# aszepieniec/stark-anatomy

Measured on AMD Instinct MI355X. Metric: ntt_field_elements_per_sec, higher is better.
Workload: dtype u128; 1 GPU; ntt_fwd_inv_2^20_1gpu; log2n=20, parallelism=single, passes_per_transform=2

## Files before the change

### stark-anatomy_amd/csrc/core.h

```cpp
#pragma once
#include <hip/hip_runtime.h>
#include <dlfcn.h>
#include <cstdio>
#include <cstdlib>
#include <cstring>
#include <algorithm>
#include <atomic>
#include <chrono>
#include <cerrno>
#include <thread>
#include <sys/random.h>
#include <deque>
#include <functional>
#include <future>
#include <map>
#include <mutex>
#include <string>
#include <tuple>
#include <vector>

#pragma GCC visibility push(default)
#include "../../include/starkcore.h"
#pragma GCC visibility pop
#include "ntt_plan.h"

namespace sc { struct FoldIn; }
using namespace sc;

struct sc_vec {
    Fe* d;
    uint64_t n;
    bool owned = true;
};
struct sc_later {
    int slot;
    uint64_t seq;
    hipStream_t st;
};
struct sc_merkle {
    uint64_t* d_levels;
    uint64_t N;
    int logN;
    int slot = -1;
    uint64_t seq = 0;
    hipStream_t st = nullptr;
    bool have_root = false;
    bool lazy = false;
    uint8_t root[64] = {};
};

struct sc_merkle_forest {
    uint64_t* d_levels;
    uint64_t N, count;
    int logN;
    uint64_t* h_roots = nullptr;
    Fe* d_cm = nullptr;
    hipEvent_t done = nullptr;
    hipStream_t st = nullptr;
    bool have_roots = false;
};

namespace sci {

struct DevBuf {
    void* p = nullptr;
    size_t bytes = 0;
};

struct PlanKey {
    int logn;
    uint64_t lo, hi;
    bool operator<(const PlanKey& o) const { return std::tie(logn, lo, hi) < std::tie(o.logn, o.lo, o.hi); }
};
struct PlanTables {
    Fe* mt = nullptr;
    int mt_log = 0;
    Fe* tl = nullptr;
    Fe* th = nullptr;
    Fe* th_ninv = nullptr;
    struct Direct { int logA, logR; bool scaled; Fe* d; };
    std::vector<Direct> direct;
    uint64_t last_use = 0;
};
struct OuterKey {
    uint64_t lo, hi, order, len, batch, col_base;
    int ninv;
    bool operator<(const OuterKey& o) const { return std::tie(lo, hi, order, len, batch, col_base, ninv) < std::tie(o.lo, o.hi, o.order, o.len, o.batch, o.col_base, o.ninv); }
};
struct OuterTable {
    Fe* d = nullptr;
    uint64_t last_use = 0;
};
struct PowKey {
    uint64_t lo, hi, hi_count;
    bool operator<(const PowKey& o) const { return std::tie(lo, hi, hi_count) < std::tie(o.lo, o.hi, o.hi_count); }
};
struct PowTables {
    Fe* lo = nullptr;
    Fe* hi = nullptr;
    uint64_t last_use = 0;
};

struct Ctx {
    bool init = false;
    int device = -1;
    hipStream_t stream = nullptr;
    std::string err;
    NttTuning tuning;
    std::map<PlanKey, PlanTables> plans;
    std::map<PowKey, PowTables> pows;
    std::map<OuterKey, OuterTable> outers;
    uint64_t tick = 0;
    bool foreign_streams = false;
    int small_divisor_direct = 1;
    int div_cols_launch_log = 26;
    int tree_cols_launch_log = 26;
    int eval_chunk_log = 8;
    int eval_points_across_min = 32;
    int eval_across_min_products_log = 26;
    int rescue_tree_split_max_nodes = -1;
    int grind_window = -1;
    int grind_unrolled = 0;
    int div_cols_chunk = 0;
    std::vector<hipStream_t> seen_streams;
    DevBuf scratch[8];
    std::map<hipStream_t, DevBuf> ntt_work;
    std::map<hipStream_t, DevBuf> ntt_flags;
    int fast_fixups = 1;
    int num_cus = 256;
    int xcd_remap = 1;
    int fixed_shapes = 1;
    int prio_balance = -1;
    int wave_local = 1;
    unsigned long long* trace = nullptr;
    int forest_four_lane_wgs = 256;
    int merkle_big_nlev = 2;
    int fri_tail = -1;
    int fri_tail_stall = -1;
    size_t verify_stage_bytes = 64ull << 20;
    uint8_t* root_slots = nullptr;
    uint8_t* later_words = nullptr;
    uint64_t root_seq = 0;
    std::vector<int> free_root_slots;
};
constexpr int ROOT_SLOTS = 256;
constexpr size_t ROOT_SLOT_BYTES = 128;
constexpr size_t LATER_WORD_BYTES = 128;
constexpr long SPIN_POLLS = 40000000;

struct PendingFree {
    void* p;
    size_t bytes;
    std::vector<hipEvent_t> evs;
};
#define HIPCHK(expr)                                                                                          \
    do {                                                                                                      \
        hipError_t _e = (expr);                                                                               \
        if (_e != hipSuccess) return fail(SC_ERR_HIP, std::string(#expr) + ": " + hipGetErrorString(_e));     \
    } while (0)

#define SCCHK(expr)              \
    do {                         \
        int _rc = (expr);        \
        if (_rc != SC_OK) return _rc; \
    } while (0)

struct NttOpts {
    uint64_t in_limit = ~0ull;
    const PowTables* coset = nullptr;
    uint32_t cols = 1;
    uint64_t col_stride_in = 0;
};
constexpr uint64_t COLS_ELEMS_PER_LAUNCH = 1ull << 26;
constexpr uint64_t SMALL_DIVISOR = 8;

constexpr uint64_t FUSE_MAX_W = 1ull << 17;

enum BuildMode { BUILD_SYNC = 0, BUILD_ASYNC = 1, BUILD_NOROOT = 2 };

extern Ctx g;
extern std::mutex g_mu;
extern hipStream_t g_comm_stream_for_free;
extern std::future<void> g_rand_worker;
extern size_t g_rand_prefetched;
extern std::multimap<size_t, void*> g_pool;
extern size_t g_pool_bytes, g_pool_cap;
extern std::deque<PendingFree> g_pending;
extern std::vector<hipEvent_t> g_event_pool;

void reap_pending(bool block);
hipError_t pool_alloc(void** p, size_t bytes);
void pool_free(void* p, size_t bytes);
void pool_clear();
hipEvent_t event_get();
int fail(int code, const std::string& msg);
int ensure_init();
int grow_buffer(DevBuf& b, size_t bytes, void** out);
inline int scratch(int slot, size_t bytes, void** out) { return grow_buffer(g.scratch[slot], bytes, out); }
int check_root(Fe root, uint64_t n);
int build_pow_table(Fe** out, uint64_t count, Fe base_m, uint64_t step, Fe scale_m, hipStream_t st);
void free_plans();
int evict_outer_tables();
int get_plan(Fe root, int logn, bool need_ninv, hipStream_t st, PlanTables** out);
inline NttTables tables_of(const PlanTables& t) {
    NttTables tb;
    tb.mt = t.mt; tb.mt_log = t.mt_log; tb.tl = t.tl; tb.th = t.th;
    return tb;
}
int get_pow(Fe base, uint64_t count, hipStream_t st, PowTables** out);
int plan_batched_direct(NttPlanDesc& d, BatchKind kind, int loglen, int logbatch, PlanTables* pt, const Fe* in, Fe* work, Fe* out, BatchExtras ex, hipStream_t st, bool* ok);
int run_plan(NttPlanDesc& d, hipStream_t st);
int ntt_device(const Fe* d_in, Fe* d_out, int logn, Fe root, bool inverse_scale, const NttOpts& o, hipStream_t st);
Fe root_inverse(Fe root, uint64_t n);
int ntt_any(const Fe* d_in, Fe* d_out, uint64_t n, Fe root, bool inverse, const NttOpts& o, hipStream_t st);
int upload(void* d, const void* h, size_t bytes, hipStream_t st);
int download(void* h, const void* d, size_t bytes, hipStream_t st);
int pointwise_div_device(const Fe* a, const Fe* b, Fe* out, uint64_t n, hipStream_t st);
int pointwise_div_enqueue(const Fe* a, const Fe* b, Fe* out, uint64_t n, hipStream_t st, uint32_t* flag);
int gather_device(const Fe* v, const uint64_t* d_idx, uint64_t k, Fe* d_out, hipStream_t st);
int read_small_polled(const void* d_src, size_t bytes, hipStream_t st, void* host_out);
bool upload_small(void* d_dst, const void* host, size_t bytes, hipStream_t st);

int merkle_climb(uint64_t* levels, uint64_t N, int lvl, hipStream_t st, volatile uint64_t* host = nullptr, uint64_t seq = 0, bool* published = nullptr);
int merkle_finish(uint64_t* levels, uint64_t width, hipStream_t st);
int root_slot_get();
int merkle_build_device(const Fe* d_elems, uint64_t N, uint8_t root_out[64], sc_merkle** tree, hipStream_t st, BuildMode mode = BUILD_SYNC, const FoldIn* fold = nullptr);
int merkle_root_wait(sc_merkle* t, bool from_free = false);
void root_poll_unlocked(std::unique_lock<std::mutex>& lk, const sc_merkle* t);
int fold_prepare(const Fe* d_in, uint64_t N, Fe alpha, Fe offset, Fe omega, Fe* d_out, hipStream_t st, FoldIn* f);
int fold_device(const Fe* d_in, uint64_t N, Fe alpha, Fe offset, Fe omega, Fe* d_out, hipStream_t st);
int fold_and_build(const Fe* d_in, uint64_t N, Fe alpha, Fe offset, Fe omega, Fe* d_out, sc_merkle** tree, hipStream_t st);
int fold_constants(uint64_t N, Fe offset, Fe omega, hipStream_t st, PowTables** pw_out, Fe* i2o_m_out);
int host_pool_get(size_t bytes, void** out);
int host_pool_put(void* p);
bool host_pool_holds(const void* p, size_t bytes);
int verify_stage_buffer(size_t bytes, uint8_t** out);

int grind_seeds_locked(const std::string& what, const void* seeds, uint64_t count, int bits, uint64_t start, uint64_t max_nonces, uint64_t* nonces_out,
                       uint8_t* found_out, void* stream);

Fe canonical_root(int logn);
Fe ninv_scaled(int logn, int j);
int ntt_cols(const Fe* in, Fe* out, int loglen, int logbatch, bool inverse, hipStream_t st);

constexpr size_t SEEN_STREAMS = 8;
inline hipStream_t pick_stream(void* s) {
    if (s && (hipStream_t)s != g.stream) {
        g.foreign_streams = true;
        hipStream_t st = (hipStream_t)s;
        if (g.seen_streams.size() <= SEEN_STREAMS && std::find(g.seen_streams.begin(), g.seen_streams.end(), st) == g.seen_streams.end())
            g.seen_streams.push_back(st);
    }
    return s ? (hipStream_t)s : g.stream;
}
inline void release_after_streams(void* p, size_t bytes) {
    if (!p) return;
    if (g.seen_streams.size() > SEEN_STREAMS) {
        (void)hipDeviceSynchronize();
        g.seen_streams.clear();
        pool_free(p, bytes);
        return;
    }
    PendingFree f{p, bytes, {}};
    auto mark = [&](hipStream_t st) -> bool {
        if (hipStreamQuery(st) == hipSuccess) return true;
        (void)hipGetLastError();
        hipEvent_t e = event_get();
        if (!e) { (void)hipStreamSynchronize(st); (void)hipGetLastError(); return true; }
        if (hipEventRecord(e, st) != hipSuccess) { (void)hipGetLastError(); g_event_pool.push_back(e); return false; }
        f.evs.push_back(e);
        return true;
    };
    if (g.stream) (void)mark(g.stream);
    if (g_comm_stream_for_free) (void)mark(g_comm_stream_for_free);
    for (size_t i = 0; i < g.seen_streams.size();) {
        if (mark(g.seen_streams[i])) ++i;
        else g.seen_streams.erase(g.seen_streams.begin() + i);
    }
    if (f.evs.empty()) { pool_free(p, bytes); return; }
    g_pending.push_back(std::move(f));
    reap_pending(false);
}
inline Fe fe_from(const uint64_t v[2]) { return Fe{v[0], v[1]}; }
inline bool is_pow2(uint64_t n) { return n && !(n & (n - 1)); }
inline int ilog2(uint64_t n) { int l = 0; while ((1ull << l) < n) ++l; return l; }

struct PoolTmp {
    void* p = nullptr;
    size_t bytes = 0;
    ~PoolTmp() { if (p) pool_free(p, bytes); }
    int get(size_t b) {
        bytes = b;
        HIPCHK(pool_alloc(&p, b));
        return SC_OK;
    }
    Fe* fe() const { return (Fe*)p; }
};

struct PoolTmpAsync {
    void* p = nullptr;
    size_t bytes = 0;
    ~PoolTmpAsync() { if (p) release_after_streams(p, bytes); }
    int get(size_t b) {
        bytes = b ? b : sizeof(Fe);
        HIPCHK(pool_alloc(&p, bytes));
        return SC_OK;
    }
    Fe* fe() const { return (Fe*)p; }
};

}
using namespace sci;
```

### stark-anatomy_amd/csrc/core.hip

```cpp
#include "core.h"


template <int LOGE> struct PassThreads { static constexpr int value = LOGE >= 4 ? 256 : (LOGE == 3 ? 512 : 1024); };

template <int LOGE>
__global__ void __launch_bounds__(PassThreads<LOGE>::value) ntt_pass_kernel(const PassParams P, uint32_t ntiles, int xcd_remap) {
    extern __shared__ __attribute__((aligned(16))) unsigned char smem_raw[];
    Fe* lds = reinterpret_cast<Fe*>(smem_raw);
    uint32_t wg = blockIdx.x, colbits = 0;
    if (P.col_enable) { colbits = (wg >> P.col_tiles_log) << P.col_tiles_log; wg -= colbits; }
    uint32_t tile = wg;
    if (xcd_remap) tile = (wg & 7u) * (ntiles >> 3) + (wg >> 3);
    tile |= colbits;
    Fe* tw = lds + (1u << (P.logR + P.logC));
    tile_twiddles_to_lds(P, P.logR, threadIdx.x, blockDim.x, tw);
    __syncthreads();
    const int nrounds = (P.logR + LOGE - 1) / LOGE;
    int sh = P.logR;
    for (int r = 0; r < nrounds; ++r) {
        const int s = (r == 0) ? (P.logR - LOGE * (nrounds - 1)) : LOGE;
        sh -= s;
        ntt_round_dispatch<LOGE>(P, s, sh, r == 0, tile, threadIdx.x, lds, tw);
        if (r + 1 < nrounds) __syncthreads();
    }
}

constexpr int TRACE_STAMPS = 16;
template <int LOGE, int GLR, int GLC, bool TRACE, bool ALT = false>
__global__ void __launch_bounds__(1 << (GLR + GLC - LOGE)) ntt_pass_kernel_fixed(const PassParams P, uint32_t ntiles, int xcd_remap, int wave_local) {
    extern __shared__ __attribute__((aligned(16))) unsigned char smem_raw[];
    Fe* lds = reinterpret_cast<Fe*>(smem_raw);
    unsigned long long* trow = nullptr;
    if constexpr (TRACE) {
        if (P.trace) {
            trow = P.trace + ((size_t)blockIdx.x * (blockDim.x >> 6) + (threadIdx.x >> 6)) * TRACE_STAMPS;
            if ((threadIdx.x & 63u) == 0) { trow[0] = __builtin_amdgcn_s_memtime(); trow[15] = __builtin_amdgcn_s_memrealtime(); }
        }
    }
    uint32_t wg = blockIdx.x, colbits = 0;
    if (P.col_enable) { colbits = (wg >> P.col_tiles_log) << P.col_tiles_log; wg -= colbits; }
    uint32_t tile = wg;
    if (xcd_remap) tile = (wg & 7u) * (ntiles >> 3) + (wg >> 3);
    tile |= colbits;
    Fe* tw = lds + (1u << (GLR + GLC));
    auto stamp = [&](int i) {
        if constexpr (TRACE) {
            if (trow) {
                if (i == 2) __builtin_amdgcn_s_waitcnt(0);
                if ((threadIdx.x & 63u) == 0 && i < 13) trow[i] = __builtin_amdgcn_s_memtime();
            }
        }
    };
    auto sync = [] { __syncthreads(); };
    auto wsync = [] { __builtin_amdgcn_fence(__ATOMIC_RELEASE, "wavefront"); __builtin_amdgcn_wave_barrier(); __builtin_amdgcn_fence(__ATOMIC_ACQUIRE, "wavefront"); };
    FixedRounds<LOGE, GLR, GLC, 0, ALT>::run(P, tile, threadIdx.x, lds, tw, sync, wsync, stamp, wave_local != 0);
    if constexpr (TRACE) {
        if (trow && (threadIdx.x & 63u) == 0) { __builtin_amdgcn_s_waitcnt(0); trow[14] = __builtin_amdgcn_s_memtime(); trow[13] = __builtin_amdgcn_s_memrealtime(); }
    }
}

template <int GLR, int GLC>
__device__ __forceinline__ uint32_t fixed8_tile(const PassParams& P, uint32_t index, uint32_t ntiles, int xcd_remap) {
    uint32_t wg = index, colbits = 0;
    if (P.col_enable) { colbits = (wg >> P.col_tiles_log) << P.col_tiles_log; wg -= colbits; }
    uint32_t tile = wg;
    if (xcd_remap) tile = (wg & 7u) * (ntiles >> 3) + (wg >> 3);
    return tile | colbits;
}
template <int GLR, int GLC>
__global__ void __launch_bounds__(1 << (GLR + GLC - 3)) __attribute__((amdgpu_waves_per_eu(4)))
ntt_pass_kernel_fixed8(const PassParams P, uint32_t ntiles, int xcd_remap, int wave_local, uint32_t* flags) {
    extern __shared__ __attribute__((aligned(16))) unsigned char smem_raw[];
    Fe* lds = reinterpret_cast<Fe*>(smem_raw);
    const uint32_t tile = fixed8_tile<GLR, GLC>(P, blockIdx.x, ntiles, xcd_remap);
    Fe* tw = lds + (1u << (GLR + GLC));
    auto stamp = [](int) {};
    auto sync = [] { __syncthreads(); };
    auto wsync = [] { __builtin_amdgcn_fence(__ATOMIC_RELEASE, "wavefront"); __builtin_amdgcn_wave_barrier(); __builtin_amdgcn_fence(__ATOMIC_ACQUIRE, "wavefront"); };
    rare_t rare = 0;
    FixedRounds<3, GLR, GLC, 0, false, true>::run(P, tile, threadIdx.x, lds, tw, sync, wsync, stamp, wave_local != 0, rare);
    if (rare_any(rare)) Round<3, 3, GLR, GLC>::store_word_at(flags + blockIdx.x, 0u, 1u);
}

template <int GLR, int GLC>
__global__ void __launch_bounds__(1 << (GLR + GLC - 3)) __attribute__((amdgpu_waves_per_eu(4)))
ntt_pass_redo8_kernel(const PassParams P, uint32_t ntiles, int xcd_remap, int wave_local, uint32_t* flags, int all) {
    extern __shared__ __attribute__((aligned(16))) unsigned char smem_raw[];
    if (!all && flags[blockIdx.x] == 0) return;
    Fe* lds = reinterpret_cast<Fe*>(smem_raw);
    Fe* tw = lds + (1u << (GLR + GLC));
    auto stamp = [](int) {};
    auto sync = [] { __syncthreads(); };
    auto wsync = [] { __builtin_amdgcn_fence(__ATOMIC_RELEASE, "wavefront"); __builtin_amdgcn_wave_barrier(); __builtin_amdgcn_fence(__ATOMIC_ACQUIRE, "wavefront"); };
    FixedRounds<3, GLR, GLC, 0, false>::run(P, fixed8_tile<GLR, GLC>(P, blockIdx.x, ntiles, xcd_remap), threadIdx.x, lds, tw, sync, wsync, stamp, wave_local != 0);
    if (!all) __syncthreads();
    if (threadIdx.x == 0) flags[blockIdx.x] = 0;
}

__global__ void __launch_bounds__(256) pow_table_kernel(Fe* out, uint64_t count, Fe base_m, uint64_t step, Fe scale_m) {
    uint64_t i = (uint64_t)blockIdx.x * blockDim.x + threadIdx.x;
    if (i < count) out[i] = pow_table_entry(base_m, i, step, scale_m);
}

__global__ void __launch_bounds__(256) twiddle_table_kernel(Fe* out, int logB, uint64_t count, uint64_t scale_exp, const Fe* __restrict__ tl, const Fe* __restrict__ th) {
    uint64_t i = (uint64_t)blockIdx.x * blockDim.x + threadIdx.x;
    if (i >= count) return;
    uint64_t k = i >> logB, b = i & ((1ull << logB) - 1);
    out[i] = pow2level(tl, th, b * k * scale_exp);
}

__global__ void __launch_bounds__(256) pointwise_mul_kernel(const Fe* __restrict__ a, const Fe* __restrict__ b, Fe* __restrict__ out, uint64_t n) {
    uint64_t i = (uint64_t)blockIdx.x * blockDim.x + threadIdx.x;
    if (i < n) out[i] = fe_mul(a[i], b[i]);
}

template <int K>
__global__ void __launch_bounds__(256) pointwise_div_kernel(const Fe* __restrict__ a, const Fe* __restrict__ b, Fe* __restrict__ out, uint64_t n, uint32_t* flag) {
    const uint64_t nthreads = (uint64_t)gridDim.x * blockDim.x;
    const uint64_t t = (uint64_t)blockIdx.x * blockDim.x + threadIdx.x;
    Fe bm[K], pre[K];
    Fe acc = fe_mont_one();
    bool zero = false;
#pragma unroll
    for (int k = 0; k < K; ++k) {
        uint64_t i = t + (uint64_t)k * nthreads;
        Fe v = (i < n) ? b[i] : fe_one();
        zero |= fe_is_zero(v);
        bm[k] = to_mont(v);
        pre[k] = acc;
        acc = mont_mul(acc, bm[k]);
    }
    if (zero) atomicOr(flag, 1u);
    Fe inv = mont_inv(acc);
#pragma unroll
    for (int k = K - 1; k >= 0; --k) {
        uint64_t i = t + (uint64_t)k * nthreads;
        Fe ik = mont_mul(inv, pre[k]);
        inv = mont_mul(inv, bm[k]);
        if (i < n) out[i] = mont_mul(a[i], ik);
    }
}

__global__ void __launch_bounds__(256) short_poly_coset_kernel(const Fe* __restrict__ b, uint32_t nb, Fe off_m, const Fe* __restrict__ tl, const Fe* __restrict__ th, Fe* __restrict__ out, uint64_t order) {
    const uint64_t i = (uint64_t)blockIdx.x * blockDim.x + threadIdx.x;
    if (i >= order) return;
    const Fe x_m = mont_mul(off_m, pow2level(tl, th, i));
    Fe acc = b[nb - 1];
    for (uint32_t k = nb - 1; k-- > 0;) acc = fe_add(mont_mul(acc, x_m), b[k]);
    out[i] = acc;
}

__global__ void __launch_bounds__(256) scale_pow_kernel(const Fe* __restrict__ in, Fe* __restrict__ out, uint64_t n, const Fe* __restrict__ lo, const Fe* __restrict__ hi) {
    uint64_t i = (uint64_t)blockIdx.x * blockDim.x + threadIdx.x;
    if (i < n) out[i] = mont_mul(in[i], pow2level(lo, hi, i));
}

__global__ void __launch_bounds__(256) scale_slab_kernel(const Fe* __restrict__ in, Fe* __restrict__ out, uint64_t rows, int logcols, uint64_t row_len, uint64_t col_base,
                                                         const Fe* __restrict__ lo, const Fe* __restrict__ hi) {
    uint64_t t = (uint64_t)blockIdx.x * blockDim.x + threadIdx.x;
    if (t >= (rows << logcols)) return;
    uint64_t r = t >> logcols, c = t & ((1ull << logcols) - 1);
    out[t] = mont_mul(in[t], pow2level(lo, hi, r * row_len + col_base + c));
}

__global__ void __launch_bounds__(256) axpy_shift_kernel(Fe* __restrict__ acc, const Fe* __restrict__ src, uint64_t n_src, uint64_t shift, Fe w_m) {
    uint64_t j = (uint64_t)blockIdx.x * blockDim.x + threadIdx.x;
    if (j >= n_src) return;
    acc[shift + j] = fe_add(acc[shift + j], mont_mul(src[j], w_m));
}

constexpr int DEGREE_PER_THREAD = 4;
constexpr unsigned DEGREE_MAX_BLOCKS = 2048;
constexpr int DEGREE_SLOTS = 8;
__global__ void __launch_bounds__(256) vec_degree_kernel(const Fe* __restrict__ v, uint64_t n, long long* out) {
    const uint64_t step = (uint64_t)gridDim.x * (256 * DEGREE_PER_THREAD);
    long long best = -1;
    for (uint64_t base = (uint64_t)blockIdx.x * (256 * DEGREE_PER_THREAD) + threadIdx.x; base - threadIdx.x < n; base += step) {
        Fe x[DEGREE_PER_THREAD];
#pragma unroll
        for (int k = 0; k < DEGREE_PER_THREAD; ++k) {
            const uint64_t i = base + 256u * k;
            x[k] = i < n ? v[i] : Fe{0, 0};
        }
#pragma unroll
        for (int k = 0; k < DEGREE_PER_THREAD; ++k) {
            const unsigned long long lanes = __ballot(!fe_is_zero(x[k]));
            if (lanes) best = (long long)(base - (threadIdx.x & 63u) + 256u * k + (63 - __clzll((long long)lanes)));
        }
    }
    __shared__ long long wave_best[4];
    if ((threadIdx.x & 63u) == 0) wave_best[threadIdx.x >> 6] = best;
    __syncthreads();
    if (threadIdx.x == 0) {
        long long m = wave_best[0];
#pragma unroll
        for (int w = 1; w < 4; ++w) m = wave_best[w] > m ? wave_best[w] : m;
        if (m >= 0) atomicMax(out + (blockIdx.x & (DEGREE_SLOTS - 1)), m);
    }
}
__global__ void __launch_bounds__(256) vec_degree_cols_kernel(const Fe* __restrict__ v, uint64_t n, uint64_t ld, uint32_t per_col, long long* out) {
    const uint64_t col = blockIdx.x / per_col;
    const uint32_t part = blockIdx.x - (uint32_t)col * per_col;
    const Fe* __restrict__ w = v + col * ld;
    const uint64_t step = (uint64_t)per_col * (256 * DEGREE_PER_THREAD);
    long long best = -1;
    for (uint64_t base = (uint64_t)part * (256 * DEGREE_PER_THREAD) + threadIdx.x; base - threadIdx.x < n; base += step) {
        Fe x[DEGREE_PER_THREAD];
#pragma unroll
        for (int k = 0; k < DEGREE_PER_THREAD; ++k) {
            const uint64_t i = base + 256u * k;
            x[k] = i < n ? w[i] : Fe{0, 0};
        }
#pragma unroll
        for (int k = 0; k < DEGREE_PER_THREAD; ++k) {
            const unsigned long long lanes = __ballot(!fe_is_zero(x[k]));
            if (lanes) best = (long long)(base - (threadIdx.x & 63u) + 256u * k + (63 - __clzll((long long)lanes)));
        }
    }
    __shared__ long long wave_best[4];
    if ((threadIdx.x & 63u) == 0) wave_best[threadIdx.x >> 6] = best;
    __syncthreads();
    if (threadIdx.x == 0) {
        long long m = wave_best[0];
#pragma unroll
        for (int k = 1; k < 4; ++k) m = wave_best[k] > m ? wave_best[k] : m;
        if (m >= 0) atomicMax(out + col, m);
    }
}
static int degree_read(void* fl, hipStream_t st, long long* deg) {
    long long slots[DEGREE_SLOTS];
    SCCHK(read_small_polled(fl, sizeof slots, st, slots));
    long long m = -1;
    for (int i = 0; i < DEGREE_SLOTS; ++i) m = slots[i] > m ? slots[i] : m;
    *deg = m;
    return SC_OK;
}
static inline unsigned degree_blocks(uint64_t n) {
    const uint64_t b = (n + 256 * DEGREE_PER_THREAD - 1) / (256 * DEGREE_PER_THREAD);
    return (unsigned)(b < DEGREE_MAX_BLOCKS ? (b ? b : 1) : DEGREE_MAX_BLOCKS);
}

__global__ void __launch_bounds__(256) mpoly_eval_kernel(const Fe* __restrict__ vals_m, uint32_t nvars, uint64_t n, const uint8_t* __restrict__ exps,
                                                        const Fe* __restrict__ coef_m, uint32_t nterms, Fe* __restrict__ out, const uint64_t* __restrict__ where) {
    uint64_t i = (uint64_t)blockIdx.x * blockDim.x + threadIdx.x;
    if (i >= n) return;
    Fe acc{0, 0};
    for (uint32_t t = 0; t < nterms; ++t) {
        Fe p = coef_m[t];
        const uint8_t* e = exps + (size_t)t * nvars;
        for (uint32_t j = 0; j < nvars; ++j) {
            const uint32_t ej = e[j];
            if (ej == 0) continue;
            const Fe v = where ? vals_m[where[2 * j] * n + ((i + where[2 * j + 1]) & (n - 1))] : vals_m[(uint64_t)j * n + i];
            for (uint32_t k = 0; k < ej; ++k) p = mont_mul(p, v);
        }
        acc = fe_add(acc, p);
    }
    out[i] = from_mont(acc);
}
__global__ void __launch_bounds__(256) to_mont_kernel(Fe* __restrict__ a, uint64_t n) {
    uint64_t i = (uint64_t)blockIdx.x * blockDim.x + threadIdx.x;
    if (i < n) a[i] = to_mont(a[i]);
}

__global__ void __launch_bounds__(256) field_selftest_kernel(int op, const Fe* __restrict__ a, const Fe* __restrict__ b, Fe* __restrict__ out, uint64_t n) {
    uint64_t i = (uint64_t)blockIdx.x * blockDim.x + threadIdx.x;
    if (i >= n) return;
    Fe x = a[i], y = b[i], r;
    switch (op) {
        case 0: r = mont_mul(x, y); break;
        case 1: r = fe_add(x, y); break;
        case 2: r = fe_sub(x, y); break;
        case 3: r = fe_mul(x, y); break;
        case 4: r = fe_half(x); break;
        case 5: r = from_mont(mont_inv(to_mont(x))); break;
        case 7: {
            Fe r0, r1;
            mont_mul2(x, y, x, y, r0, r1);
            r = fe_eq(r0, r1) ? r0 : Fe{~0ull, ~0ull};
            break;
        }
        default: r = mont_mul_c(x, y); break;
    }
    out[i] = r;
}

template <bool MASK> __device__ __forceinline__ uint32_t selftest_word(rare_t rare) {
    const uint32_t own = MASK ? (uint32_t)((rare >> (threadIdx.x & 63u)) & 1u) : (uint32_t)(rare != 0);
    return own | (rare_any(rare) ? 2u : 0u);
}
__global__ void __launch_bounds__(256) field_selftest2_kernel(int op, const Fe* __restrict__ a, const Fe* __restrict__ b, const Fe* __restrict__ c,
                                                             const Fe* __restrict__ d, Fe* __restrict__ out, uint32_t* __restrict__ word, uint64_t n) {
    uint64_t i = (uint64_t)blockIdx.x * blockDim.x + threadIdx.x;
    if (i >= n) return;
    const Fe x = a[i], y = b[i], z = c[i], w = d[i];
    Fe r0{0, 0}, r1{0, 0}, r2{0, 0}, r3{0, 0};
    rare_t rare = 0;
    uint32_t flags = 0;
    switch (op) {
        case 0: mont_mul2(x, y, z, w, r0, r1); break;
        case 1: fe_addsub2(x, y, z, w, r0, r1, r2, r3); break;
        case 2: r0 = fe_add_fast(x, y, rare); flags = selftest_word<SC_ASM_ADDSUB != 0>(rare); break;
        case 3: r0 = fe_sub_fast(x, y, rare); flags = selftest_word<SC_ASM_ADDSUB != 0>(rare); break;
        case 4: r0 = mont_mul_fast(x, y, rare); flags = selftest_word<SC_ASM_MUL != 0>(rare); break;
        case 5: mont_mul2_fast(x, y, z, w, r0, r1, rare); flags = selftest_word<SC_ASM_MUL != 0>(rare); break;
        case 6: fe_addsub2_fast(x, y, z, w, r0, r1, r2, r3, rare); flags = selftest_word<SC_ASM_ADDSUB != 0>(rare); break;
        default: r0 = fe_neg(x); break;
    }
    out[i] = r0; out[n + i] = r1; out[2 * n + i] = r2; out[3 * n + i] = r3;
    word[i] = flags;
}

__global__ void __launch_bounds__(256) sample_bytes_kernel(const uint8_t* __restrict__ bytes, uint64_t count, uint32_t width, Fe* __restrict__ out) {
    uint64_t i = (uint64_t)blockIdx.x * blockDim.x + threadIdx.x;
    if (i >= count) return;
    out[i] = fe_sample_bytes(bytes + i * width, width);
}

__global__ void __launch_bounds__(256) gather_kernel(const Fe* __restrict__ v, const uint64_t* __restrict__ idx, uint64_t k, Fe* __restrict__ out) {
    uint64_t i = (uint64_t)blockIdx.x * blockDim.x + threadIdx.x;
    if (i < k) out[i] = v[idx[i]];
}


namespace sci {

Ctx g;
std::mutex g_mu;
hipStream_t g_comm_stream_for_free = nullptr;
std::future<void> g_rand_worker;
size_t g_rand_prefetched = 0;

std::multimap<size_t, void*> g_pool;
size_t g_pool_bytes = 0;
size_t g_pool_cap = 8ull << 30;

void reap_pending(bool block);
hipError_t pool_alloc(void** p, size_t bytes) {
    reap_pending(false);
    auto it = g_pool.find(bytes);
    if (it != g_pool.end()) {
        *p = it->second;
        g_pool.erase(it);
        g_pool_bytes -= bytes;
        return hipSuccess;
    }
    const bool slow_log = getenv("STARKCORE_LOG_SLOW_ALLOC") != nullptr;
    const auto t0 = std::chrono::steady_clock::now();
    hipError_t e = hipMalloc(p, bytes);
    if (slow_log) {
        const double ms = std::chrono::duration<double, std::milli>(std::chrono::steady_clock::now() - t0).count();
        if (ms > 1.0) fprintf(stderr, "starkcore: hipMalloc(%zu MB) took %.1f ms (pool %zu MB in %zu buffers)\n", bytes >> 20, ms, g_pool_bytes >> 20, g_pool.size());
    }
    if (e != hipSuccess) {
        (void)hipGetLastError();
        reap_pending(true);
        auto it2 = g_pool.find(bytes);
        if (it2 != g_pool.end()) {
            *p = it2->second;
            g_pool.erase(it2);
            g_pool_bytes -= bytes;
            return hipSuccess;
        }
        e = hipMalloc(p, bytes);
    }
    if (e != hipSuccess && !g_pool.empty()) {
        (void)hipDeviceSynchronize();
        for (auto& kv : g_pool) (void)hipFree(kv.second);
        g_pool.clear();
        g_pool_bytes = 0;
        (void)hipGetLastError();
        e = hipMalloc(p, bytes);
    }
    return e;
}

void pool_free(void* p, size_t bytes) {
    if (!p) return;
    if (g_pool_bytes + bytes <= g_pool_cap) {
        g_pool.emplace(bytes, p);
        g_pool_bytes += bytes;
    } else {
        const auto t0 = std::chrono::steady_clock::now();
        (void)hipFree(p);
        if (getenv("STARKCORE_LOG_SLOW_ALLOC")) {
            const double ms = std::chrono::duration<double, std::milli>(std::chrono::steady_clock::now() - t0).count();
            if (ms > 1.0) fprintf(stderr, "starkcore: hipFree(%zu MB) took %.1f ms (pool at its cap of %zu MB)\n", bytes >> 20, ms, g_pool_cap >> 20);
        }
    }
}

void pool_clear() {
    for (auto& kv : g_pool) (void)hipFree(kv.second);
    g_pool.clear();
    g_pool_bytes = 0;
}

std::deque<PendingFree> g_pending;
std::vector<hipEvent_t> g_event_pool;

hipEvent_t event_get() {
    if (!g_event_pool.empty()) { hipEvent_t e = g_event_pool.back(); g_event_pool.pop_back(); return e; }
    hipEvent_t e = nullptr;
    if (hipEventCreateWithFlags(&e, hipEventDisableTiming) != hipSuccess) { (void)hipGetLastError(); return nullptr; }
    return e;
}

void reap_pending(bool block) {
    for (size_t i = 0; i < g_pending.size();) {
        PendingFree& f = g_pending[i];
        bool done = true;
        for (hipEvent_t e : f.evs) {
            hipError_t q = block ? hipEventSynchronize(e) : hipEventQuery(e);
            if (q == hipErrorNotReady) { (void)hipGetLastError(); done = false; break; }
            if (q != hipSuccess) (void)hipGetLastError();
        }
        if (!done) { ++i; continue; }
        for (hipEvent_t e : f.evs) g_event_pool.push_back(e);
        pool_free(f.p, f.bytes);
        g_pending[i] = std::move(g_pending.back());
        g_pending.pop_back();
    }
}

int fail(int code, const std::string& msg) {
    g.err = msg;
    return code;
}

int ensure_init() {
    if (g.init) {
        static thread_local int bound = -1;
        if (bound != g.device) { HIPCHK(hipSetDevice(g.device)); bound = g.device; }
        return SC_OK;
    }
    int n = 0;
    hipError_t e = hipGetDeviceCount(&n);
    if (e != hipSuccess || n <= 0) return fail(SC_ERR_HIP, std::string("no HIP device available: ") + hipGetErrorString(e));
    int dev = 0;
    if (const char* lr = getenv("LOCAL_RANK")) dev = atoi(lr) % n;
    if (const char* sd = getenv("STARKCORE_DEVICE")) dev = atoi(sd) % n;
    HIPCHK(hipSetDevice(dev));
    HIPCHK(hipStreamCreateWithFlags(&g.stream, hipStreamNonBlocking));
    { int cus = 0; if (hipDeviceGetAttribute(&cus, hipDeviceAttributeMultiprocessorCount, dev) == hipSuccess && cus > 0) g.num_cus = cus; }
    { size_t free_b = 0, total_b = 0; if (hipMemGetInfo(&free_b, &total_b) == hipSuccess && total_b) g_pool_cap = total_b / 4; else (void)hipGetLastError(); }
    if (const char* lws = getenv("LOCAL_WORLD_SIZE")) { const int per_dev = (atoi(lws) + n - 1) / n; if (per_dev > 1) g_pool_cap /= (size_t)per_dev; }
    if (const char* cap = getenv("STARKCORE_POOL_CAP_MB")) g_pool_cap = (size_t)atoll(cap) << 20;
    g.device = dev;
    g.init = true;
    return SC_OK;
}

int grow_buffer(DevBuf& b, size_t bytes, void** out) {
    if (b.bytes < bytes) {
        if (b.p) { HIPCHK(hipDeviceSynchronize()); HIPCHK(hipFree(b.p)); b.p = nullptr; b.bytes = 0; }
        size_t want = bytes < (1u << 20) ? (1u << 20) : bytes;
        HIPCHK(hipMalloc(&b.p, want));
        b.bytes = want;
    }
    *out = b.p;
    return SC_OK;
}

int check_root(Fe root, uint64_t n) {
    if (fe_ge_p(root)) return fail(SC_ERR_BAD_ARG, "root is not a canonical residue");
    Fe rm = to_mont(root);
    Fe one = fe_mont_one();
    Fe half = mont_pow(rm, n / 2);
    Fe full = mont_mul(half, half);
    if (!fe_eq(full, one)) return fail(SC_ERR_ROOT_ORDER, "primitive root must be nth root of unity, where n is len(values)");
    if (fe_eq(half, one)) return fail(SC_ERR_ROOT_NOT_PRIMITIVE, "primitive root is not primitive nth root of unity, where n is len(values)");
    return SC_OK;
}

int build_pow_table(Fe** out, uint64_t count, Fe base_m, uint64_t step, Fe scale_m, hipStream_t st) {
    if (count == 0) count = 1;
    HIPCHK(hipMalloc((void**)out, count * sizeof(Fe)));
    unsigned blocks = (unsigned)((count + 255) / 256);
    hipLaunchKernelGGL(pow_table_kernel, dim3(blocks), dim3(256), 0, st, *out, count, base_m, step, scale_m);
    HIPCHK(hipGetLastError());
    return SC_OK;
}

void free_plan_tables(PlanTables& t) {
    hipFree(t.mt); hipFree(t.tl); hipFree(t.th);
    if (t.th_ninv) hipFree(t.th_ninv);
    for (const PlanTables::Direct& e : t.direct) hipFree(e.d);
}

void free_plans() {
    for (auto& kv : g.plans) free_plan_tables(kv.second);
    g.plans.clear();
    for (auto& kv : g.pows) { hipFree(kv.second.lo); hipFree(kv.second.hi); }
    g.pows.clear();
    for (auto& kv : g.outers) hipFree(kv.second.d);
    g.outers.clear();
}

constexpr uint64_t PIN_WINDOW = 64;
constexpr size_t PLAN_CAP = 256, POW_CAP = 64;

template <class Map, class FreeFn>
int evict_tables(Map& m, size_t cap, FreeFn free_entry) {
    if (m.size() < cap) return SC_OK;
    std::vector<std::pair<uint64_t, typename Map::iterator>> old;
    for (auto it = m.begin(); it != m.end(); ++it)
        if (it->second.last_use + PIN_WINDOW < g.tick) old.emplace_back(it->second.last_use, it);
    if (old.empty()) return SC_OK;
    std::sort(old.begin(), old.end(), [](const auto& a, const auto& b) { return a.first < b.first; });
    size_t drop = cap / 4 ? cap / 4 : 1;
    if (drop > old.size()) drop = old.size();
    HIPCHK(hipDeviceSynchronize());
    for (size_t i = 0; i < drop; ++i) { free_entry(old[i].second->second); m.erase(old[i].second); }
    return SC_OK;
}

int get_plan(Fe root, int logn, bool need_ninv, hipStream_t st, PlanTables** out) {
    PlanKey key{logn, root.lo, root.hi};
    auto it = g.plans.find(key);
    bool built = false;
    ++g.tick;
    if (it == g.plans.end()) {
        SCCHK(evict_tables(g.plans, PLAN_CAP, free_plan_tables));
        const uint64_t n = 1ull << logn;
        Fe rm = to_mont(root);
        const TableSizes sz = table_sizes(logn);
        PlanTables t;
        t.mt_log = sz.mt_log;
        SCCHK(build_pow_table(&t.mt, sz.mt, rm, n >> sz.mt_log, fe_mont_one(), st));
        SCCHK(build_pow_table(&t.tl, sz.tl, rm, 1, fe_mont_one(), st));
        SCCHK(build_pow_table(&t.th, sz.th, rm, 4096, fe_mont_one(), st));
        it = g.plans.emplace(key, t).first;
        built = true;
    }
    if (need_ninv && !it->second.th_ninv) {
        const uint64_t n = 1ull << logn;
        Fe ninv_m = mont_inv(to_mont(Fe{n, 0}));
        SCCHK(build_pow_table(&it->second.th_ninv, table_sizes(logn).th, to_mont(root), 4096, ninv_m, st));
        built = true;
    }
    if (built) HIPCHK(hipStreamSynchronize(st));
    it->second.last_use = g.tick;
    *out = &it->second;
    return SC_OK;
}

int get_pow(Fe base, uint64_t count, hipStream_t st, PowTables** out) {
    uint64_t hi_count = (count >> 12) + 1;
    uint64_t hc = 1; while (hc < hi_count) hc <<= 1;
    PowKey key{base.lo, base.hi, hc};
    auto it = g.pows.find(key);
    ++g.tick;
    if (it == g.pows.end()) {
        SCCHK(evict_tables(g.pows, POW_CAP, [](PowTables& t) { hipFree(t.lo); hipFree(t.hi); }));
        Fe bm = to_mont(base);
        PowTables t;
        SCCHK(build_pow_table(&t.lo, 4096, bm, 1, fe_mont_one(), st));
        SCCHK(build_pow_table(&t.hi, hc, bm, 4096, fe_mont_one(), st));
        HIPCHK(hipStreamSynchronize(st));
        it = g.pows.emplace(key, t).first;
    }
    it->second.last_use = g.tick;
    *out = &it->second;
    return SC_OK;
}

int direct_twiddles(PlanTables* pt, const NttPlanDesc& d, int i, bool scaled, hipStream_t st, const Fe** out) {
    const DirectTable t = direct_table(d, i, scaled);
    *out = nullptr;
    if (t.logR + t.logB > g.tuning.direct_tw_max_log) return SC_OK;
    for (const PlanTables::Direct& e : pt->direct)
        if (e.logA == t.logA && e.logR == t.logR && e.scaled == t.scaled) { *out = e.d; return SC_OK; }
    const uint64_t count = 1ull << (t.logR + t.logB);
    Fe* p;
    HIPCHK(hipMalloc((void**)&p, count * sizeof(Fe)));
    pt->direct.push_back({t.logA, t.logR, t.scaled, p});
    hipLaunchKernelGGL(twiddle_table_kernel, dim3((unsigned)((count + 255) / 256)), dim3(256), 0, st, p, t.logB, count, 1ull << t.logA,
                       pt->tl, t.scaled ? pt->th_ninv : pt->th);
    HIPCHK(hipGetLastError());
    HIPCHK(hipStreamSynchronize(st));
    *out = p;
    return SC_OK;
}

int plan_batched_direct(NttPlanDesc& d, BatchKind kind, int loglen, int logbatch, PlanTables* pt, const Fe* in, Fe* work, Fe* out, BatchExtras ex, hipStream_t st, bool* ok) {
    const NttTables tb = tables_of(*pt);
    *ok = plan_batched(d, kind, loglen, logbatch, tb, in, work, out, g.tuning, ex);
    if (!*ok || d.npasses != 2) return SC_OK;
    SCCHK(direct_twiddles(pt, d, 0, false, st, &ex.inner_twd));
    if (ex.inner_twd) *ok = plan_batched(d, kind, loglen, logbatch, tb, in, work, out, g.tuning, ex);
    return SC_OK;
}

int pass_flags(hipStream_t st, uint32_t nwg, uint32_t** out) {
    DevBuf& b = g.ntt_flags[st];
    const void* before = b.p;
    const size_t had = b.bytes;
    void* p;
    SCCHK(grow_buffer(b, (size_t)nwg * sizeof(uint32_t), &p));
    if (p != before || b.bytes != had) HIPCHK(hipMemsetAsync(p, 0, b.bytes, st));
    *out = (uint32_t*)p;
    return SC_OK;
}

template <int LOGE>
int launch_pass(const NttPassDesc& pd, hipStream_t st) {
    int remap = (g.xcd_remap && pd.ntiles >= 16 && (pd.ntiles & 7u) == 0) ? 1 : 0;
    const PassKernel k = pass_kernel(pd, g.fixed_shapes != 0);
    if constexpr (LOGE == 2) {
        if (k.kind == PK_FIXED4) {
            const int lr = pd.p.logR, lc = pd.p.logC;
#define SC_LAUNCH_FIXED(LR, LC, TR, ALT) \
    hipLaunchKernelGGL((ntt_pass_kernel_fixed<2, LR, LC, TR, ALT>), dim3(pd.ntiles * pd.cols), dim3(pd.threads), pd.lds_bytes, st, pd.p, pd.ntiles, remap, g.wave_local)
#define SC_FIXED(LR, LC)                                                          \
            if (lr == LR && lc == LC) {                                           \
                if (k.trace) SC_LAUNCH_FIXED(LR, LC, true, false);                \
                else if (k.alt) SC_LAUNCH_FIXED(LR, LC, false, true);             \
                else SC_LAUNCH_FIXED(LR, LC, false, false);                       \
                return SC_OK;                                                     \
            }
            SC_FIXED4_SHAPES(SC_FIXED)
#undef SC_FIXED
        }
    }
    if constexpr (LOGE == 3) {
        if (k.kind == PK_FIXED8) {
            const int lr = pd.p.logR, lc = pd.p.logC;
            const uint32_t nwg = pd.ntiles * pd.cols;
            const bool fast = g.fast_fixups != 0 && fast_pass_ok(pd.p) && !pass_in_place(pd);
            const int all = (!fast || g.fast_fixups == 2) ? 1 : 0;
            uint32_t* flags;
            SCCHK(pass_flags(st, nwg, &flags));
#define SC_FIXED8(LR, LC)                                                                                                                                   \
            if (lr == LR && lc == LC) {                                                                                                                     \
                if (fast) hipLaunchKernelGGL((ntt_pass_kernel_fixed8<LR, LC>), dim3(nwg), dim3(pd.threads), pd.lds_bytes, st, pd.p, pd.ntiles, remap, g.wave_local, flags); \
                hipLaunchKernelGGL((ntt_pass_redo8_kernel<LR, LC>), dim3(nwg), dim3(pd.threads), pd.lds_bytes, st, pd.p, pd.ntiles, remap, g.wave_local, flags, all); \
                return SC_OK;                                                                                                                               \
            }
            SC_FIXED8_SHAPES(SC_FIXED8)
#undef SC_FIXED8
        }
    }
    hipLaunchKernelGGL(ntt_pass_kernel<LOGE>, dim3(pd.ntiles * pd.cols), dim3(pd.threads), pd.lds_bytes, st, pd.p, pd.ntiles, remap);
    return SC_OK;
}

int run_plan(NttPlanDesc& d, hipStream_t st) {
    size_t trace_off = 0;
    for (int i = 0; i < d.npasses; ++i) {
        d.pass[i].p.prio_balance = pass_prio_balance(d.pass[i], g.prio_balance, g.num_cus);
        d.pass[i].p.trace = g.trace ? g.trace + trace_off : nullptr;
        trace_off += (size_t)d.pass[i].ntiles * d.pass[i].cols * (d.pass[i].threads >> 6) * TRACE_STAMPS;
        switch (d.pass[i].loge) {
            case 1: SCCHK(launch_pass<1>(d.pass[i], st)); break;
            case 2: SCCHK(launch_pass<2>(d.pass[i], st)); break;
            case 3: SCCHK(launch_pass<3>(d.pass[i], st)); break;
            case 4: SCCHK(launch_pass<4>(d.pass[i], st)); break;
            default: return fail(SC_ERR_UNSUPPORTED, "bad loge");
        }
        HIPCHK(hipGetLastError());
    }
    return SC_OK;
}

int ntt_device(const Fe* d_in, Fe* d_out, int logn, Fe root, bool inverse_scale, const NttOpts& o, hipStream_t st) {
    PlanTables* pt;
    SCCHK(get_plan(root, logn, inverse_scale, st, &pt));
    const uint64_t n = 1ull << logn;
    const int m = plan_num_passes(logn, g.tuning);
    NttTables tb = tables_of(*pt);
    tb.th_scaled = (inverse_scale && m > 1) ? pt->th_ninv : nullptr;
    NttIo io;
    io.in = d_in; io.out = d_out; io.in_limit = o.in_limit; io.cols = o.cols; io.col_stride_in = o.col_stride_in;
    if (m > 1) { void* w; SCCHK(grow_buffer(g.ntt_work[st], n * o.cols * sizeof(Fe), &w)); io.work = (Fe*)w; }
    if (o.coset) { io.ol = o.coset->lo; io.oh = o.coset->hi; }
    if (inverse_scale && m == 1) { io.scale_last = true; io.scale = mont_inv(to_mont(Fe{n, 0})); }
    NttPlanDesc d;
    if (!plan_ntt(d, logn, tb, io, g.tuning)) return fail(SC_ERR_UNSUPPORTED, "unsupported transform length");
    if (d.npasses > 1) {
        bool any = false;
        for (int i = 0; i + 1 < d.npasses; ++i) {
            SCCHK(direct_twiddles(pt, d, i, inverse_scale, st, &tb.twd[i]));
            any |= tb.twd[i] != nullptr;
        }
        if (any && !plan_ntt(d, logn, tb, io, g.tuning)) return fail(SC_ERR_UNSUPPORTED, "unsupported transform length");
    }
    return run_plan(d, st);
}

Fe root_inverse(Fe root, uint64_t n) {
    return from_mont(mont_pow(to_mont(root), n - 1));
}

int ntt_any(const Fe* d_in, Fe* d_out, uint64_t n, Fe root, bool inverse, const NttOpts& o, hipStream_t st) {
    if (n <= 1) {
        if (n == 1 && d_in != d_out) HIPCHK(hipMemcpyAsync(d_out, d_in, sizeof(Fe), hipMemcpyDeviceToDevice, st));
        return SC_OK;
    }
    if (!is_pow2(n)) return fail(SC_ERR_NOT_POW2, "cannot compute ntt of non-power-of-two sequence");
    SCCHK(check_root(root, n));
    return ntt_device(d_in, d_out, ilog2(n), inverse ? root_inverse(root, n) : root, inverse, o, st);
}

int upload(void* d, const void* h, size_t bytes, hipStream_t st) {
    if (bytes) HIPCHK(hipMemcpyAsync(d, h, bytes, hipMemcpyHostToDevice, st));
    return SC_OK;
}
int download(void* h, const void* d, size_t bytes, hipStream_t st) {
    if (bytes) HIPCHK(hipMemcpyAsync(h, d, bytes, hipMemcpyDeviceToHost, st));
    HIPCHK(hipStreamSynchronize(st));
    return SC_OK;
}

int pointwise_div_enqueue(const Fe* a, const Fe* b, Fe* out, uint64_t n, hipStream_t st, uint32_t* flag) {
    HIPCHK(hipMemsetAsync(flag, 0, 8, st));
    static const int K = [] { const char* e = getenv("STARKCORE_DIV_K"); return e && atoi(e) == 8 ? 8 : 16; }();
    const uint64_t threads = (n + K - 1) / K;
    const unsigned blocks = (unsigned)((threads + 255) / 256);
    if (K == 8) hipLaunchKernelGGL(pointwise_div_kernel<8>, dim3(blocks), dim3(256), 0, st, a, b, out, n, flag);
    else hipLaunchKernelGGL(pointwise_div_kernel<16>, dim3(blocks), dim3(256), 0, st, a, b, out, n, flag);
    HIPCHK(hipGetLastError());
    return SC_OK;
}
int pointwise_div_device(const Fe* a, const Fe* b, Fe* out, uint64_t n, hipStream_t st) {
    void* fl;
    SCCHK(scratch(4, 256, &fl));
    SCCHK(pointwise_div_enqueue(a, b, out, n, st, (uint32_t*)fl));
    uint64_t hflag = 0;
    SCCHK(read_small_polled(fl, 8, st, &hflag));
    if ((uint32_t)hflag) return fail(SC_ERR_DIV_ZERO, "divide by zero");
    return SC_OK;
}

__global__ void __launch_bounds__(64) words_publish_kernel(const uint64_t* __restrict__ src, uint32_t nwords, volatile uint64_t* host, uint64_t seq) {
    if (threadIdx.x < nwords) host[threadIdx.x] = src[threadIdx.x];
    __threadfence_system();
    if (threadIdx.x == 0) host[8] = seq;
}
int read_small_polled(const void* d_src, size_t bytes, hipStream_t st, void* host_out) {
    const int slot = (bytes <= 64 && ((uintptr_t)d_src & 7) == 0) ? root_slot_get() : -1;
    if (slot < 0) {
        HIPCHK(hipMemcpyAsync(host_out, d_src, bytes, hipMemcpyDeviceToHost, st));
        HIPCHK(hipStreamSynchronize(st));
        return SC_OK;
    }
    const uint64_t seq = ++g.root_seq;
    volatile uint64_t* host = (volatile uint64_t*)(g.root_slots + ROOT_SLOT_BYTES * slot);
    hipLaunchKernelGGL(words_publish_kernel, dim3(1), dim3(64), 0, st, (const uint64_t*)d_src, (uint32_t)((bytes + 7) / 8), host, seq);
    hipError_t e = hipGetLastError();
    bool landed = false;
    if (e == hipSuccess) {
        for (long spin = 0; spin < SPIN_POLLS; ++spin) {
            if (__atomic_load_n(host + 8, __ATOMIC_ACQUIRE) == seq) { landed = true; break; }
            if ((spin & 4095) == 4095) {
                e = hipStreamQuery(st);
                if (e != hipErrorNotReady) break;
                (void)hipGetLastError();
                e = hipSuccess;
            }
        }
        if (!landed) {
            (void)hipGetLastError();
            e = hipStreamSynchronize(st);
            landed = e == hipSuccess && __atomic_load_n(host + 8, __ATOMIC_ACQUIRE) == seq;
            if (e == hipSuccess && !landed) e = hipErrorUnknown;
        }
    }
    if (landed) memcpy(host_out, (const void*)host, bytes);
    else (void)hipStreamSynchronize(st);
    g.free_root_slots.push_back(slot);
    if (!landed) return fail(SC_ERR_HIP, hipGetErrorString(e));
    return SC_OK;
}

static int later_words(int slot, uint32_t** zero_flag, long long** degree_slots) {
    if (!g.later_words) HIPCHK(hipMalloc((void**)&g.later_words, LATER_WORD_BYTES * ROOT_SLOTS));
    uint8_t* w = g.later_words + LATER_WORD_BYTES * slot;
    *degree_slots = (long long*)w;
    *zero_flag = (uint32_t*)(w + DEGREE_SLOTS * sizeof(long long));
    return SC_OK;
}
__global__ void __launch_bounds__(64) divide_flags_publish_kernel(const uint32_t* __restrict__ zero_flag, const long long* __restrict__ degree_slots,
                                                                 volatile uint64_t* host, uint64_t seq) {
    if (threadIdx.x == 0) {
        long long m = -1;
        if (degree_slots) for (int i = 0; i < DEGREE_SLOTS; ++i) m = degree_slots[i] > m ? degree_slots[i] : m;
        host[0] = zero_flag ? (uint64_t)*zero_flag : 0ull;
        host[1] = (uint64_t)m;
        __threadfence_system();
        host[8] = seq;
    }
}
static int divide_flags_later(int slot, const uint32_t* zero_flag, const long long* degree_slots, hipStream_t st, sc_later** out) {
    const uint64_t seq = ++g.root_seq;
    volatile uint64_t* host = (volatile uint64_t*)(g.root_slots + ROOT_SLOT_BYTES * slot);
    hipLaunchKernelGGL(divide_flags_publish_kernel, dim3(1), dim3(64), 0, st, zero_flag, degree_slots, host, seq);
    HIPCHK(hipGetLastError());
    *out = new sc_later{slot, seq, st};
    return SC_OK;
}
static int later_abandon(int slot, hipStream_t st, int rc) {
    (void)hipStreamSynchronize(st);
    g.free_root_slots.push_back(slot);
    return rc;
}
int later_wait(sc_later* h, uint64_t words[8]) {
    volatile uint64_t* host = (volatile uint64_t*)(g.root_slots + ROOT_SLOT_BYTES * h->slot);
    bool landed = false;
    hipError_t e = hipSuccess;
    for (long spin = 0; spin < SPIN_POLLS; ++spin) {
        if (__atomic_load_n(host + 8, __ATOMIC_ACQUIRE) == h->seq) { landed = true; break; }
        if ((spin & 4095) == 4095) {
            e = hipStreamQuery(h->st);
            if (e != hipErrorNotReady) break;
            (void)hipGetLastError();
            e = hipSuccess;
        }
    }
    if (!landed) {
        (void)hipGetLastError();
        e = hipStreamSynchronize(h->st);
        landed = e == hipSuccess && __atomic_load_n(host + 8, __ATOMIC_ACQUIRE) == h->seq;
        if (e == hipSuccess && !landed) e = hipErrorUnknown;
    }
    if (landed) memcpy(words, (const void*)host, 64);
    g.free_root_slots.push_back(h->slot);
    delete h;
    if (!landed) return fail(SC_ERR_HIP, hipGetErrorString(e));
    return SC_OK;
}

int gather_device(const Fe* v, const uint64_t* d_idx, uint64_t k, Fe* d_out, hipStream_t st) {
    hipLaunchKernelGGL(gather_kernel, dim3((unsigned)((k + 255) / 256)), dim3(256), 0, st, v, d_idx, k, d_out);
    HIPCHK(hipGetLastError());
    return SC_OK;
}

int evict_outer_tables() { return evict_tables(g.outers, (size_t)16, [](OuterTable& t) { hipFree(t.d); }); }

}


extern "C" {

int sc_device_count(void) {
    int n = 0;
    if (hipGetDeviceCount(&n) != hipSuccess) return 0;
    return n;
}

int sc_init(int device) {
    std::lock_guard<std::mutex> lk(g_mu);
    if (g.init && (device < 0 || device == g.device)) return SC_OK;
    if (g.init) return fail(SC_ERR_BAD_ARG, "already initialised on another device");
    if (device >= 0) { char buf[16]; snprintf(buf, sizeof buf, "%d", device); setenv("STARKCORE_DEVICE", buf, 1); }
    return ensure_init();
}

int sc_shutdown(void) {
    std::lock_guard<std::mutex> lk(g_mu);
    if (g_rand_worker.valid()) { g_rand_worker.get(); g_rand_prefetched = 0; }
    if (!g.init) return SC_OK;
    hipDeviceSynchronize();
    reap_pending(true);
    for (hipEvent_t e : g_event_pool) (void)hipEventDestroy(e);
    g_event_pool.clear();
    free_plans();
    pool_clear();
    for (auto& b : g.scratch) { if (b.p) hipFree(b.p); b = DevBuf{}; }
    for (auto& kv : g.ntt_work) if (kv.second.p) hipFree(kv.second.p);
    g.ntt_work.clear();
    for (auto& kv : g.ntt_flags) if (kv.second.p) hipFree(kv.second.p);
    g.ntt_flags.clear();
    if (g.later_words) hipFree(g.later_words);
    g.later_words = nullptr;
    if (g.stream) hipStreamDestroy(g.stream);
    g.stream = nullptr;
    g.seen_streams.clear();
    g.foreign_streams = false;
    g.init = false;
    return SC_OK;
}

const char* sc_last_error(void) { return g.err.c_str(); }

int sc_synchronize(void) {
    std::lock_guard<std::mutex> lk(g_mu);
    SCCHK(ensure_init());
    HIPCHK(hipStreamSynchronize(g.stream));
    return SC_OK;
}

int sc_stream(void** stream_out) {
    std::lock_guard<std::mutex> lk(g_mu);
    SCCHK(ensure_init());
    if (!stream_out) return fail(SC_ERR_BAD_ARG, "null argument");
    *stream_out = (void*)g.stream;
    return SC_OK;
}

int sc_stream_join(void* other) {
    std::lock_guard<std::mutex> lk(g_mu);
    SCCHK(ensure_init());
    hipStream_t o = (hipStream_t)other;
    if (o == g.stream) return SC_OK;
    (void)pick_stream(other);
    hipEvent_t a = event_get(), b = event_get();
    if (!a || !b) { if (a) g_event_pool.push_back(a); if (b) g_event_pool.push_back(b); HIPCHK(hipStreamSynchronize(o)); HIPCHK(hipStreamSynchronize(g.stream)); return SC_OK; }
    hipError_t e = hipEventRecord(a, o);
    if (e == hipSuccess) e = hipStreamWaitEvent(g.stream, a, 0);
    if (e == hipSuccess) e = hipEventRecord(b, g.stream);
    if (e == hipSuccess) e = hipStreamWaitEvent(o, b, 0);
    g_event_pool.push_back(a);
    g_event_pool.push_back(b);
    if (e != hipSuccess) return fail(SC_ERR_HIP, hipGetErrorString(e));
    return SC_OK;
}

int sc_set_tuning(const char* key, int value) {
    std::lock_guard<std::mutex> lk(g_mu);
    std::string k(key ? key : "");
    if (k == "max_tile_log") g.tuning.max_tile_log = value;
    else if (k == "loge") g.tuning.loge = value;
    else if (k == "max_col_log") g.tuning.max_col_log = value;
    else if (k == "min_tiles_log") g.tuning.min_tiles_log = value;
    else if (k == "single_pass_max_log") g.tuning.single_pass_max_log = value;
    else if (k == "max_digit_log") g.tuning.max_digit_log = value;
    else if (k == "direct_tw_max_log") g.tuning.direct_tw_max_log = value;
    else if (k == "xcd_remap") g.xcd_remap = value;
    else if (k == "fixed_shapes") g.fixed_shapes = value;
    else if (k == "wave_local") g.wave_local = value;
    else if (k == "fast_fixups") g.fast_fixups = value < 0 ? 0 : (value > 2 ? 2 : value);
    else if (k == "prio_balance") g.prio_balance = value;
    else if (k == "loge_cols") g.tuning.loge_cols = value;
    else if (k == "tw_on_load") g.tuning.tw_on_load = value;
    else if (k == "prune") g.tuning.prune = value;
    else if (k == "merkle_big_nlev") g.merkle_big_nlev = value < 0 ? 0 : (value > 8 ? 8 : value);
    else if (k == "forest_four_lane_wgs") g.forest_four_lane_wgs = value < 0 ? 0 : value;
    else if (k == "fri_tail") g.fri_tail = value ? 1 : 0;
    else if (k == "small_divisor_direct") g.small_divisor_direct = value ? 1 : 0;
    else if (k == "div_cols_chunk") g.div_cols_chunk = value < 0 ? 0 : (value > 65535 ? 65535 : value);
    else if (k == "div_cols_launch_log") g.div_cols_launch_log = value < 1 ? 1 : (value > 26 ? 26 : value);
    else if (k == "tree_cols_launch_log") g.tree_cols_launch_log = value < 1 ? 1 : (value > 26 ? 26 : value);
    else if (k == "eval_chunk_log") g.eval_chunk_log = value < 8 ? 8 : (value > 24 ? 24 : value);
    else if (k == "eval_points_across_min") g.eval_points_across_min = value < 1 ? 1 : value;
    else if (k == "eval_across_min_products_log") g.eval_across_min_products_log = value < 0 ? 0 : (value > 64 ? 64 : value);
    else if (k == "rescue_tree_split_max_nodes") g.rescue_tree_split_max_nodes = value < -1 ? -1 : value;
    else if (k == "grind_window") g.grind_window = value < 1 ? -1 : value;
    else if (k == "grind_unrolled") g.grind_unrolled = value > 0 ? 1 : 0;
    else if (k == "verify_stage_kb") g.verify_stage_bytes = (size_t)(value < 16 ? 16 : value) << 10;
    else if (k == "fri_tail_stall") g.fri_tail_stall = value;
    else if (k == "pool_cap_mb") g_pool_cap = (size_t)(value < 0 ? 0 : value) << 20;
    else if (k == "pool_trim") {
        if (g.init) { (void)hipDeviceSynchronize(); reap_pending(true); pool_clear(); }
    }
    else return fail(SC_ERR_BAD_ARG, "unknown tuning key " + k);
    return SC_OK;
}

int sc_ntt_num_passes(uint64_t n) {
    std::lock_guard<std::mutex> lk(g_mu);
    if (n < 2 || !is_pow2(n)) return 0;
    return plan_num_passes(ilog2(n), g.tuning);
}

int sc_debug_trace(void* d_buf) {
    std::lock_guard<std::mutex> lk(g_mu);
    g.trace = (unsigned long long*)d_buf;
    return SC_OK;
}

int sc_vec_alloc(uint64_t n, sc_vec_t** out) {
    std::lock_guard<std::mutex> lk(g_mu);
    SCCHK(ensure_init());
    sc_vec* v = new sc_vec{nullptr, n};
    hipError_t e = pool_alloc((void**)&v->d, (n ? n : 1) * sizeof(Fe));
    if (e != hipSuccess) { delete v; return fail(SC_ERR_HIP, hipGetErrorString(e)); }
    *out = v;
    return SC_OK;
}
int sc_vec_free(sc_vec_t* v) {
    std::lock_guard<std::mutex> lk(g_mu);
    if (!v) return SC_OK;
    if (v->owned) release_after_streams(v->d, (v->n ? v->n : 1) * sizeof(Fe));
    delete v;
    return SC_OK;
}
int sc_vec_wrap(void* d_elems, uint64_t n, sc_vec_t** out) {
    if (!d_elems || !out) return fail(SC_ERR_BAD_ARG, "null argument");
    sc_vec* v = new sc_vec{(Fe*)d_elems, n};
    v->owned = false;
    *out = v;
    return SC_OK;
}
uint64_t sc_vec_len(const sc_vec_t* v) { return v ? v->n : 0; }
void* sc_vec_ptr(sc_vec_t* v) { return v ? v->d : nullptr; }
int sc_vec_zero(sc_vec_t* v) {
    std::lock_guard<std::mutex> lk(g_mu);
    if (!v) return fail(SC_ERR_BAD_ARG, "null vector");
    SCCHK(ensure_init());
    if (v->n) HIPCHK(hipMemsetAsync(v->d, 0, v->n * sizeof(Fe), g.stream));
    return SC_OK;
}
}
namespace sci {
struct SmallPayload { uint64_t w[256]; };
__global__ void __launch_bounds__(256) small_upload_kernel(uint64_t* __restrict__ dst, const SmallPayload p, uint32_t nwords) {
    if (threadIdx.x < nwords) dst[threadIdx.x] = p.w[threadIdx.x];
}
bool upload_small(void* d_dst, const void* host, size_t bytes, hipStream_t st) {
    if (bytes > 4 * sizeof(SmallPayload)) return false;
    const uint8_t* src = (const uint8_t*)host;
    uint64_t* dst = (uint64_t*)d_dst;
    for (size_t left = bytes; left;) {
        const size_t take = left < sizeof(SmallPayload) ? left : sizeof(SmallPayload);
        SmallPayload p;
        p.w[(take - 1) / 8] = 0;
        memcpy(p.w, src, take);
        hipLaunchKernelGGL(small_upload_kernel, dim3(1), dim3(256), 0, st, dst, p, (uint32_t)((take + 7) / 8));
        src += take; dst += (take + 7) / 8; left -= take;
    }
    return hipGetLastError() == hipSuccess;
}
}
extern "C" {
int sc_vec_upload(sc_vec_t* v, uint64_t offset, const void* host, uint64_t count) {
    std::lock_guard<std::mutex> lk(g_mu);
    SCCHK(ensure_init());
    if (!v || offset + count > v->n) return fail(SC_ERR_BAD_ARG, "upload out of range");
    if (count && upload_small(v->d + offset, host, count * sizeof(Fe), g.stream)) return SC_OK;
    SCCHK(upload(v->d + offset, host, count * sizeof(Fe), g.stream));
    HIPCHK(hipStreamSynchronize(g.stream));
    return SC_OK;
}
int sc_vec_download(const sc_vec_t* v, uint64_t offset, void* host, uint64_t count) {
    std::lock_guard<std::mutex> lk(g_mu);
    SCCHK(ensure_init());
    if (!v || offset + count > v->n) return fail(SC_ERR_BAD_ARG, "download out of range");
    return download(host, v->d + offset, count * sizeof(Fe), g.stream);
}
int sc_sample_bytes_dev(const void* bytes, uint64_t count, uint32_t width, void* d_out, void* stream) {
    std::lock_guard<std::mutex> lk(g_mu);
    SCCHK(ensure_init());
    if (!count) return SC_OK;
    if (!bytes || !d_out || width == 0 || width > 32) return fail(SC_ERR_BAD_ARG, "byte strings of 1..32 bytes expected");
    hipStream_t st = pick_stream(stream);
    void* buf;
    SCCHK(scratch(6, count * width + 256, &buf));
    SCCHK(upload(buf, bytes, count * width, st));
    hipLaunchKernelGGL(sample_bytes_kernel, dim3((unsigned)((count + 255) / 256)), dim3(256), 0, st, (const uint8_t*)buf, count, width, (Fe*)d_out);
    HIPCHK(hipGetLastError());
    HIPCHK(hipStreamSynchronize(st));
    return SC_OK;
}
namespace {
uint8_t* g_rand_host = nullptr;
size_t g_rand_host_bytes = 0;
hipEvent_t g_rand_copied = nullptr;
std::atomic<int> g_rand_failed{0};

void rand_fill(size_t bytes) {
    unsigned hw = std::thread::hardware_concurrency();
    size_t nthreads = bytes / (256u << 10);
    if (nthreads > 32) nthreads = 32;
    if (hw && nthreads > hw) nthreads = hw;
    static const long cap = [] { const char* e = getenv("STARKCORE_RAND_THREADS"); return e ? atol(e) : 0L; }();
    if (cap > 0 && nthreads > (size_t)cap) nthreads = (size_t)cap;
    if (nthreads < 1) nthreads = 1;
    auto fill = [](size_t a, size_t b) {
        while (a < b) {
            size_t want = b - a < (1u << 20) ? b - a : (1u << 20);
            ssize_t r = getrandom(g_rand_host + a, want, 0);
            if (r < 0) { if (errno == EINTR) continue; g_rand_failed = 1; return; }
            a += (size_t)r;
        }
    };
    if (nthreads == 1) { fill(0, bytes); return; }
    std::vector<std::thread> pool;
    const size_t per = (bytes + nthreads - 1) / nthreads;
    for (size_t i = 0; i < nthreads; ++i) {
        const size_t a = i * per, b = a + per < bytes ? a + per : bytes;
        if (a < b) pool.emplace_back(fill, a, b);
    }
    for (auto& t : pool) t.join();
}
uint8_t* g_rand_dev = nullptr;
size_t g_rand_dev_bytes = 0;
hipStream_t g_rand_stream = nullptr;
hipEvent_t g_rand_consumed = nullptr;

int rand_buffer(size_t bytes) {
    if (g_rand_worker.valid()) { g_rand_worker.get(); g_rand_prefetched = 0; }
    if (g_rand_copied) HIPCHK(hipEventSynchronize(g_rand_copied));
    if (g_rand_consumed) HIPCHK(hipEventSynchronize(g_rand_consumed));
    if (g_rand_host_bytes < bytes) {
        if (g_rand_host) { (void)hipHostFree(g_rand_host); g_rand_host = nullptr; g_rand_host_bytes = 0; }
        HIPCHK(hipHostMalloc((void**)&g_rand_host, bytes, hipHostMallocDefault));
        g_rand_host_bytes = bytes;
    }
    if (g_rand_dev_bytes < bytes) {
        if (g_rand_dev) { (void)hipFree(g_rand_dev); g_rand_dev = nullptr; g_rand_dev_bytes = 0; }
        HIPCHK(hipMalloc((void**)&g_rand_dev, bytes + 256));
        g_rand_dev_bytes = bytes;
    }
    if (!g_rand_copied) HIPCHK(hipEventCreateWithFlags(&g_rand_copied, hipEventDisableTiming));
    if (!g_rand_consumed) HIPCHK(hipEventCreateWithFlags(&g_rand_consumed, hipEventDisableTiming));
    if (!g_rand_stream) HIPCHK(hipStreamCreateWithFlags(&g_rand_stream, hipStreamNonBlocking));
    return SC_OK;
}
void rand_fill_and_copy(size_t bytes, int device) {
    rand_fill(bytes);
    if (g_rand_failed) return;
    if (hipSetDevice(device) != hipSuccess || hipMemcpyAsync(g_rand_dev, g_rand_host, bytes, hipMemcpyHostToDevice, g_rand_stream) != hipSuccess ||
        hipEventRecord(g_rand_copied, g_rand_stream) != hipSuccess) {
        (void)hipGetLastError();
        g_rand_failed = 2;
    }
}
}
int sc_urandom_prefetch(uint64_t count, uint32_t width) {
    std::lock_guard<std::mutex> lk(g_mu);
    SCCHK(ensure_init());
    if (!count || width == 0 || width > 32) return fail(SC_ERR_BAD_ARG, "byte strings of 1..32 bytes expected");
    const size_t bytes = (size_t)count * width;
    SCCHK(rand_buffer(bytes));
    g_rand_failed = 0;
    g_rand_prefetched = bytes;
    g_rand_worker = std::async(std::launch::async, rand_fill_and_copy, bytes, g.device);
    return SC_OK;
}
int sc_sample_urandom_dev(uint64_t count, uint32_t width, void* d_out, void* stream) {
    std::lock_guard<std::mutex> lk(g_mu);
    SCCHK(ensure_init());
    if (!count) return SC_OK;
    if (!d_out || width == 0 || width > 32) return fail(SC_ERR_BAD_ARG, "byte strings of 1..32 bytes expected");
    hipStream_t st = pick_stream(stream);
    const size_t bytes = (size_t)count * width;
    if (g_rand_worker.valid() && g_rand_prefetched == bytes) {
        g_rand_worker.get();
        g_rand_prefetched = 0;
        if (g_rand_failed == 1) return fail(SC_ERR_HIP, "getrandom failed");
        if (g_rand_failed == 2) return fail(SC_ERR_HIP, "copy of the drawn bytes failed");
        HIPCHK(hipStreamWaitEvent(st, g_rand_copied, 0));
    } else {
        SCCHK(rand_buffer(bytes));
        g_rand_failed = 0;
        rand_fill(bytes);
        if (g_rand_failed) return fail(SC_ERR_HIP, "getrandom failed");
        HIPCHK(hipMemcpyAsync(g_rand_dev, g_rand_host, bytes, hipMemcpyHostToDevice, st));
        HIPCHK(hipEventRecord(g_rand_copied, st));
    }
    hipLaunchKernelGGL(sample_bytes_kernel, dim3((unsigned)((count + 255) / 256)), dim3(256), 0, st, (const uint8_t*)g_rand_dev, count, width, (Fe*)d_out);
    HIPCHK(hipGetLastError());
    HIPCHK(hipEventRecord(g_rand_consumed, st));
    return SC_OK;
}

int sc_memcpy_dev(void* d_dst, const void* d_src, uint64_t count, void* stream) {
    std::lock_guard<std::mutex> lk(g_mu);
    SCCHK(ensure_init());
    if (count && (!d_dst || !d_src)) return fail(SC_ERR_BAD_ARG, "null argument");
    if (count) HIPCHK(hipMemcpyAsync(d_dst, d_src, count * sizeof(Fe), hipMemcpyDeviceToDevice, pick_stream(stream)));
    return SC_OK;
}
int sc_vec_gather(const sc_vec_t* v, const uint64_t* indices, uint64_t k, void* host_out) {
    std::lock_guard<std::mutex> lk(g_mu);
    SCCHK(ensure_init());
    if (!v) return fail(SC_ERR_BAD_ARG, "null vector");
    if (k == 0) return SC_OK;
    for (uint64_t i = 0; i < k; ++i) if (indices[i] >= v->n) return fail(SC_ERR_BAD_ARG, "gather index out of range");
    void* buf;
    const size_t idx_bytes = (k * 8 + 255) & ~255ull;
    SCCHK(scratch(4, 256 + idx_bytes + k * sizeof(Fe), &buf));
    uint64_t* d_idx = (uint64_t*)((char*)buf + 256);
    Fe* d_out = (Fe*)((char*)buf + 256 + idx_bytes);
    SCCHK(upload(d_idx, indices, k * 8, g.stream));
    hipLaunchKernelGGL(gather_kernel, dim3((unsigned)((k + 255) / 256)), dim3(256), 0, g.stream, v->d, d_idx, k, d_out);
    HIPCHK(hipGetLastError());
    return download(host_out, d_out, k * sizeof(Fe), g.stream);
}

int sc_field_selftest(int op, const void* a, const void* b, void* out, uint64_t n) {
    std::lock_guard<std::mutex> lk(g_mu);
    SCCHK(ensure_init());
    if (!n) return SC_OK;
    void *da, *db, *dc;
    SCCHK(scratch(1, n * sizeof(Fe), &da));
    SCCHK(scratch(2, n * sizeof(Fe), &db));
    SCCHK(scratch(3, n * sizeof(Fe), &dc));
    SCCHK(upload(da, a, n * sizeof(Fe), g.stream));
    SCCHK(upload(db, b, n * sizeof(Fe), g.stream));
    hipLaunchKernelGGL(field_selftest_kernel, dim3((unsigned)((n + 255) / 256)), dim3(256), 0, g.stream, op, (const Fe*)da, (const Fe*)db, (Fe*)dc, n);
    HIPCHK(hipGetLastError());
    return download(out, dc, n * sizeof(Fe), g.stream);
}

int sc_field_selftest2(int op, const void* a, const void* b, const void* c, const void* d, void* out, uint32_t* word, uint64_t n) {
    std::lock_guard<std::mutex> lk(g_mu);
    SCCHK(ensure_init());
    if (op < 0 || op > 7) return fail(SC_ERR_BAD_ARG, "unknown field self-test op");
    if (!n) return SC_OK;
    if (!a || !b || !c || !d || !out || !word) return fail(SC_ERR_BAD_ARG, "null argument");
    void *din, *dout, *dword;
    const size_t plane = n * sizeof(Fe);
    SCCHK(scratch(1, 4 * plane, &din));
    SCCHK(scratch(2, 4 * plane, &dout));
    SCCHK(scratch(3, n * sizeof(uint32_t), &dword));
    const void* src[4] = {a, b, c, d};
    for (int k = 0; k < 4; ++k) SCCHK(upload((char*)din + k * plane, src[k], plane, g.stream));
    const Fe* in = (const Fe*)din;
    hipLaunchKernelGGL(field_selftest2_kernel, dim3((unsigned)((n + 255) / 256)), dim3(256), 0, g.stream, op, in, in + n, in + 2 * n, in + 3 * n,
                       (Fe*)dout, (uint32_t*)dword, n);
    HIPCHK(hipGetLastError());
    HIPCHK(hipMemcpyAsync(out, dout, 4 * plane, hipMemcpyDeviceToHost, g.stream));
    return download(word, dword, n * sizeof(uint32_t), g.stream);
}

int sc_ntt_dev(const void* d_in, void* d_out, uint64_t n, const uint64_t root[2], int inverse, void* stream) {
    std::lock_guard<std::mutex> lk(g_mu);
    SCCHK(ensure_init());
    return ntt_any((const Fe*)d_in, (Fe*)d_out, n, fe_from(root), inverse != 0, NttOpts{}, pick_stream(stream));
}

int sc_ntt_columns_dev(const void* d_in, void* d_out, uint64_t n, uint64_t cols, const uint64_t root[2], int inverse, void* stream) {
    std::lock_guard<std::mutex> lk(g_mu);
    SCCHK(ensure_init());
    hipStream_t st = pick_stream(stream);
    if (cols == 0) return SC_OK;
    if (n > 1 && !is_pow2(n)) return fail(SC_ERR_NOT_POW2, "cannot compute ntt of non-power-of-two sequence");
    if (n <= 1) {
        if (n == 1 && d_in != d_out) HIPCHK(hipMemcpyAsync(d_out, d_in, cols * sizeof(Fe), hipMemcpyDeviceToDevice, st));
        return SC_OK;
    }
    const Fe* in = (const Fe*)d_in;
    Fe* out = (Fe*)d_out;
    uint64_t per = COLS_ELEMS_PER_LAUNCH / n;
    if (per < 1) per = 1;
    if (per > 65536) per = 65536;
    for (uint64_t done = 0; done < cols; done += per) {
        NttOpts o;
        o.cols = (uint32_t)(cols - done < per ? cols - done : per);
        SCCHK(ntt_any(in + done * n, out + done * n, n, fe_from(root), inverse != 0, o, st));
    }
    return SC_OK;
}

int sc_ntt(const void* in, void* out, uint64_t n, const uint64_t root[2], int inverse) {
    std::lock_guard<std::mutex> lk(g_mu);
    SCCHK(ensure_init());
    if (n == 0) return SC_OK;
    if (!is_pow2(n)) return fail(SC_ERR_NOT_POW2, "cannot compute ntt of non-power-of-two sequence");
    void* a; void* b;
    SCCHK(scratch(1, n * sizeof(Fe), &a));
    SCCHK(scratch(2, n * sizeof(Fe), &b));
    SCCHK(upload(a, in, n * sizeof(Fe), g.stream));
    SCCHK(ntt_any((const Fe*)a, (Fe*)b, n, fe_from(root), inverse != 0, NttOpts{}, g.stream));
    return download(out, b, n * sizeof(Fe), g.stream);
}

int sc_coset_evaluate_dev(const void* d_coeffs, uint64_t m, const uint64_t offset[2], const uint64_t generator[2], uint64_t order, void* d_out, void* stream) {
    std::lock_guard<std::mutex> lk(g_mu);
    SCCHK(ensure_init());
    hipStream_t st = pick_stream(stream);
    if (m > order) return fail(SC_ERR_BAD_ARG, "more coefficients than the evaluation order");
    if (order <= 1) {
        if (order == 1) {
            if (m == 1) HIPCHK(hipMemcpyAsync(d_out, d_coeffs, sizeof(Fe), hipMemcpyDeviceToDevice, st));
            else HIPCHK(hipMemsetAsync(d_out, 0, sizeof(Fe), st));
        }
        return SC_OK;
    }
    if (!is_pow2(order)) return fail(SC_ERR_NOT_POW2, "cannot compute ntt of non-power-of-two sequence");
    Fe gen = fe_from(generator), off = fe_from(offset);
    SCCHK(check_root(gen, order));
    if (fe_ge_p(off)) return fail(SC_ERR_BAD_ARG, "offset is not a canonical residue");
    PowTables* pw;
    SCCHK(get_pow(off, m ? m : 1, st, &pw));
    NttOpts o;
    o.in_limit = m;
    o.coset = pw;
    return ntt_device((const Fe*)d_coeffs, (Fe*)d_out, ilog2(order), gen, false, o, st);
}

int sc_coset_evaluate_columns_dev(const void* d_coeffs, uint64_t m, uint64_t cols, const uint64_t offset[2], const uint64_t generator[2], uint64_t order, void* d_out, void* stream) {
    std::lock_guard<std::mutex> lk(g_mu);
    SCCHK(ensure_init());
    hipStream_t st = pick_stream(stream);
    if (cols == 0) return SC_OK;
    if (m == 0 || m > order) return fail(SC_ERR_BAD_ARG, m ? "more coefficients than the evaluation order" : "a batch of empty polynomials");
    if (!is_pow2(order)) return fail(SC_ERR_NOT_POW2, "cannot compute ntt of non-power-of-two sequence");
    if (order < 2) return fail(SC_ERR_BAD_ARG, "evaluation order below 2");
    Fe gen = fe_from(generator), off = fe_from(offset);
    SCCHK(check_root(gen, order));
    if (fe_ge_p(off)) return fail(SC_ERR_BAD_ARG, "offset is not a canonical residue");
    PowTables* pw;
    SCCHK(get_pow(off, m, st, &pw));
    uint64_t per = COLS_ELEMS_PER_LAUNCH / order;
    if (per < 1) per = 1;
    if (per > 65536) per = 65536;
    for (uint64_t done = 0; done < cols; done += per) {
        NttOpts o;
        o.in_limit = m;
        o.coset = pw;
        o.cols = (uint32_t)(cols - done < per ? cols - done : per);
        o.col_stride_in = m;
        SCCHK(ntt_device((const Fe*)d_coeffs + done * m, (Fe*)d_out + done * order, ilog2(order), gen, false, o, st));
    }
    return SC_OK;
}

int sc_coset_evaluate(const void* coeffs, uint64_t m, const uint64_t offset[2], const uint64_t generator[2], uint64_t order, void* out) {
    void* a; void* b;
    {
        std::lock_guard<std::mutex> lk(g_mu);
        SCCHK(ensure_init());
        if (order == 0) return SC_OK;
        if (m > order) return fail(SC_ERR_BAD_ARG, "more coefficients than the evaluation order");
        SCCHK(scratch(1, (m ? m : 1) * sizeof(Fe), &a));
        SCCHK(scratch(2, order * sizeof(Fe), &b));
        SCCHK(upload(a, coeffs, m * sizeof(Fe), g.stream));
    }
    SCCHK(sc_coset_evaluate_dev(a, m, offset, generator, order, b, nullptr));
    std::lock_guard<std::mutex> lk(g_mu);
    return download(out, b, order * sizeof(Fe), g.stream);
}

int sc_pointwise_mul_dev(const void* d_a, const void* d_b, void* d_out, uint64_t n, void* stream) {
    std::lock_guard<std::mutex> lk(g_mu);
    SCCHK(ensure_init());
    if (!n) return SC_OK;
    hipLaunchKernelGGL(pointwise_mul_kernel, dim3((unsigned)((n + 255) / 256)), dim3(256), 0, pick_stream(stream), (const Fe*)d_a, (const Fe*)d_b, (Fe*)d_out, n);
    HIPCHK(hipGetLastError());
    return SC_OK;
}
int sc_pointwise_div_dev(const void* d_a, const void* d_b, void* d_out, uint64_t n, void* stream) {
    std::lock_guard<std::mutex> lk(g_mu);
    SCCHK(ensure_init());
    if (!n) return SC_OK;
    return pointwise_div_device((const Fe*)d_a, (const Fe*)d_b, (Fe*)d_out, n, pick_stream(stream));
}
int sc_scale_dev(const void* d_in, void* d_out, uint64_t n, const uint64_t factor[2], void* stream) {
    std::lock_guard<std::mutex> lk(g_mu);
    SCCHK(ensure_init());
    if (!n) return SC_OK;
    if (!factor || fe_ge_p(fe_from(factor))) return fail(SC_ERR_BAD_ARG, "factor is not a canonical residue");
    hipStream_t st = pick_stream(stream);
    PowTables* pw;
    SCCHK(get_pow(fe_from(factor), n, st, &pw));
    hipLaunchKernelGGL(scale_pow_kernel, dim3((unsigned)((n + 255) / 256)), dim3(256), 0, st, (const Fe*)d_in, (Fe*)d_out, n, pw->lo, pw->hi);
    HIPCHK(hipGetLastError());
    return SC_OK;
}

int sc_axpy_shift_dev(void* d_acc, uint64_t n_acc, const void* d_src, uint64_t n_src, uint64_t shift, const uint64_t weight[2], void* stream) {
    std::lock_guard<std::mutex> lk(g_mu);
    SCCHK(ensure_init());
    if (!n_src) return SC_OK;
    if (shift + n_src > n_acc || shift + n_src < shift) return fail(SC_ERR_BAD_ARG, "shifted term does not fit the accumulator");
    Fe w = fe_from(weight);
    if (fe_ge_p(w)) return fail(SC_ERR_BAD_ARG, "weight is not a canonical residue");
    hipLaunchKernelGGL(axpy_shift_kernel, dim3((unsigned)((n_src + 255) / 256)), dim3(256), 0, pick_stream(stream), (Fe*)d_acc, (const Fe*)d_src, n_src, shift, to_mont(w));
    HIPCHK(hipGetLastError());
    return SC_OK;
}

int sc_scale_slab_dev(const void* d_in, void* d_out, uint64_t rows, uint64_t cols, uint64_t row_len, uint64_t col_base, const uint64_t factor[2], void* stream) {
    std::lock_guard<std::mutex> lk(g_mu);
    SCCHK(ensure_init());
    if (!rows || !cols) return SC_OK;
    if (!is_pow2(cols) || col_base + cols > row_len) return fail(SC_ERR_BAD_ARG, "slab columns must be a power of two inside the row");
    if (!factor || fe_ge_p(fe_from(factor))) return fail(SC_ERR_BAD_ARG, "factor is not a canonical residue");
    hipStream_t st = pick_stream(stream);
    PowTables* pw;
    SCCHK(get_pow(fe_from(factor), rows * row_len, st, &pw));
    const uint64_t cnt = rows * cols;
    hipLaunchKernelGGL(scale_slab_kernel, dim3((unsigned)((cnt + 255) / 256)), dim3(256), 0, st, (const Fe*)d_in, (Fe*)d_out, rows, ilog2(cols), row_len, col_base, pw->lo, pw->hi);
    HIPCHK(hipGetLastError());
    return SC_OK;
}

int sc_poly_mul(const void* a, uint64_t na, const void* b, uint64_t nb, const uint64_t root[2], uint64_t order, void* out, uint64_t n_out) {
    std::lock_guard<std::mutex> lk(g_mu);
    SCCHK(ensure_init());
    if (!is_pow2(order) || order < 2) return fail(SC_ERR_NOT_POW2, "cannot compute ntt of non-power-of-two sequence");
    if (na > order || nb > order || n_out > order || na == 0 || nb == 0) return fail(SC_ERR_BAD_ARG, "operand longer than the transform order");
    Fe rt = fe_from(root);
    SCCHK(check_root(rt, order));
    hipStream_t st = g.stream;
    void *da, *db, *dc;
    SCCHK(scratch(1, order * sizeof(Fe), &da));
    SCCHK(scratch(2, order * sizeof(Fe), &db));
    SCCHK(scratch(3, order * sizeof(Fe), &dc));
    const int logn = ilog2(order);
    NttOpts o;
    SCCHK(upload(dc, a, na * sizeof(Fe), st));
    o.in_limit = na;
    SCCHK(ntt_device((const Fe*)dc, (Fe*)da, logn, rt, false, o, st));
    SCCHK(upload(dc, b, nb * sizeof(Fe), st));
    o.in_limit = nb;
    SCCHK(ntt_device((const Fe*)dc, (Fe*)db, logn, rt, false, o, st));
    hipLaunchKernelGGL(pointwise_mul_kernel, dim3((unsigned)((order + 255) / 256)), dim3(256), 0, st, (const Fe*)da, (const Fe*)db, (Fe*)dc, order);
    HIPCHK(hipGetLastError());
    SCCHK(ntt_device((const Fe*)dc, (Fe*)da, logn, root_inverse(rt, order), true, NttOpts{}, st));
    return download(out, da, n_out * sizeof(Fe), st);
}

static int coset_divide_core(const Fe* d_a, uint64_t na, const Fe* d_b, uint64_t nb, Fe off, Fe rt, uint64_t order, Fe** full, hipStream_t st, uint32_t* zero_flag = nullptr) {
    void *da, *db, *dc;
    SCCHK(scratch(1, order * sizeof(Fe), &da));
    SCCHK(scratch(2, order * sizeof(Fe), &db));
    SCCHK(scratch(3, order * sizeof(Fe), &dc));
    const int logn = ilog2(order);
    PowTables* pw;
    SCCHK(get_pow(off, order, st, &pw));
    NttOpts o;
    o.coset = pw;
    o.in_limit = na;
    SCCHK(ntt_device(d_a, (Fe*)da, logn, rt, false, o, st));
    if (nb <= SMALL_DIVISOR && g.small_divisor_direct) {
        PlanTables* pt;
        SCCHK(get_plan(rt, logn, false, st, &pt));
        hipLaunchKernelGGL(short_poly_coset_kernel, dim3((unsigned)((order + 255) / 256)), dim3(256), 0, st, d_b, (uint32_t)nb, to_mont(off), pt->tl, pt->th, (Fe*)db, order);
        HIPCHK(hipGetLastError());
    } else {
        o.in_limit = nb;
        SCCHK(ntt_device(d_b, (Fe*)db, logn, rt, false, o, st));
    }
    if (zero_flag) SCCHK(pointwise_div_enqueue((const Fe*)da, (const Fe*)db, (Fe*)dc, order, st, zero_flag));
    else SCCHK(pointwise_div_device((const Fe*)da, (const Fe*)db, (Fe*)dc, order, st));
    SCCHK(ntt_device((const Fe*)dc, (Fe*)da, logn, root_inverse(rt, order), true, NttOpts{}, st));
    Fe off_inv = from_mont(mont_inv(to_mont(off)));
    PowTables* pinv;
    SCCHK(get_pow(off_inv, order, st, &pinv));
    hipLaunchKernelGGL(scale_pow_kernel, dim3((unsigned)((order + 255) / 256)), dim3(256), 0, st, (const Fe*)da, (Fe*)db, order, pinv->lo, pinv->hi);
    HIPCHK(hipGetLastError());
    *full = (Fe*)db;
    return SC_OK;
}

static int coset_divide_args(uint64_t na, uint64_t nb, uint64_t n_out, const uint64_t offset[2], const uint64_t root[2], uint64_t order, Fe* rt, Fe* off) {
    if (!is_pow2(order) || order < 2) return fail(SC_ERR_NOT_POW2, "cannot compute ntt of non-power-of-two sequence");
    if (na > order || nb > order || n_out > order || na == 0 || nb == 0) return fail(SC_ERR_BAD_ARG, "operand longer than the transform order");
    *rt = fe_from(root); *off = fe_from(offset);
    SCCHK(check_root(*rt, order));
    if (fe_is_zero(*off) || fe_ge_p(*off)) return fail(SC_ERR_BAD_ARG, "bad coset offset");
    return SC_OK;
}

int sc_coset_divide(const void* a, uint64_t na, const void* b, uint64_t nb, const uint64_t offset[2], const uint64_t root[2], uint64_t order, void* out, uint64_t n_out) {
    std::lock_guard<std::mutex> lk(g_mu);
    SCCHK(ensure_init());
    Fe rt, off;
    SCCHK(coset_divide_args(na, nb, n_out, offset, root, order, &rt, &off));
    hipStream_t st = g.stream;
    void *ua, *ub;
    SCCHK(scratch(6, (na + nb) * sizeof(Fe), &ua));
    ub = (Fe*)ua + na;
    SCCHK(upload(ua, a, na * sizeof(Fe), st));
    SCCHK(upload(ub, b, nb * sizeof(Fe), st));
    Fe* full;
    SCCHK(coset_divide_core((const Fe*)ua, na, (const Fe*)ub, nb, off, rt, order, &full, st));
    return download(out, full, n_out * sizeof(Fe), st);
}

int sc_coset_divide_dev(const void* d_a, uint64_t na, const void* d_b, uint64_t nb, const uint64_t offset[2], const uint64_t root[2], uint64_t order,
                        void* d_out, uint64_t n_out, int* exact, void* stream) {
    std::lock_guard<std::mutex> lk(g_mu);
    SCCHK(ensure_init());
    Fe rt, off;
    SCCHK(coset_divide_args(na, nb, n_out, offset, root, order, &rt, &off));
    hipStream_t st = pick_stream(stream);
    Fe* full;
    SCCHK(coset_divide_core((const Fe*)d_a, na, (const Fe*)d_b, nb, off, rt, order, &full, st));
    if (n_out) HIPCHK(hipMemcpyAsync(d_out, full, n_out * sizeof(Fe), hipMemcpyDeviceToDevice, st));
    if (exact) {
        void* fl;
        SCCHK(scratch(7, 256, &fl));
        long long deg = -1;
        HIPCHK(hipMemsetAsync(fl, 0xFF, DEGREE_SLOTS * sizeof deg, st));
        if (order > n_out) {
            const uint64_t cnt = order - n_out;
            hipLaunchKernelGGL(vec_degree_kernel, dim3(degree_blocks(cnt)), dim3(256), 0, st, (const Fe*)full + n_out, cnt, (long long*)fl);
            HIPCHK(hipGetLastError());
        }
        SCCHK(degree_read(fl, st, &deg));
        *exact = deg < 0 ? 1 : 0;
    }
    return SC_OK;
}

int sc_coset_divide_later_dev(const void* d_a, uint64_t na, const void* d_b, uint64_t nb, const uint64_t offset[2], const uint64_t root[2], uint64_t order,
                              void* d_out, uint64_t n_out, sc_later_t** later, void* stream) {
    std::lock_guard<std::mutex> lk(g_mu);
    SCCHK(ensure_init());
    if (!later) return fail(SC_ERR_BAD_ARG, "null argument");
    Fe rt, off;
    SCCHK(coset_divide_args(na, nb, n_out, offset, root, order, &rt, &off));
    hipStream_t st = pick_stream(stream);
    const int slot = root_slot_get();
    if (slot < 0) return fail(SC_ERR_UNSUPPORTED, "no pinned slot free for a deferred check (nothing enqueued)");
    const int rc = [&]() -> int {
        uint32_t* zero_flag;
        long long* deg;
        SCCHK(later_words(slot, &zero_flag, &deg));
        Fe* full;
        SCCHK(coset_divide_core((const Fe*)d_a, na, (const Fe*)d_b, nb, off, rt, order, &full, st, zero_flag));
        if (n_out) HIPCHK(hipMemcpyAsync(d_out, full, n_out * sizeof(Fe), hipMemcpyDeviceToDevice, st));
        HIPCHK(hipMemsetAsync(deg, 0xFF, DEGREE_SLOTS * sizeof(long long), st));
        if (order > n_out) {
            const uint64_t cnt = order - n_out;
            hipLaunchKernelGGL(vec_degree_kernel, dim3(degree_blocks(cnt)), dim3(256), 0, st, (const Fe*)full + n_out, cnt, deg);
            HIPCHK(hipGetLastError());
        }
        return divide_flags_later(slot, zero_flag, deg, st, later);
    }();
    return rc == SC_OK ? SC_OK : later_abandon(slot, st, rc);
}
int sc_pointwise_div_later_dev(const void* d_a, const void* d_b, void* d_out, uint64_t n, sc_later_t** later, void* stream) {
    std::lock_guard<std::mutex> lk(g_mu);
    SCCHK(ensure_init());
    if (!later || !n) return fail(SC_ERR_BAD_ARG, "null argument");
    hipStream_t st = pick_stream(stream);
    const int slot = root_slot_get();
    if (slot < 0) return fail(SC_ERR_UNSUPPORTED, "no pinned slot free for a deferred check (nothing enqueued)");
    const int rc = [&]() -> int {
        uint32_t* zero_flag;
        long long* deg;
        SCCHK(later_words(slot, &zero_flag, &deg));
        SCCHK(pointwise_div_enqueue((const Fe*)d_a, (const Fe*)d_b, (Fe*)d_out, n, st, zero_flag));
        return divide_flags_later(slot, zero_flag, nullptr, st, later);
    }();
    return rc == SC_OK ? SC_OK : later_abandon(slot, st, rc);
}
int sc_later_wait(sc_later_t* later, int64_t words_out[8]) {
    std::lock_guard<std::mutex> lk(g_mu);
    if (!later || !words_out) return fail(SC_ERR_BAD_ARG, "null argument");
    SCCHK(ensure_init());
    return later_wait(later, (uint64_t*)words_out);
}

int sc_vec_degree_dev(const void* d_v, uint64_t n, int64_t* degree_out, void* stream) {
    std::lock_guard<std::mutex> lk(g_mu);
    SCCHK(ensure_init());
    hipStream_t st = pick_stream(stream);
    void* fl;
    SCCHK(scratch(7, 256, &fl));
    long long deg = -1;
    HIPCHK(hipMemsetAsync(fl, 0xFF, DEGREE_SLOTS * sizeof deg, st));
    const uint64_t top = n < (1ull << 16) ? n : (1ull << 16);
    if (top) {
        hipLaunchKernelGGL(vec_degree_kernel, dim3(degree_blocks(top)), dim3(256), 0, st, (const Fe*)d_v + (n - top), top, (long long*)fl);
        HIPCHK(hipGetLastError());
    }
    SCCHK(degree_read(fl, st, &deg));
    if (deg >= 0) deg += (long long)(n - top);
    else if (n > top) {
        hipLaunchKernelGGL(vec_degree_kernel, dim3(degree_blocks(n - top)), dim3(256), 0, st, (const Fe*)d_v, n - top, (long long*)fl);
        HIPCHK(hipGetLastError());
        SCCHK(degree_read(fl, st, &deg));
    }
    *degree_out = (int64_t)deg;
    return SC_OK;
}

constexpr uint64_t DEGREE_COLS_PER_LAUNCH = 4096;
int sc_vec_degree_columns_dev(const void* d_v, uint64_t n, uint64_t ld, uint64_t cols, int64_t* degrees_out, void* stream) {
    std::lock_guard<std::mutex> lk(g_mu);
    SCCHK(ensure_init());
    if (cols == 0) return SC_OK;
    if (!degrees_out || (n && !d_v) || ld < n) return fail(SC_ERR_BAD_ARG, n && ld < n ? "a column stride below the column length" : "null argument");
    hipStream_t st = pick_stream(stream);
    if (n == 0) {
        for (uint64_t c = 0; c < cols; ++c) degrees_out[c] = -1;
        return SC_OK;
    }
    void* fl;
    SCCHK(scratch(7, DEGREE_COLS_PER_LAUNCH * sizeof(long long), &fl));
    const uint64_t rows = (n + 256 * DEGREE_PER_THREAD - 1) / (256 * DEGREE_PER_THREAD);
    const uint32_t per_col = (uint32_t)(rows < 64 ? rows : 64);
    for (uint64_t done = 0; done < cols; done += DEGREE_COLS_PER_LAUNCH) {
        const uint64_t k = cols - done < DEGREE_COLS_PER_LAUNCH ? cols - done : DEGREE_COLS_PER_LAUNCH;
        const uint64_t words = (k + DEGREE_SLOTS - 1) / DEGREE_SLOTS * DEGREE_SLOTS;
        HIPCHK(hipMemsetAsync(fl, 0xFF, words * sizeof(long long), st));
        hipLaunchKernelGGL(vec_degree_cols_kernel, dim3((unsigned)(k * per_col)), dim3(256), 0, st, (const Fe*)d_v + done * ld, n, ld, per_col, (long long*)fl);
        HIPCHK(hipGetLastError());
        for (uint64_t w = 0; w < k; w += DEGREE_SLOTS) {
            long long slots[DEGREE_SLOTS];
            SCCHK(read_small_polled((const long long*)fl + w, sizeof slots, st, slots));
            for (uint64_t i = 0; i < DEGREE_SLOTS && w + i < k; ++i) degrees_out[done + w + i] = (int64_t)slots[i];
        }
    }
    return SC_OK;
}

int sc_mpoly_eval_dev(void* d_vals, uint64_t nvars, uint64_t n, const uint8_t* exps, const void* coefs, uint64_t nterms, void* d_out, void* stream) {
    return sc_mpoly_eval_ex_dev(d_vals, nvars, n, exps, coefs, nterms, d_out, 0, stream);
}
int sc_mpoly_eval_ex_dev(void* d_vals, uint64_t nvars, uint64_t n, const uint8_t* exps, const void* coefs, uint64_t nterms, void* d_out, int vals_converted, void* stream) {
    return sc_mpoly_eval_rot_dev(d_vals, nvars, n, exps, coefs, nterms, d_out, vals_converted, nullptr, nullptr, stream);
}
int sc_mpoly_eval_rot_dev(void* d_vals, uint64_t nvars, uint64_t n, const uint8_t* exps, const void* coefs, uint64_t nterms, void* d_out, int vals_converted,
                          const uint32_t* var_src, const uint64_t* var_rot, void* stream) {
    std::lock_guard<std::mutex> lk(g_mu);
    SCCHK(ensure_init());
    hipStream_t st = pick_stream(stream);
    if (!d_vals || !d_out || nvars == 0 || nvars > 255 || n == 0) return fail(SC_ERR_BAD_ARG, "bad argument");
    if ((var_src == nullptr) != (var_rot == nullptr)) return fail(SC_ERR_BAD_ARG, "var_src and var_rot come together");
    std::vector<uint64_t> where;
    if (var_src) {
        if (!is_pow2(n)) return fail(SC_ERR_NOT_POW2, "turned variables need a power-of-two domain");
        const uint8_t* e = exps;
        for (uint64_t j = 0; j < nvars; ++j) {
            const uint32_t s = var_src[j];
            if (s == SC_MPOLY_ABSENT) {
                for (uint64_t t = 0; t < nterms; ++t) if (e[t * nvars + j]) return fail(SC_ERR_BAD_ARG, "a term uses a variable that is marked absent");
                where.push_back(j); where.push_back(0);
                continue;
            }
            if (s >= nvars || var_src[s] != s || var_rot[s] != 0 || (s == j && var_rot[j] != 0)) return fail(SC_ERR_BAD_ARG, "a turned variable must point at one stored in its own place");
            where.push_back(s); where.push_back(var_rot[j] & (n - 1));
        }
    }
    const Fe* c = (const Fe*)coefs;
    std::vector<Fe> cm(nterms ? nterms : 1);
    for (uint64_t t = 0; t < nterms; ++t) {
        if (fe_ge_p(c[t])) return fail(SC_ERR_BAD_ARG, "coefficient is not a canonical residue");
        cm[t] = to_mont(c[t]);
    }
    const size_t cbytes = (cm.size() * sizeof(Fe) + 255) & ~255ull;
    const size_t ebytes = (nterms * nvars + 255) & ~255ull;
    void* buf;
    SCCHK(scratch(4, cbytes + ebytes + 16 * nvars + 256, &buf));
    uint64_t* d_where = where.empty() ? nullptr : (uint64_t*)((char*)buf + cbytes + ebytes);
    const bool small = upload_small(buf, cm.data(), cm.size() * sizeof(Fe), st) && (!nterms || upload_small((char*)buf + cbytes, exps, nterms * nvars, st)) &&
                       (!d_where || upload_small(d_where, where.data(), where.size() * 8, st));
    if (!small) {
        SCCHK(upload(buf, cm.data(), cm.size() * sizeof(Fe), st));
        if (nterms) SCCHK(upload((char*)buf + cbytes, exps, nterms * nvars, st));
        if (d_where) SCCHK(upload(d_where, where.data(), where.size() * 8, st));
    }
    if (!vals_converted) {
        if (!var_src) hipLaunchKernelGGL(to_mont_kernel, dim3((unsigned)((nvars * n + 255) / 256)), dim3(256), 0, st, (Fe*)d_vals, nvars * n);
        else
            for (uint64_t j = 0; j < nvars; ++j)
                if (var_src[j] == j) hipLaunchKernelGGL(to_mont_kernel, dim3((unsigned)((n + 255) / 256)), dim3(256), 0, st, (Fe*)d_vals + j * n, n);
    }
    hipLaunchKernelGGL(mpoly_eval_kernel, dim3((unsigned)((n + 255) / 256)), dim3(256), 0, st, (const Fe*)d_vals, (uint32_t)nvars, n,
                       (const uint8_t*)((char*)buf + cbytes), (const Fe*)buf, (uint32_t)nterms, (Fe*)d_out, (const uint64_t*)d_where);
    HIPCHK(hipGetLastError());
    if (!small || st != g.stream) HIPCHK(hipStreamSynchronize(st));
    return SC_OK;
}

}
```

### stark-anatomy_amd/csrc/field.cuh

```cuda
#pragma once
#include <stdint.h>

#if defined(__HIPCC__)
#define SC_HD __host__ __device__ __forceinline__
#else
#define SC_HD inline
#endif

namespace sc {

typedef unsigned __int128 u128;

struct alignas(16) Fe {
    uint64_t lo, hi;
};

static constexpr uint64_t P_LO = 1ull;
static constexpr uint64_t P_HI = 0xCB80000000000000ull;
static constexpr uint64_t R_LO = 0xFFFFFFFFFFFFFFFFull, R_HI = 0x347FFFFFFFFFFFFFull;
static constexpr uint64_t R2_LO = 0x5BD53A7F0E778236ull, R2_HI = 0xAAF4AD9A1A6AEDC2ull;

SC_HD Fe fe_zero() { return Fe{0, 0}; }
SC_HD Fe fe_one() { return Fe{1, 0}; }
SC_HD Fe fe_mont_one() { return Fe{R_LO, R_HI}; }
SC_HD bool fe_is_zero(Fe a) { return (a.lo | a.hi) == 0; }
SC_HD bool fe_eq(Fe a, Fe b) { return a.lo == b.lo && a.hi == b.hi; }
SC_HD bool fe_ge_p(Fe a) { return a.hi > P_HI || (a.hi == P_HI && a.lo >= P_LO); }

SC_HD Fe fe_add(Fe a, Fe b);
SC_HD Fe fe_sub(Fe a, Fe b);
SC_HD Fe mont_mul(Fe a, Fe b);

SC_HD Fe fe_add_c(Fe a, Fe b) {
    uint64_t lo = a.lo + b.lo;
    uint64_t c0 = lo < a.lo;
    uint64_t hi = a.hi + b.hi;
    uint64_t c1 = hi < a.hi;
    uint64_t hi2 = hi + c0;
    c1 |= (hi2 < hi);
    bool ge = c1 || hi2 > P_HI || (hi2 == P_HI && lo >= P_LO);
    uint64_t sl = ge ? P_LO : 0, sh = ge ? P_HI : 0;
    uint64_t rl = lo - sl;
    uint64_t br = lo < sl;
    return Fe{rl, hi2 - sh - br};
}

SC_HD Fe fe_sub_c(Fe a, Fe b) {
    uint64_t lo = a.lo - b.lo;
    uint64_t b0 = a.lo < b.lo;
    uint64_t hi = a.hi - b.hi;
    uint64_t b1 = a.hi < b.hi;
    uint64_t hi2 = hi - b0;
    b1 |= (hi < b0);
    uint64_t al = b1 ? P_LO : 0, ah = b1 ? P_HI : 0;
    uint64_t rl = lo + al;
    uint64_t c = rl < lo;
    return Fe{rl, hi2 + ah + c};
}

SC_HD Fe fe_neg(Fe a) { return fe_is_zero(a) ? a : fe_sub(Fe{P_LO, P_HI}, a); }

SC_HD Fe fe_half(Fe a) {
    if (a.lo & 1) {
        uint64_t lo = a.lo + P_LO;
        uint64_t c0 = lo < a.lo;
        uint64_t hi = a.hi + P_HI;
        uint64_t c1 = hi < a.hi;
        uint64_t hi2 = hi + c0;
        c1 |= (hi2 < hi);
        return Fe{(lo >> 1) | (hi2 << 63), (hi2 >> 1) | (c1 << 63)};
    }
    return Fe{(a.lo >> 1) | (a.hi << 63), a.hi >> 1};
}

SC_HD Fe mont_mul_c(Fe a, Fe b) {
    u128 p00 = (u128)a.lo * b.lo, p01 = (u128)a.lo * b.hi, p10 = (u128)a.hi * b.lo, p11 = (u128)a.hi * b.hi;
    uint64_t t0 = (uint64_t)p00;
    u128 mid = (p00 >> 64) + (uint64_t)p01 + (uint64_t)p10;
    uint64_t t1 = (uint64_t)mid;
    u128 hi = (mid >> 64) + (p01 >> 64) + (p10 >> 64) + (uint64_t)p11;
    uint64_t t2 = (uint64_t)hi;
    uint64_t t3 = (uint64_t)((hi >> 64) + (p11 >> 64));
    uint64_t m0 = 0 - t0;
    u128 x = (u128)m0 * P_HI + t1 + (uint64_t)(t0 != 0);
    uint64_t u1 = (uint64_t)x;
    u128 y = (x >> 64) + t2;
    uint64_t u2 = (uint64_t)y;
    uint64_t u3 = t3 + (uint64_t)(y >> 64);
    uint64_t c3 = u3 < t3;
    uint64_t m1 = 0 - u1;
    u128 x2 = (u128)m1 * P_HI + u2 + (uint64_t)(u1 != 0);
    uint64_t v2 = (uint64_t)x2;
    u128 y2 = (x2 >> 64) + u3;
    uint64_t v3 = (uint64_t)y2;
    uint64_t c4 = c3 + (uint64_t)(y2 >> 64);
    bool ge = c4 || v3 > P_HI || (v3 == P_HI && v2 >= P_LO);
    uint64_t sl = ge ? P_LO : 0, sh = ge ? P_HI : 0;
    uint64_t rl = v2 - sl;
    uint64_t br = v2 < sl;
    return Fe{rl, v3 - sh - br};
}

typedef uint64_t rare_t;
static constexpr uint32_t P_TOP32 = (uint32_t)(P_HI >> 32);

SC_HD Fe fe_fixup_fast_c(uint64_t lo, uint64_t hi, bool neg, rare_t& rare) {
    const uint32_t d0 = (uint32_t)lo, d3 = (uint32_t)(hi >> 32);
    const uint32_t o0 = d0 + (neg ? 1u : 0u);
    rare |= (neg && o0 == 0) ? 1u : 0u;
    const uint32_t o3 = neg ? d3 + P_TOP32 : d3;
    return Fe{(lo & 0xFFFFFFFF00000000ull) | o0, (hi & 0xFFFFFFFFull) | ((uint64_t)o3 << 32)};
}
SC_HD Fe fe_sub_fast_c(Fe a, Fe b, rare_t& rare) {
    const uint64_t lo = a.lo - b.lo;
    const uint64_t b0 = a.lo < b.lo;
    const uint64_t hi = a.hi - b.hi;
    const bool neg = (a.hi < b.hi) || (hi < b0);
    return fe_fixup_fast_c(lo, hi - b0, neg, rare);
}
SC_HD Fe fe_add_fast_c(Fe a, Fe b, rare_t& rare) {
    const uint64_t lo = a.lo + b.lo;
    const uint64_t c0 = lo < a.lo;
    const uint64_t hi = a.hi + b.hi;
    const uint64_t hi2 = hi + c0;
    const bool ca = (hi < a.hi) || (hi2 < hi);
    const uint32_t r0 = (uint32_t)lo, r3 = (uint32_t)(hi2 >> 32);
    const bool sel = ca || r3 >= P_TOP32;
    const uint32_t o0 = r0 - (sel ? 1u : 0u);
    rare |= (sel && r0 == 0) ? 1u : 0u;
    const uint32_t o3 = sel ? r3 - P_TOP32 : r3;
    return Fe{(lo & 0xFFFFFFFF00000000ull) | o0, (hi2 & 0xFFFFFFFFull) | ((uint64_t)o3 << 32)};
}
SC_HD Fe mont_mul_fast_c(Fe a, Fe b, rare_t& rare) {
    u128 p00 = (u128)a.lo * b.lo, p01 = (u128)a.lo * b.hi, p10 = (u128)a.hi * b.lo, p11 = (u128)a.hi * b.hi;
    const uint64_t t0 = (uint64_t)p00;
    u128 mid = (p00 >> 64) + (uint64_t)p01 + (uint64_t)p10;
    const uint64_t t1 = (uint64_t)mid;
    u128 top = (mid >> 64) + (p01 >> 64) + (p10 >> 64) + p11;
    const uint32_t w0 = (uint32_t)t0, w1 = (uint32_t)(t0 >> 32), w2 = (uint32_t)t1, w3 = (uint32_t)(t1 >> 32);
    const uint64_t PH = P_TOP32;
    const uint64_t s0 = (uint64_t)w0 * PH;
    const uint32_t m3 = w3 - (uint32_t)s0;
    const uint64_t delta = w3 < (uint32_t)s0;
    const uint64_t s1 = (uint64_t)w1 * PH + (s0 >> 32);
    const uint64_t s2 = (uint64_t)w2 * PH + (s1 >> 32);
    const uint64_t s3 = (uint64_t)m3 * PH + (s2 >> 32);
    const u128 q = (u128)(uint32_t)s1 | ((u128)(uint32_t)s2 << 32) | ((u128)s3 << 64);
    const u128 d = top - q;
    const bool neg = top < q || d < delta;
    const u128 r = d - delta;
    return fe_fixup_fast_c((uint64_t)r, (uint64_t)(r >> 64), neg, rare);
}

SC_HD Fe to_mont(Fe a) { return mont_mul(a, Fe{R2_LO, R2_HI}); }
SC_HD Fe from_mont(Fe a) { return mont_mul(a, fe_one()); }
SC_HD Fe fe_mul(Fe a, Fe b) { return mont_mul(mont_mul(a, b), Fe{R2_LO, R2_HI}); }

SC_HD Fe mont_pow(Fe base_m, uint64_t e) {
    Fe acc = fe_mont_one();
    while (e) {
        if (e & 1) acc = mont_mul(acc, base_m);
        base_m = mont_mul(base_m, base_m);
        e >>= 1;
    }
    return acc;
}

SC_HD Fe mont_pow128(Fe base_m, uint64_t e_lo, uint64_t e_hi) {
    Fe acc = fe_mont_one();
    for (int i = 0; i < 64; ++i) {
        if ((e_lo >> i) & 1) acc = mont_mul(acc, base_m);
        base_m = mont_mul(base_m, base_m);
    }
    for (int i = 0; i < 64 && (e_hi >> i); ++i) {
        if ((e_hi >> i) & 1) acc = mont_mul(acc, base_m);
        base_m = mont_mul(base_m, base_m);
    }
    return acc;
}

SC_HD Fe mont_sqr_n(Fe v, int n) {
    for (int i = 0; i < n; ++i) v = mont_mul(v, v);
    return v;
}
SC_HD Fe mont_inv(Fe x) {
#if !defined(__HIP_DEVICE_COMPILE__)
    return mont_pow128(x, 0xFFFFFFFFFFFFFFFFull, P_HI - 1);
#else
    const Fe x2 = mont_mul(mont_sqr_n(x, 1), x);
    const Fe x3 = mont_mul(mont_sqr_n(x2, 1), x);
    const Fe x6 = mont_mul(mont_sqr_n(x3, 3), x3);
    const Fe x7 = mont_mul(mont_sqr_n(x6, 1), x);
    const Fe x14 = mont_mul(mont_sqr_n(x7, 7), x7);
    const Fe x28 = mont_mul(mont_sqr_n(x14, 14), x14);
    const Fe x29 = mont_mul(mont_sqr_n(x28, 1), x);
    const Fe x58 = mont_mul(mont_sqr_n(x29, 29), x29);
    const Fe x59 = mont_mul(mont_sqr_n(x58, 1), x);
    const Fe x118 = mont_mul(mont_sqr_n(x59, 59), x59);
    const Fe y = mont_mul(mont_sqr_n(x118, 1), x);
    const Fe z = mont_mul(y, x);
    Fe w = mont_mul(mont_sqr_n(z, 1), z);
    w = mont_mul(mont_sqr_n(w, 3), z);
    w = mont_mul(mont_sqr_n(w, 2), z);
    w = mont_mul(mont_sqr_n(w, 1), z);
    w = mont_sqr_n(w, 1);
    return mont_mul(w, y);
#endif
}

}

#ifndef SC_ASM_MUL
#define SC_ASM_MUL 1
#endif
#ifndef SC_ASM_ADDSUB
#define SC_ASM_ADDSUB 1
#endif
#include "field_asm.cuh"

namespace sc {
SC_HD Fe mont_mul(Fe a, Fe b) {
#if defined(__HIP_DEVICE_COMPILE__) && SC_ASM_MUL
    return mont_mul_asm(a, b);
#else
    return mont_mul_c(a, b);
#endif
}
#ifndef SC_MUL2
#define SC_MUL2 1
#endif
SC_HD void mont_mul2(Fe a0, Fe b0, Fe a1, Fe b1, Fe& r0, Fe& r1) {
#if defined(__HIP_DEVICE_COMPILE__) && SC_ASM_MUL && SC_MUL2
    mont_mul2_asm(a0, b0, a1, b1, r0, r1);
#else
    r0 = mont_mul(a0, b0);
    r1 = mont_mul(a1, b1);
#endif
}
SC_HD void fe_addsub2(Fe u0, Fe v0, Fe u1, Fe v1, Fe& s0, Fe& d0, Fe& s1, Fe& d1) {
#if defined(__HIP_DEVICE_COMPILE__) && SC_ASM_ADDSUB && SC_MUL2
    fe_addsub2_asm(u0, v0, u1, v1, s0, d0, s1, d1);
#else
    s0 = fe_add(u0, v0); d0 = fe_sub(u0, v0);
    s1 = fe_add(u1, v1); d1 = fe_sub(u1, v1);
#endif
}
SC_HD Fe fe_add(Fe a, Fe b) {
#if defined(__HIP_DEVICE_COMPILE__) && SC_ASM_ADDSUB
    return fe_add_asm(a, b);
#else
    return fe_add_c(a, b);
#endif
}
SC_HD Fe fe_sub(Fe a, Fe b) {
#if defined(__HIP_DEVICE_COMPILE__) && SC_ASM_ADDSUB
    return fe_sub_asm(a, b);
#else
    return fe_sub_c(a, b);
#endif
}
SC_HD bool rare_any(rare_t rare) {
#if defined(__HIP_DEVICE_COMPILE__)
    return rare_any_asm(rare);
#else
    return rare != 0;
#endif
}
SC_HD Fe fe_add_fast(Fe a, Fe b, rare_t& rare) {
#if defined(__HIP_DEVICE_COMPILE__) && SC_ASM_ADDSUB
    return fe_add_fast_asm(a, b, rare);
#else
    return fe_add_fast_c(a, b, rare);
#endif
}
SC_HD Fe fe_sub_fast(Fe a, Fe b, rare_t& rare) {
#if defined(__HIP_DEVICE_COMPILE__) && SC_ASM_ADDSUB
    return fe_sub_fast_asm(a, b, rare);
#else
    return fe_sub_fast_c(a, b, rare);
#endif
}
SC_HD Fe mont_mul_fast(Fe a, Fe b, rare_t& rare) {
#if defined(__HIP_DEVICE_COMPILE__) && SC_ASM_MUL
    return mont_mul_fast_asm(a, b, rare);
#else
    return mont_mul_fast_c(a, b, rare);
#endif
}
SC_HD void mont_mul2_fast(Fe a0, Fe b0, Fe a1, Fe b1, Fe& r0, Fe& r1, rare_t& rare) {
#if defined(__HIP_DEVICE_COMPILE__) && SC_ASM_MUL && SC_MUL2
    mont_mul2_fast_asm(a0, b0, a1, b1, r0, r1, rare);
#else
    r0 = mont_mul_fast(a0, b0, rare);
    r1 = mont_mul_fast(a1, b1, rare);
#endif
}
SC_HD void fe_addsub2_fast(Fe u0, Fe v0, Fe u1, Fe v1, Fe& s0, Fe& d0, Fe& s1, Fe& d1, rare_t& rare) {
#if defined(__HIP_DEVICE_COMPILE__) && SC_ASM_ADDSUB && SC_MUL2
    fe_addsub2_fast_asm(u0, v0, u1, v1, s0, d0, s1, d1, rare);
#else
    s0 = fe_add_fast(u0, v0, rare); d0 = fe_sub_fast(u0, v0, rare);
    s1 = fe_add_fast(u1, v1, rare); d1 = fe_sub_fast(u1, v1, rare);
#endif
}

SC_HD Fe fe_sample_bytes(const uint8_t* b, uint32_t width) {
    uint64_t w0 = 0, w1 = 0, w2 = 0, w3 = 0;
    for (uint32_t k = 0; k < width; ++k) {
        const uint32_t pos = width - 1 - k;
        const uint64_t v = (uint64_t)b[k] << (8 * (pos & 7));
        const uint32_t word = pos >> 3;
        w0 |= word == 0 ? v : 0;
        w1 |= word == 1 ? v : 0;
        w2 |= word == 2 ? v : 0;
        w3 |= word == 3 ? v : 0;
    }
    Fe lo{w0, w1}, hi{w2, w3};
    if (fe_ge_p(lo)) lo = fe_sub(lo, Fe{P_LO, P_HI});
    if (fe_ge_p(hi)) hi = fe_sub(hi, Fe{P_LO, P_HI});
    return fe_add(lo, to_mont(hi));
}
}
```

### stark-anatomy_amd/csrc/field_asm.cuh

```cuda
#pragma once

#if defined(__HIP_DEVICE_COMPILE__)
namespace sc {

typedef uint64_t smask_t;

#ifndef SC_HAZ_NOP
#define SC_HAZ_NOP "s_nop 1\n\t"
#endif

__device__ __forceinline__ uint64_t a_mad(uint32_t a, uint32_t b, uint64_t c) {
    uint64_t d; smask_t cy;
    asm("v_mad_u64_u32 %0, %1, %2, %3, %4" : "=v"(d), "=s"(cy) : "v"(a), "v"(b), "v"(c));
    return d;
}
__device__ __forceinline__ uint64_t a_madc(uint32_t a, uint32_t b, uint64_t c, smask_t& cy) {
    uint64_t d;
    asm("v_mad_u64_u32 %0, %1, %2, %3, %4" : "=v"(d), "=s"(cy) : "v"(a), "v"(b), "v"(c));
    return d;
}
__device__ __forceinline__ uint32_t a_add_co(uint32_t x, uint32_t y, smask_t& co) {
    uint32_t s;
    asm("v_add_co_u32_e64 %0, %1, %2, %3" : "=v"(s), "=s"(co) : "v"(x), "v"(y));
    return s;
}
__device__ __forceinline__ uint32_t a_addc(uint32_t x, uint32_t y, smask_t ci, smask_t& co) {
    uint32_t s;
    asm(SC_HAZ_NOP "v_addc_co_u32_e64 %0, %1, %2, %3, %4" : "=v"(s), "=s"(co) : "v"(x), "v"(y), "s"(ci));
    return s;
}
__device__ __forceinline__ uint32_t a_addc_last(uint32_t x, uint32_t y, smask_t ci) {
    uint32_t s; smask_t co;
    asm(SC_HAZ_NOP "v_addc_co_u32_e64 %0, %1, %2, %3, %4" : "=v"(s), "=s"(co) : "v"(x), "v"(y), "s"(ci));
    return s;
}
__device__ __forceinline__ uint32_t a_inc(uint32_t x, smask_t ci) {
    uint32_t s; smask_t co;
    asm(SC_HAZ_NOP "v_addc_co_u32_e64 %0, %1, 0, %2, %3" : "=v"(s), "=s"(co) : "v"(x), "s"(ci));
    return s;
}
__device__ __forceinline__ uint32_t a_sub_co(uint32_t x, uint32_t y, smask_t& bo) {
    uint32_t s;
    asm("v_sub_co_u32_e64 %0, %1, %2, %3" : "=v"(s), "=s"(bo) : "v"(x), "v"(y));
    return s;
}
__device__ __forceinline__ uint32_t a_subb(uint32_t x, uint32_t y, smask_t bi, smask_t& bo) {
    uint32_t s;
    asm(SC_HAZ_NOP "v_subb_co_u32_e64 %0, %1, %2, %3, %4" : "=v"(s), "=s"(bo) : "v"(x), "v"(y), "s"(bi));
    return s;
}
__device__ __forceinline__ uint32_t a_negb(uint32_t y, smask_t bi, smask_t& bo) {
    uint32_t s;
    asm(SC_HAZ_NOP "v_subb_co_u32_e64 %0, %1, 0, %2, %3" : "=v"(s), "=s"(bo) : "v"(y), "s"(bi));
    return s;
}
__device__ __forceinline__ uint32_t a_cnd(uint32_t a, uint32_t b, smask_t sel) {
    uint32_t r;
    asm(SC_HAZ_NOP "v_cndmask_b32_e64 %0, %1, %2, %3" : "=v"(r) : "v"(a), "v"(b), "s"(sel));
    return r;
}

__device__ __forceinline__ void rare_or(smask_t& rare, smask_t c) { asm volatile("s_or_b64 %0, %0, %1" : "+s"(rare) : "s"(c) : "scc"); }
__device__ __forceinline__ bool rare_any_asm(smask_t rare) {
    uint32_t any;
    asm("s_cmp_lg_u64 %1, 0\n\ts_cselect_b32 %0, 1, 0" : "=s"(any) : "s"(rare) : "scc");
    return __builtin_amdgcn_readfirstlane(any) != 0;
}

__device__ __forceinline__ uint32_t lo32(uint64_t x) { return (uint32_t)x; }
__device__ __forceinline__ uint32_t hi32(uint64_t x) { return (uint32_t)(x >> 32); }

static constexpr uint32_t PH3 = 0xCB800000u;

__device__ __forceinline__ Fe a_cond_sub_p(uint32_t r0, uint32_t r1, uint32_t r2, uint32_t r3, smask_t cf) {
    smask_t b;
    uint32_t d0 = a_sub_co(r0, 1u, b);
    uint32_t d1 = a_subb(r1, 0u, b, b);
    uint32_t d2 = a_subb(r2, 0u, b, b);
    uint32_t d3 = a_subb(r3, PH3, b, b);
    smask_t sel = cf | ~b;
    uint32_t o0 = a_cnd(r0, d0, sel), o1 = a_cnd(r1, d1, sel), o2 = a_cnd(r2, d2, sel), o3 = a_cnd(r3, d3, sel);
    return Fe{((uint64_t)o1 << 32) | o0, ((uint64_t)o3 << 32) | o2};
}

__device__ __forceinline__ Fe a_fixup_fast(uint32_t d0, uint32_t d1, uint32_t d2, uint32_t d3, smask_t bw, smask_t& rare) {
    smask_t c;
    const uint32_t d3p = d3 + PH3;
    uint32_t o0 = a_addc(d0, 0u, bw, c);
    uint32_t o3 = a_cnd(d3, d3p, bw);
    rare_or(rare, c);
    return Fe{((uint64_t)d1 << 32) | o0, ((uint64_t)o3 << 32) | d2};
}

template <bool FAST>
__device__ __forceinline__ Fe mont_mul_core(Fe a, Fe b, smask_t& rare) {
    const uint32_t a0 = lo32(a.lo), a1 = hi32(a.lo), a2 = lo32(a.hi), a3 = hi32(a.hi);
    const uint32_t b0 = lo32(b.lo), b1 = hi32(b.lo), b2 = lo32(b.hi), b3 = hi32(b.hi);
    smask_t c;
    uint64_t E0 = a_mad(a0, b0, 0);
    uint64_t O0 = a_mad(a0, b1, 0);
    O0 = a_madc(a1, b0, O0, c);
    uint32_t nO0 = a_inc(0u, c);
    uint64_t E1 = a_mad(a0, b2, 0);
    E1 = a_madc(a1, b1, E1, c);
    uint32_t nE1 = a_inc(0u, c);
    E1 = a_madc(a2, b0, E1, c);
    nE1 = a_inc(nE1, c);
    uint64_t O1 = a_mad(a0, b3, (uint64_t)nO0);
    O1 = a_madc(a1, b2, O1, c);
    uint32_t nO1 = a_inc(0u, c);
    O1 = a_madc(a2, b1, O1, c);
    nO1 = a_inc(nO1, c);
    O1 = a_madc(a3, b0, O1, c);
    nO1 = a_inc(nO1, c);
    uint64_t E2 = a_mad(a1, b3, (uint64_t)nE1);
    E2 = a_madc(a2, b2, E2, c);
    uint32_t nE2 = a_inc(0u, c);
    E2 = a_madc(a3, b1, E2, c);
    nE2 = a_inc(nE2, c);
    uint64_t O2 = a_mad(a2, b3, (uint64_t)nO1);
    O2 = a_madc(a3, b2, O2, c);
    uint32_t nO2 = a_inc(0u, c);
    uint64_t E3 = a_mad(a3, b3, (uint64_t)nE2);
    const uint32_t t0 = lo32(E0);
    uint32_t t1 = a_add_co(hi32(E0), lo32(O0), c);
    uint32_t t2 = a_addc(lo32(E1), hi32(O0), c, c);
    uint32_t t3 = a_addc(hi32(E1), lo32(O1), c, c);
    uint32_t t4 = a_addc(lo32(E2), hi32(O1), c, c);
    uint32_t t5 = a_addc(hi32(E2), lo32(O2), c, c);
    uint32_t t6 = a_addc(lo32(E3), hi32(O2), c, c);
    uint32_t t7 = a_addc_last(hi32(E3), nO2, c);
    const uint32_t PHc = PH3;
    uint64_t s0 = a_mad(t0, PHc, 0);
    smask_t bw;
    uint32_t m3 = a_sub_co(t3, lo32(s0), bw);
    uint64_t s1 = a_mad(t1, PHc, (uint64_t)hi32(s0));
    uint64_t s2 = a_mad(t2, PHc, (uint64_t)hi32(s1));
    uint64_t s3 = a_mad(m3, PHc, (uint64_t)hi32(s2));
    uint32_t r0 = a_subb(t4, lo32(s1), bw, bw);
    uint32_t r1 = a_subb(t5, lo32(s2), bw, bw);
    uint32_t r2 = a_subb(t6, lo32(s3), bw, bw);
    uint32_t r3 = a_subb(t7, hi32(s3), bw, bw);
    if constexpr (FAST) return a_fixup_fast(r0, r1, r2, r3, bw, rare);
    uint32_t ph = a_cnd(0u, PH3, bw);
    uint32_t o0 = a_addc(r0, 0u, bw, c);
    uint32_t o1 = a_addc(r1, 0u, c, c);
    uint32_t o2 = a_addc(r2, 0u, c, c);
    uint32_t o3 = a_addc_last(r3, ph, c);
    return Fe{((uint64_t)o1 << 32) | o0, ((uint64_t)o3 << 32) | o2};
}
__device__ __forceinline__ Fe mont_mul_asm(Fe a, Fe b) {
    smask_t none = 0;
    return mont_mul_core<false>(a, b, none);
}
__device__ __forceinline__ Fe mont_mul_fast_asm(Fe a, Fe b, smask_t& rare) { return mont_mul_core<true>(a, b, rare); }

#define SC_V_MAD(d, cy, x, y, c)   asm volatile("v_mad_u64_u32 %0, %1, %2, %3, %4" : "=v"(d), "=s"(cy) : "v"(x), "v"(y), "v"(c))
#define SC_V_INC(d, x, ci, co)     asm volatile("v_addc_co_u32_e64 %0, %1, 0, %2, %3" : "=v"(d), "=s"(co) : "v"(x), "s"(ci))
#define SC_V_ADDCO(d, co, x, y)    asm volatile("v_add_co_u32_e64 %0, %1, %2, %3" : "=v"(d), "=s"(co) : "v"(x), "v"(y))
#define SC_V_ADDC(d, co, x, y, ci) asm volatile("v_addc_co_u32_e64 %0, %1, %2, %3, %4" : "=v"(d), "=s"(co) : "v"(x), "v"(y), "s"(ci))
#define SC_V_SUBCO(d, bo, x, y)    asm volatile("v_sub_co_u32_e64 %0, %1, %2, %3" : "=v"(d), "=s"(bo) : "v"(x), "v"(y))
#define SC_V_SUBB(d, bo, x, y, bi) asm volatile("v_subb_co_u32_e64 %0, %1, %2, %3, %4" : "=v"(d), "=s"(bo) : "v"(x), "v"(y), "s"(bi))
#define SC_V_CND(d, x, y, m)       asm volatile("v_cndmask_b32_e64 %0, %1, %2, %3" : "=v"(d) : "v"(x), "v"(y), "s"(m))
#define SC_V_NOP0()                asm volatile("s_nop 0")

template <int W> __device__ __forceinline__ void v_mad_dump(uint64_t& d, uint32_t x, uint32_t y, uint64_t c) {
    if constexpr (W == 0) asm volatile("v_mad_u64_u32 %0, vcc, %1, %2, %3" : "=v"(d) : "v"(x), "v"(y), "v"(c) : "vcc");
    else asm volatile("v_mad_u64_u32 %0, s[100:101], %1, %2, %3" : "=v"(d) : "v"(x), "v"(y), "v"(c) : "s100", "s101");
}
template <int W> __device__ __forceinline__ void v_inc_dump(uint32_t& d, uint32_t x, smask_t ci) {
    if constexpr (W == 0) asm volatile("v_addc_co_u32_e64 %0, vcc, %1, 0, %2" : "=v"(d) : "v"(x), "s"(ci) : "vcc");
    else asm volatile("v_addc_co_u32_e64 %0, s[100:101], %1, 0, %2" : "=v"(d) : "v"(x), "s"(ci) : "s100", "s101");
}
template <int W> __device__ __forceinline__ void v_addc_dump(uint32_t& d, uint32_t x, uint32_t y, smask_t ci) {
    if constexpr (W == 0) asm volatile("v_addc_co_u32_e64 %0, vcc, %1, %2, %3" : "=v"(d) : "v"(x), "v"(y), "s"(ci) : "vcc");
    else asm volatile("v_addc_co_u32_e64 %0, s[100:101], %1, %2, %3" : "=v"(d) : "v"(x), "v"(y), "s"(ci) : "s100", "s101");
}
#define SC_V_MADD(d, x, y, c)      v_mad_dump<W>(d, x, y, c)
#define SC_V_INCD(d, x, ci)        v_inc_dump<W>(d, x, ci)
#define SC_V_ADDCD(d, x, y, ci)    v_addc_dump<W>(d, x, y, ci)

struct MulState {
    uint32_t a0, a1, a2, a3, b0, b1, b2, b3;
    uint64_t E0, O0, E1, O1, E2, O2, E3, s0, s1, s2, s3;
    uint32_t nO0, nE1, nO1, nE2, nO2, t1, t2, t3, t4, t5, t6, t7, m3, r0, r1, r2, r3, ph, o0, o1, o2, o3;
    smask_t c1, c2, c3, c4, c5, c6, c7, c8, c9, ct, bw, cx;
};

template <bool FAST>
__device__ __forceinline__ void mont_mul2_core(Fe xa, Fe wa, Fe xb, Fe wb, Fe& ra, Fe& rb, smask_t& rare) {
    MulState A, B;
    A.a0 = lo32(xa.lo); A.a1 = hi32(xa.lo); A.a2 = lo32(xa.hi); A.a3 = hi32(xa.hi);
    A.b0 = lo32(wa.lo); A.b1 = hi32(wa.lo); A.b2 = lo32(wa.hi); A.b3 = hi32(wa.hi);
    B.a0 = lo32(xb.lo); B.a1 = hi32(xb.lo); B.a2 = lo32(xb.hi); B.a3 = hi32(xb.hi);
    B.b0 = lo32(wb.lo); B.b1 = hi32(wb.lo); B.b2 = lo32(wb.hi); B.b3 = hi32(wb.hi);
    const uint64_t zero64 = 0;
    const uint32_t zero32 = 0, PHc = PH3;
#define SC_BOTH(STEP) { MulState& M = A; [[maybe_unused]] constexpr int W = 0; STEP } { MulState& M = B; [[maybe_unused]] constexpr int W = 1; STEP }
    SC_BOTH(SC_V_MADD(M.E0, M.a0, M.b0, zero64);)
    SC_BOTH(SC_V_MADD(M.O0, M.a0, M.b1, zero64);)
    SC_BOTH(SC_V_MADD(M.E1, M.a0, M.b2, zero64);)
    SC_BOTH(SC_V_MAD(M.O0, M.c1, M.a1, M.b0, M.O0);)
    SC_BOTH(SC_V_MAD(M.E1, M.c2, M.a1, M.b1, M.E1);)
    SC_BOTH(SC_V_MAD(M.E1, M.c3, M.a2, M.b0, M.E1);)
    SC_BOTH(SC_V_INCD(M.nO0, zero32, M.c1);)
    SC_BOTH(SC_V_INCD(M.nE1, zero32, M.c2);)
    SC_BOTH(SC_V_INCD(M.nE1, M.nE1, M.c3);)
    SC_BOTH(SC_V_MADD(M.O1, M.a0, M.b3, (uint64_t)M.nO0 | ((uint64_t)M.nE1 << 32));)
    SC_BOTH(SC_V_MAD(M.O1, M.c4, M.a1, M.b2, M.O1);)
    SC_BOTH(SC_V_MAD(M.O1, M.c5, M.a2, M.b1, M.O1);)
    SC_BOTH(SC_V_INCD(M.nO1, zero32, M.c4);)
    SC_BOTH(SC_V_MAD(M.O1, M.c6, M.a3, M.b0, M.O1);)
    SC_BOTH(SC_V_MADD(M.E2, M.a1, M.b3, zero64);)
    SC_BOTH(SC_V_INCD(M.nO1, M.nO1, M.c5);)
    SC_BOTH(SC_V_MAD(M.E2, M.c7, M.a2, M.b2, M.E2);)
    SC_BOTH(SC_V_INCD(M.nO1, M.nO1, M.c6);)
    SC_BOTH(SC_V_MAD(M.E2, M.c8, M.a3, M.b1, M.E2);)
    SC_BOTH(SC_V_INCD(M.nE2, zero32, M.c7);)
    SC_BOTH(SC_V_MADD(M.E3, M.a3, M.b3, zero64);)
    SC_BOTH(SC_V_INCD(M.nE2, M.nE2, M.c8);)
    SC_BOTH(SC_V_MADD(M.O2, M.a2, M.b3, (uint64_t)M.nO1 | ((uint64_t)M.nE2 << 32));)
    SC_BOTH(SC_V_MAD(M.O2, M.c9, M.a3, M.b2, M.O2);)
    SC_BOTH(SC_V_ADDCO(M.t1, M.ct, hi32(M.E0), lo32(M.O0));)
    SC_BOTH(SC_V_MADD(M.s0, lo32(M.E0), PHc, zero64);)
    SC_BOTH(SC_V_INCD(M.nO2, zero32, M.c9);)
    SC_BOTH(SC_V_ADDC(M.t2, M.ct, lo32(M.E1), hi32(M.O0), M.ct);)
    SC_BOTH(SC_V_MADD(M.s1, M.t1, PHc, (uint64_t)hi32(M.s0));)
    SC_BOTH(SC_V_ADDC(M.t3, M.ct, hi32(M.E1), lo32(M.O1), M.ct);)
    SC_BOTH(SC_V_MADD(M.s2, M.t2, PHc, (uint64_t)hi32(M.s1));)
    SC_BOTH(SC_V_SUBCO(M.m3, M.bw, M.t3, lo32(M.s0));)
    SC_BOTH(SC_V_ADDC(M.t4, M.ct, lo32(M.E2), hi32(M.O1), M.ct);)
    SC_BOTH(SC_V_MADD(M.s3, M.m3, PHc, (uint64_t)hi32(M.s2));)
    SC_BOTH(SC_V_ADDC(M.t5, M.ct, hi32(M.E2), lo32(M.O2), M.ct);)
    SC_BOTH(SC_V_SUBB(M.r0, M.bw, M.t4, lo32(M.s1), M.bw);)
    SC_BOTH(SC_V_ADDC(M.t6, M.ct, lo32(M.E3), hi32(M.O2), M.ct);)
    SC_BOTH(SC_V_SUBB(M.r1, M.bw, M.t5, lo32(M.s2), M.bw);)
    SC_BOTH(SC_V_ADDC(M.t7, M.cx, hi32(M.E3), M.nO2, M.ct);)
    SC_BOTH(SC_V_SUBB(M.r2, M.bw, M.t6, lo32(M.s3), M.bw);)
    SC_V_NOP0();
    SC_BOTH(SC_V_SUBB(M.r3, M.bw, M.t7, hi32(M.s3), M.bw);)
    SC_V_NOP0();
    if constexpr (FAST) {
        A.ph = A.r3 + PHc;
        B.ph = B.r3 + PHc;
        SC_BOTH(SC_V_ADDC(M.o0, M.cx, M.r0, zero32, M.bw);)
        SC_BOTH(SC_V_CND(M.o3, M.r3, M.ph, M.bw);)
        rare_or(rare, A.cx);
        rare_or(rare, B.cx);
        ra = Fe{((uint64_t)A.r1 << 32) | A.o0, ((uint64_t)A.o3 << 32) | A.r2};
        rb = Fe{((uint64_t)B.r1 << 32) | B.o0, ((uint64_t)B.o3 << 32) | B.r2};
        return;
    }
    SC_BOTH(SC_V_CND(M.ph, zero32, PHc, M.bw);)
    SC_BOTH(SC_V_ADDC(M.o0, M.cx, M.r0, zero32, M.bw);)
    SC_V_NOP0();
    SC_BOTH(SC_V_ADDC(M.o1, M.cx, M.r1, zero32, M.cx);)
    SC_V_NOP0();
    SC_BOTH(SC_V_ADDC(M.o2, M.cx, M.r2, zero32, M.cx);)
    SC_V_NOP0();
    SC_BOTH(SC_V_ADDCD(M.o3, M.r3, M.ph, M.cx);)
#undef SC_BOTH
    ra = Fe{((uint64_t)A.o1 << 32) | A.o0, ((uint64_t)A.o3 << 32) | A.o2};
    rb = Fe{((uint64_t)B.o1 << 32) | B.o0, ((uint64_t)B.o3 << 32) | B.o2};
}
__device__ __forceinline__ void mont_mul2_asm(Fe xa, Fe wa, Fe xb, Fe wb, Fe& ra, Fe& rb) {
    smask_t none = 0;
    mont_mul2_core<false>(xa, wa, xb, wb, ra, rb, none);
}
__device__ __forceinline__ void mont_mul2_fast_asm(Fe xa, Fe wa, Fe xb, Fe wb, Fe& ra, Fe& rb, smask_t& rare) {
    mont_mul2_core<true>(xa, wa, xb, wb, ra, rb, rare);
}

struct AddSubState {
    uint32_t u0, u1, u2, u3, v0, v1, v2, v3;
    uint32_t r0, r1, r2, r3, t0, t1, t2, t3, d0, d1, d2, d3, ph, e0, e1, e2, e3, s0, s1, s2, s3;
    smask_t ca, cb, bd, ce, sel;
};

__device__ __forceinline__ void fe_addsub2_asm(Fe ua, Fe va, Fe ub, Fe vb, Fe& sa, Fe& da, Fe& sb, Fe& db) {
    AddSubState A, B;
    A.u0 = lo32(ua.lo); A.u1 = hi32(ua.lo); A.u2 = lo32(ua.hi); A.u3 = hi32(ua.hi);
    A.v0 = lo32(va.lo); A.v1 = hi32(va.lo); A.v2 = lo32(va.hi); A.v3 = hi32(va.hi);
    B.u0 = lo32(ub.lo); B.u1 = hi32(ub.lo); B.u2 = lo32(ub.hi); B.u3 = hi32(ub.hi);
    B.v0 = lo32(vb.lo); B.v1 = hi32(vb.lo); B.v2 = lo32(vb.hi); B.v3 = hi32(vb.hi);
    const uint32_t zero32 = 0, one32 = 1, PHc = PH3;
#define SC_BOTH(STEP) { AddSubState& M = A; [[maybe_unused]] constexpr int W = 0; STEP } { AddSubState& M = B; [[maybe_unused]] constexpr int W = 1; STEP }
    SC_BOTH(SC_V_ADDCO(M.r0, M.ca, M.u0, M.v0); SC_V_SUBCO(M.d0, M.bd, M.u0, M.v0);)
    SC_BOTH(SC_V_ADDC(M.r1, M.ca, M.u1, M.v1, M.ca); SC_V_SUBB(M.d1, M.bd, M.u1, M.v1, M.bd);)
    SC_BOTH(SC_V_ADDC(M.r2, M.ca, M.u2, M.v2, M.ca); SC_V_SUBB(M.d2, M.bd, M.u2, M.v2, M.bd);)
    SC_BOTH(SC_V_ADDC(M.r3, M.ca, M.u3, M.v3, M.ca); SC_V_SUBB(M.d3, M.bd, M.u3, M.v3, M.bd);)
    SC_BOTH(SC_V_SUBCO(M.t0, M.cb, M.r0, one32); SC_V_CND(M.ph, zero32, PHc, M.bd);)
    SC_BOTH(SC_V_SUBB(M.t1, M.cb, M.r1, zero32, M.cb); SC_V_ADDC(M.e0, M.ce, M.d0, zero32, M.bd);)
    SC_BOTH(SC_V_SUBB(M.t2, M.cb, M.r2, zero32, M.cb); SC_V_ADDC(M.e1, M.ce, M.d1, zero32, M.ce);)
    SC_BOTH(SC_V_SUBB(M.t3, M.cb, M.r3, PHc, M.cb); SC_V_ADDC(M.e2, M.ce, M.d2, zero32, M.ce);)
    A.sel = A.ca | ~A.cb;
    B.sel = B.ca | ~B.cb;
    SC_BOTH(SC_V_CND(M.s0, M.r0, M.t0, M.sel); SC_V_ADDCD(M.e3, M.d3, M.ph, M.ce);)
    SC_BOTH(SC_V_CND(M.s1, M.r1, M.t1, M.sel);)
    SC_BOTH(SC_V_CND(M.s2, M.r2, M.t2, M.sel);)
    SC_BOTH(SC_V_CND(M.s3, M.r3, M.t3, M.sel);)
#undef SC_BOTH
    sa = Fe{((uint64_t)A.s1 << 32) | A.s0, ((uint64_t)A.s3 << 32) | A.s2};
    da = Fe{((uint64_t)A.e1 << 32) | A.e0, ((uint64_t)A.e3 << 32) | A.e2};
    sb = Fe{((uint64_t)B.s1 << 32) | B.s0, ((uint64_t)B.s3 << 32) | B.s2};
    db = Fe{((uint64_t)B.e1 << 32) | B.e0, ((uint64_t)B.e3 << 32) | B.e2};
}

__device__ __forceinline__ Fe fe_add_asm(Fe a, Fe b) {
    smask_t c;
    uint32_t r0 = a_add_co(lo32(a.lo), lo32(b.lo), c);
    uint32_t r1 = a_addc(hi32(a.lo), hi32(b.lo), c, c);
    uint32_t r2 = a_addc(lo32(a.hi), lo32(b.hi), c, c);
    uint32_t r3 = a_addc(hi32(a.hi), hi32(b.hi), c, c);
    return a_cond_sub_p(r0, r1, r2, r3, c);
}

__device__ __forceinline__ Fe fe_sub_asm(Fe a, Fe b) {
    smask_t bw;
    uint32_t d0 = a_sub_co(lo32(a.lo), lo32(b.lo), bw);
    uint32_t d1 = a_subb(hi32(a.lo), hi32(b.lo), bw, bw);
    uint32_t d2 = a_subb(lo32(a.hi), lo32(b.hi), bw, bw);
    uint32_t d3 = a_subb(hi32(a.hi), hi32(b.hi), bw, bw);
    smask_t c;
    uint32_t ph = a_cnd(0u, PH3, bw);
    uint32_t o0 = a_addc(d0, 0u, bw, c);
    uint32_t o1 = a_addc(d1, 0u, c, c);
    uint32_t o2 = a_addc(d2, 0u, c, c);
    uint32_t o3 = a_addc_last(d3, ph, c);
    return Fe{((uint64_t)o1 << 32) | o0, ((uint64_t)o3 << 32) | o2};
}

__device__ __forceinline__ Fe fe_sub_fast_asm(Fe a, Fe b, smask_t& rare) {
    smask_t bw;
    uint32_t d0 = a_sub_co(lo32(a.lo), lo32(b.lo), bw);
    uint32_t d1 = a_subb(hi32(a.lo), hi32(b.lo), bw, bw);
    uint32_t d2 = a_subb(lo32(a.hi), lo32(b.hi), bw, bw);
    uint32_t d3 = a_subb(hi32(a.hi), hi32(b.hi), bw, bw);
    return a_fixup_fast(d0, d1, d2, d3, bw, rare);
}

__device__ __forceinline__ Fe fe_add_fast_asm(Fe a, Fe b, smask_t& rare) {
    smask_t ca, cb, bo;
    uint32_t r0 = a_add_co(lo32(a.lo), lo32(b.lo), ca);
    uint32_t r1 = a_addc(hi32(a.lo), hi32(b.lo), ca, ca);
    uint32_t r2 = a_addc(lo32(a.hi), lo32(b.hi), ca, ca);
    uint32_t r3 = a_addc(hi32(a.hi), hi32(b.hi), ca, ca);
    uint32_t t3 = a_sub_co(r3, PH3, cb);
    const smask_t sel = ca | ~cb;
    uint32_t o0 = a_subb(r0, 0u, sel, bo);
    uint32_t o3 = a_cnd(r3, t3, sel);
    rare_or(rare, bo);
    return Fe{((uint64_t)r1 << 32) | o0, ((uint64_t)o3 << 32) | r2};
}

__device__ __forceinline__ void fe_addsub2_fast_asm(Fe ua, Fe va, Fe ub, Fe vb, Fe& sa, Fe& da, Fe& sb, Fe& db, smask_t& rare) {
    AddSubState A, B;
    A.u0 = lo32(ua.lo); A.u1 = hi32(ua.lo); A.u2 = lo32(ua.hi); A.u3 = hi32(ua.hi);
    A.v0 = lo32(va.lo); A.v1 = hi32(va.lo); A.v2 = lo32(va.hi); A.v3 = hi32(va.hi);
    B.u0 = lo32(ub.lo); B.u1 = hi32(ub.lo); B.u2 = lo32(ub.hi); B.u3 = hi32(ub.hi);
    B.v0 = lo32(vb.lo); B.v1 = hi32(vb.lo); B.v2 = lo32(vb.hi); B.v3 = hi32(vb.hi);
    const uint32_t zero32 = 0, PHc = PH3;
#define SC_BOTH(STEP) { AddSubState& M = A; STEP } { AddSubState& M = B; STEP }
    SC_BOTH(SC_V_ADDCO(M.r0, M.ca, M.u0, M.v0); SC_V_SUBCO(M.d0, M.bd, M.u0, M.v0);)
    SC_BOTH(SC_V_ADDC(M.r1, M.ca, M.u1, M.v1, M.ca); SC_V_SUBB(M.d1, M.bd, M.u1, M.v1, M.bd);)
    SC_BOTH(SC_V_ADDC(M.r2, M.ca, M.u2, M.v2, M.ca); SC_V_SUBB(M.d2, M.bd, M.u2, M.v2, M.bd);)
    SC_BOTH(SC_V_ADDC(M.r3, M.ca, M.u3, M.v3, M.ca); SC_V_SUBB(M.d3, M.bd, M.u3, M.v3, M.bd);)
    SC_BOTH(SC_V_SUBCO(M.t3, M.cb, M.r3, PHc);)
    A.ph = A.d3 + PHc;
    B.ph = B.d3 + PHc;
    SC_BOTH(SC_V_ADDC(M.e0, M.ce, M.d0, zero32, M.bd);)
    SC_BOTH(SC_V_CND(M.e3, M.d3, M.ph, M.bd);)
    A.sel = A.ca | ~A.cb;
    B.sel = B.ca | ~B.cb;
    SC_BOTH(SC_V_SUBB(M.s0, M.cb, M.r0, zero32, M.sel);)
    SC_BOTH(SC_V_CND(M.s3, M.r3, M.t3, M.sel);)
#undef SC_BOTH
    rare_or(rare, A.ce);
    rare_or(rare, B.ce);
    rare_or(rare, A.cb);
    rare_or(rare, B.cb);
    sa = Fe{((uint64_t)A.r1 << 32) | A.s0, ((uint64_t)A.s3 << 32) | A.r2};
    da = Fe{((uint64_t)A.d1 << 32) | A.e0, ((uint64_t)A.e3 << 32) | A.d2};
    sb = Fe{((uint64_t)B.r1 << 32) | B.s0, ((uint64_t)B.s3 << 32) | B.r2};
    db = Fe{((uint64_t)B.d1 << 32) | B.e0, ((uint64_t)B.e3 << 32) | B.d2};
}

}
#endif
```

### stark-anatomy_amd/csrc/ntt_tile.cuh

```cuda
#pragma once
#include "field.cuh"

namespace sc {

#ifndef SC_MAX_BLOCKS
#define SC_MAX_BLOCKS 16
#endif

struct PassParams {
    const Fe* in;
    Fe* out;
    int logR, logC;
    int lo_log, mid_log;
    uint64_t in_hi, in_mid, in_lo, in_rs, in_cs;
    int in_split;
    uint64_t in_rs_hi;
    uint64_t out_hi, out_mid, out_lo, out_rs, out_cs;
    int rfast_load;
    const Fe* mt;
    int mt_shift;
    int tw_enable;
    int tw_col_shift;
    uint64_t tw_scale;
    uint64_t tw_col_base, tw_row_k, tw_row_mid;
    const Fe* tl;
    const Fe* th;
    const Fe* twd;
    uint64_t twd_stride;
    const Fe* twd_in;
    uint64_t twd_in_mask;
    int scale_enable;
    Fe scale;
    uint64_t in_limit;
    int coset_enable;
    const Fe* ol;
    const Fe* oh;
    int prune_log;
    int prio_balance;
    int blk_enable;
    int blk_log;
    uint32_t blk_row_k, blk_row_mid;
    Fe* out_blk[SC_MAX_BLOCKS];
    int col_enable;
    int col_tiles_log;
    uint64_t col_stride, col_stride_in;
    unsigned long long* trace;
};

SC_HD uint32_t bitrev32(uint32_t x, int bits) {
#if defined(__HIP_DEVICE_COMPILE__)
    return bits ? (__brev(x) >> (32 - bits)) : 0u;
#else
    uint32_t r = 0;
    for (int i = 0; i < bits; ++i) r |= ((x >> i) & 1u) << (bits - 1 - i);
    return r;
#endif
}

SC_HD uint32_t lds_index(uint32_t r, uint32_t c, int logC) {
    uint32_t cm = (1u << logC) - 1u;
    return (r << logC) | ((c ^ r) & cm);
}

#ifndef SC_TWD_NT
#define SC_TWD_NT 0
#endif
SC_HD Fe load_stream(const Fe* p) {
#if defined(__HIP_DEVICE_COMPILE__) && SC_TWD_NT
    typedef unsigned long long sc_u64x2 __attribute__((ext_vector_type(2)));
    const sc_u64x2 v = __builtin_nontemporal_load(reinterpret_cast<const sc_u64x2*>(p));
    return Fe{v.x, v.y};
#else
    return *p;
#endif
}

SC_HD Fe pow2level(const Fe* lo, const Fe* hi, uint64_t e) {
    Fe a = lo[e & 4095u];
    Fe b = hi[e >> 12];
    return mont_mul(a, b);
}

SC_HD Fe pow_table_entry(Fe base_m, uint64_t i, uint64_t step, Fe scale_m) {
    return mont_mul(mont_pow(base_m, i * step), scale_m);
}

template <int LOGE, int S, int GLR = -1, int GLC = -1>
struct Round {
    static constexpr int E = 1 << LOGE;
    static constexpr int F = 1 << S;
    static constexpr int G = E >> S;
    uint32_t rr[G];
    uint32_t cc[G];
    uint32_t t_lo, t_mid, t_hi;
    uint64_t col_off, col_off_in;
    int logR, logC;
    bool rfast;

    SC_HD void setup(const PassParams& P, bool first, uint32_t tile, uint32_t tid) {
        logR = (GLR >= 0) ? GLR : P.logR;
        logC = (GLC >= 0) ? GLC : P.logC;
        const uint32_t T = 1u << (logR + logC - LOGE);
        col_off = col_off_in = 0;
        if (P.col_enable) {
            col_off = (uint64_t)(tile >> P.col_tiles_log) * P.col_stride;
            col_off_in = (uint64_t)(tile >> P.col_tiles_log) * P.col_stride_in;
            tile &= (1u << P.col_tiles_log) - 1u;
        }
        t_lo = tile & ((1u << P.lo_log) - 1u);
        t_mid = (tile >> P.lo_log) & ((1u << P.mid_log) - 1u);
        t_hi = tile >> (P.lo_log + P.mid_log);
#pragma unroll
        for (int g = 0; g < G; ++g) {
            uint32_t rem = (uint32_t)g * T + tid;
            uint32_t rrem, c;
            if (first && P.rfast_load) {
                rrem = rem & ((1u << (logR - S)) - 1u);
                c = rem >> (logR - S);
            } else {
                c = rem & ((1u << logC) - 1u);
                rrem = rem >> logC;
            }
            rr[g] = rrem;
            cc[g] = c;
        }
        if constexpr (SPLIT_ADDR) rfast = first && P.rfast_load;
    }
    struct Uc { uint32_t rrem, c; };
    SC_HD Uc split(uint32_t rem) const {
        const uint32_t rs = logR - S;
        return Uc{rfast ? (rem & ((1u << rs) - 1u)) : (rem >> logC), rfast ? (rem >> rs) : (rem & ((1u << logC) - 1u))};
    }
    SC_HD static uint32_t row_of(uint32_t rrem, uint32_t fi, int sh) {
        return ((rrem >> sh) << (sh + S)) | (fi << sh) | (rrem & ((1u << sh) - 1u));
    }
    SC_HD uint32_t row(int i, int sh) const { return row_of(rr[i >> S], (uint32_t)(i & (F - 1)), sh); }

    static constexpr bool SPLIT_ADDR = GLR >= 0 && GLC >= 0 && LOGE == 3;
    SC_HD Uc group_part(int g) const { return split((uint32_t)g * (1u << (logR + logC - LOGE))); }
    template <class T> SC_HD static T sgpr_pin(T v) {
#if defined(__HIP_DEVICE_COMPILE__)
        asm("" : "+s"(v));
#endif
        return v;
    }
#if defined(__HIP_DEVICE_COMPILE__)
    typedef __attribute__((address_space(1))) char gchar;
    typedef __attribute__((address_space(1))) Fe gfe;
    SC_HD static uint32_t vgpr_pin(uint32_t v) { asm("" : "+v"(v)); return v; }
    SC_HD static Fe load_at(const Fe* base, uint32_t lane_bytes) {
        return *reinterpret_cast<const gfe*>(reinterpret_cast<const gchar*>(sgpr_pin(reinterpret_cast<uint64_t>(base))) + vgpr_pin(lane_bytes));
    }
    SC_HD static void store_at(Fe* base, uint32_t lane_bytes, Fe v) {
        *reinterpret_cast<gfe*>(reinterpret_cast<gchar*>(sgpr_pin(reinterpret_cast<uint64_t>(base))) + vgpr_pin(lane_bytes)) = v;
    }
    SC_HD static void store_word_at(uint32_t* base, uint32_t lane_bytes, uint32_t v) {
        typedef __attribute__((address_space(1))) uint32_t gword;
        *reinterpret_cast<gword*>(reinterpret_cast<gchar*>(sgpr_pin(reinterpret_cast<uint64_t>(base))) + vgpr_pin(lane_bytes)) = v;
    }
#else
    static void store_word_at(uint32_t* base, uint32_t lane_bytes, uint32_t v) { *reinterpret_cast<uint32_t*>(reinterpret_cast<char*>(base) + lane_bytes) = v; }
    static Fe load_at(const Fe* base, uint32_t lane_bytes) { return *reinterpret_cast<const Fe*>(reinterpret_cast<const char*>(base) + lane_bytes); }
    static void store_at(Fe* base, uint32_t lane_bytes, Fe v) { *reinterpret_cast<Fe*>(reinterpret_cast<char*>(base) + lane_bytes) = v; }
#endif
    SC_HD uint64_t in_index(const PassParams& P, int i, int sh) const {
        const uint32_t r = row(i, sh), c = cc[i >> S];
        uint64_t j = (uint64_t)t_hi * P.in_hi + (uint64_t)t_mid * P.in_mid + (uint64_t)t_lo * P.in_lo + (uint64_t)c * P.in_cs;
        if (P.in_split) j += (uint64_t)(r & ((1u << P.in_split) - 1u)) * P.in_rs + (uint64_t)(r >> P.in_split) * P.in_rs_hi;
        else j += (uint64_t)r * P.in_rs;
        return j;
    }
    SC_HD void gather_global(const PassParams& P, int sh, Fe* x, Fe* tin) const {
        if constexpr (SPLIT_ADDR) {
            if (!P.in_split) {
                if (P.in_limit == ~0ull) gather_split<false>(P, sh, x, tin);
                else gather_split<true>(P, sh, x, tin);
                return;
            }
        }
#pragma unroll
        for (int i = 0; i < E; ++i) {
            const uint64_t j = in_index(P, i, sh);
            Fe v = fe_zero();
            if (j < P.in_limit) v = P.in[col_off_in + j];
            x[i] = v;
            if (P.twd_in) tin[i] = P.twd_in[j & P.twd_in_mask];
        }
    }
    template <bool LIMIT>
    SC_HD void gather_split(const PassParams& P, int sh, Fe* x, Fe* tin) const {
        const uint64_t tile_j = (uint64_t)t_hi * P.in_hi + (uint64_t)t_mid * P.in_mid + (uint64_t)t_lo * P.in_lo;
        const uint32_t lane = row_of(rr[0], 0, sh) * (uint32_t)P.in_rs + cc[0] * (uint32_t)P.in_cs;
        const Fe* src = P.in + col_off_in;
#pragma unroll
        for (int i = 0; i < E; ++i) {
            const Uc u = group_part(i >> S);
            const uint64_t ju = tile_j + (uint64_t)row_of(u.rrem, (uint32_t)(i & (F - 1)), sh) * P.in_rs + (uint64_t)u.c * P.in_cs;
            if constexpr (LIMIT) {
                const uint64_t room = P.in_limit > ju ? P.in_limit - ju : 0;
                const uint32_t room32 = sgpr_pin(room > 0xffffffffull ? 0xffffffffu : (uint32_t)room);
                x[i] = lane < room32 ? load_at(src + ju, lane << 4) : fe_zero();
            } else {
                x[i] = load_at(src + ju, lane << 4);
            }
            if (P.twd_in) tin[i] = P.twd_in[(ju + lane) & P.twd_in_mask];
        }
    }
    template <bool FAST = false>
    SC_HD void finish_global(const PassParams& P, int sh, Fe* x, const Fe* tin, rare_t* rare = nullptr) const {
        if (!FAST && P.coset_enable) {
#pragma unroll
            for (int i = 0; i < E; ++i) {
                const uint64_t j = in_index(P, i, sh);
                if (j < P.in_limit) x[i] = mont_mul(x[i], pow2level(P.ol, P.oh, j));
            }
        }
        if (P.twd_in) {
#pragma unroll
            for (int i = 0; i + 1 < E; i += 2) mul2<FAST>(x[i], tin[i], x[i + 1], tin[i + 1], x[i], x[i + 1], rare);
            if (E & 1) x[E - 1] = mul1<FAST>(x[E - 1], tin[E - 1], rare);
        }
    }
    template <bool FAST> SC_HD static Fe mul1(Fe a, Fe b, rare_t* rare) {
        if constexpr (FAST) return mont_mul_fast(a, b, *rare);
        else return mont_mul(a, b);
    }
    template <bool FAST> SC_HD static void mul2(Fe a0, Fe b0, Fe a1, Fe b1, Fe& r0, Fe& r1, rare_t* rare) {
        if constexpr (FAST) mont_mul2_fast(a0, b0, a1, b1, r0, r1, *rare);
        else mont_mul2(a0, b0, a1, b1, r0, r1);
    }
    SC_HD void gather_lds(int sh, Fe* x, const Fe* lds) const {
#pragma unroll
        for (int i = 0; i < E; ++i) x[i] = lds[lds_index(row(i, sh), cc[i >> S], logC)];
    }
    template <bool FAST = false>
    SC_HD void butterflies(int sh, Fe* x, const Fe* tw, int tw_shift, int prune_log = 0, int last_hint = -1, int prio = 0, rare_t* rare = nullptr) const {
        const bool last = last_hint < 0 ? (sh == 0) : (last_hint != 0);
        set_prio(prio, 3);
#pragma unroll
        for (int q = 0; q < S; ++q) {
            const int bit = S - 1 - q;
            const int b = sh + bit;
            const int tau = logR - 1 - b;
            if (!FAST && tau < prune_log) {
                const uint32_t nz = 1u << (logR - prune_log);
#pragma unroll
                for (int i0 = 0; i0 < E; ++i0) {
                    if (i0 & (1 << bit)) continue;
                    const int i1 = i0 | (1 << bit);
                    const int g = i0 >> S;
                    const uint32_t fi_low = (uint32_t)(i0 & (F - 1)) & ((1u << bit) - 1u);
                    const Fe u = x[i0];
                    Fe d = fe_zero();
                    if ((row(i0, sh) & ((2u << b) - 1u)) < nz) {
                        if (last && (bit == 0 || fi_low == 0)) {
                            d = u;
                        } else {
                            const uint32_t row_lo = rr[g] & ((1u << sh) - 1u);
                            const uint32_t e = ((fi_low << sh) | row_lo) << tau;
                            d = mont_mul(u, tw[(uint64_t)e << tw_shift]);
                        }
                    }
                    x[i1] = d;
                }
                continue;
            }
            Fe dd[E / 2];
            uint32_t ee[E / 2];
            bool triv[E / 2];
#pragma unroll
            for (int bf = 0; bf < E / 2; bf += 2) {
                const int i0 = ((bf >> bit) << (bit + 1)) | (bf & ((1 << bit) - 1));
                const int i1 = i0 | (1 << bit);
                if (bf + 1 < E / 2) {
                    const int j0 = (((bf + 1) >> bit) << (bit + 1)) | ((bf + 1) & ((1 << bit) - 1));
                    const int j1 = j0 | (1 << bit);
                    if constexpr (FAST) fe_addsub2_fast(x[i0], x[i1], x[j0], x[j1], x[i0], dd[bf], x[j0], dd[bf + 1], *rare);
                    else fe_addsub2(x[i0], x[i1], x[j0], x[j1], x[i0], dd[bf], x[j0], dd[bf + 1]);
                } else {
                    Fe u = x[i0], v = x[i1];
                    if constexpr (FAST) {
                        x[i0] = fe_add_fast(u, v, *rare);
                        dd[bf] = fe_sub_fast(u, v, *rare);
                    } else {
                        x[i0] = fe_add(u, v);
                        dd[bf] = fe_sub(u, v);
                    }
                }
            }
#pragma unroll
            for (int bf = 0; bf < E / 2; ++bf) {
                const int i0 = ((bf >> bit) << (bit + 1)) | (bf & ((1 << bit) - 1));
                const int g = i0 >> S;
                const uint32_t fi_low = (uint32_t)(i0 & (F - 1)) & ((1u << bit) - 1u);
                triv[bf] = last && (bit == 0 || fi_low == 0);
                const uint32_t row_lo = rr[g] & ((1u << sh) - 1u);
                ee[bf] = ((fi_low << sh) | row_lo) << tau;
                if (q == 0 && bf == 0) set_prio(prio, 2);
                if (q == S - 1 && bf == 0) set_prio(prio, 1);
            }
#pragma unroll
            for (int bf = 0; bf < E / 2; bf += 2) {
                const int ia = (((bf >> bit) << (bit + 1)) | (bf & ((1 << bit) - 1))) | (1 << bit);
                if (bf + 1 < E / 2) {
                    const int ib = ((((bf + 1) >> bit) << (bit + 1)) | ((bf + 1) & ((1 << bit) - 1))) | (1 << bit);
                    if (!triv[bf] && !triv[bf + 1]) {
                        mul2<FAST>(dd[bf], tw[(uint64_t)ee[bf] << tw_shift], dd[bf + 1], tw[(uint64_t)ee[bf + 1] << tw_shift], x[ia], x[ib], rare);
                    } else {
                        x[ia] = triv[bf] ? dd[bf] : mul1<FAST>(dd[bf], tw[(uint64_t)ee[bf] << tw_shift], rare);
                        x[ib] = triv[bf + 1] ? dd[bf + 1] : mul1<FAST>(dd[bf + 1], tw[(uint64_t)ee[bf + 1] << tw_shift], rare);
                    }
                } else {
                    x[ia] = triv[bf] ? dd[bf] : mul1<FAST>(dd[bf], tw[(uint64_t)ee[bf] << tw_shift], rare);
                }
            }
            if (q == S - 1) set_prio(prio, 0);
        }
    }
    SC_HD static void set_prio(int enable, int level) {
#if defined(__HIP_DEVICE_COMPILE__)
        if (enable) {
            switch (level) {
                case 3: __builtin_amdgcn_s_setprio(3); break;
                case 2: __builtin_amdgcn_s_setprio(2); break;
                case 1: __builtin_amdgcn_s_setprio(1); break;
                default: __builtin_amdgcn_s_setprio(0); break;
            }
        }
#endif
    }
    SC_HD void scatter_lds(int sh, const Fe* x, Fe* lds) const {
#pragma unroll
        for (int i = 0; i < E; ++i) lds[lds_index(row(i, sh), cc[i >> S], logC)] = x[i];
    }
    SC_HD void load_twd(const PassParams& P, Fe* t) const {
        if constexpr (SPLIT_ADDR) {
            const uint32_t lane = bitrev32(row_of(rr[0], 0, 0), logR) * (uint32_t)(P.tw_row_k * P.twd_stride) + (cc[0] >> P.tw_col_shift);
#pragma unroll
            for (int i = 0; i < E; ++i) {
                const Uc u = group_part(i >> S);
                const uint32_t k = bitrev32(row_of(u.rrem, (uint32_t)(i & (F - 1)), 0), logR);
                const uint64_t colidx = ((((uint64_t)t_lo << logC) | u.c) >> P.tw_col_shift) + P.tw_col_base;
                const uint64_t ju = ((uint64_t)k * P.tw_row_k + (uint64_t)t_mid * P.tw_row_mid) * P.twd_stride + colidx;
#if SC_TWD_NT
                t[i] = load_stream(P.twd + ju + lane);
#else
                t[i] = load_at(P.twd + ju, lane << 4);
#endif
            }
            return;
        }
#pragma unroll
        for (int i = 0; i < E; ++i) {
            const uint32_t k = bitrev32(row(i, 0), logR);
            const uint64_t colidx = ((((uint64_t)t_lo << logC) | cc[i >> S]) >> P.tw_col_shift) + P.tw_col_base;
            t[i] = load_stream(&P.twd[((uint64_t)k * P.tw_row_k + (uint64_t)t_mid * P.tw_row_mid) * P.twd_stride + colidx]);
        }
    }
    SC_HD void scatter_global(const PassParams& P, const Fe* x) const {
        Fe none[E];
        if (P.blk_enable) scatter_global<true>(P, x, none, false);
        else scatter_global<false>(P, x, none, false);
    }
    template <bool ALT, bool FAST = false>
    SC_HD void scatter_global(const PassParams& P, const Fe* x, const Fe (&twd_prefetched)[E], bool have_prefetched, rare_t* rare = nullptr) const {
        Fe v[E];
#pragma unroll
        for (int i = 0; i < E; ++i) v[i] = x[i];
        if (P.tw_enable) {
            Fe t[E];
            if (P.twd) {
                if (have_prefetched) {
#pragma unroll
                    for (int i = 0; i < E; ++i) t[i] = twd_prefetched[i];
                } else {
                    load_twd(P, t);
                }
            } else {
                Fe a[E], b[E];
#pragma unroll
                for (int i = 0; i < E; ++i) {
                    const uint32_t k = bitrev32(row(i, 0), logR);
                    const uint64_t colidx = ((((uint64_t)t_lo << logC) | cc[i >> S]) >> P.tw_col_shift) + P.tw_col_base;
                    const uint64_t e = colidx * ((uint64_t)k * P.tw_row_k + (uint64_t)t_mid * P.tw_row_mid) * P.tw_scale;
                    a[i] = P.tl[e & 4095u];
                    b[i] = P.th[e >> 12];
                }
#pragma unroll
                for (int i = 0; i + 1 < E; i += 2) mont_mul2(a[i], b[i], a[i + 1], b[i + 1], t[i], t[i + 1]);
                if (E & 1) t[E - 1] = mont_mul(a[E - 1], b[E - 1]);
            }
#pragma unroll
            for (int i = 0; i + 1 < E; i += 2) mul2<FAST>(v[i], t[i], v[i + 1], t[i + 1], v[i], v[i + 1], rare);
            if (E & 1) v[E - 1] = mul1<FAST>(v[E - 1], t[E - 1], rare);
        }
        if (P.scale_enable) {
#pragma unroll
            for (int i = 0; i < E; ++i) v[i] = mul1<FAST>(v[i], P.scale, rare);
        }
        if constexpr (SPLIT_ADDR && !ALT) {
            const uint64_t tile_j = (uint64_t)t_hi * P.out_hi + (uint64_t)t_mid * P.out_mid + (uint64_t)t_lo * P.out_lo;
            const uint32_t lane = bitrev32(row_of(rr[0], 0, 0), logR) * (uint32_t)P.out_rs + cc[0] * (uint32_t)P.out_cs;
            Fe* dst = P.out + col_off;
#pragma unroll
            for (int i = 0; i < E; ++i) {
                const Uc u = group_part(i >> S);
                const uint32_t k = bitrev32(row_of(u.rrem, (uint32_t)(i & (F - 1)), 0), logR);
                const uint64_t ju = tile_j + (uint64_t)k * P.out_rs + (uint64_t)u.c * P.out_cs;
                store_at(dst + ju, lane << 4, v[i]);
            }
            return;
        }
#pragma unroll
        for (int i = 0; i < E; ++i) {
            const uint32_t k = bitrev32(row(i, 0), logR), c = cc[i >> S];
            uint64_t j = (uint64_t)t_hi * P.out_hi + (uint64_t)t_mid * P.out_mid + (uint64_t)t_lo * P.out_lo + (uint64_t)k * P.out_rs + (uint64_t)c * P.out_cs;
            if constexpr (ALT) {
                const uint32_t nat = k * P.blk_row_k + t_mid * P.blk_row_mid;
                Fe* dst = P.out_blk[nat >> P.blk_log];
                dst[col_off + j] = v[i];
            } else {
                P.out[col_off + j] = v[i];
            }
        }
    }
};

template <int LOGE, int S, int GLR = -1, int GLC = -1, bool FAST = false>
SC_HD void ntt_round(const PassParams& P, int sh, bool first, uint32_t tile, uint32_t tid, Fe* lds, const Fe* tw, rare_t* rare = nullptr) {
    constexpr int E = 1 << LOGE;
    Round<LOGE, S, GLR, GLC> R;
    R.setup(P, first, tile, tid);
    Fe x[E];
    if (first) {
        Fe tin[E];
        R.gather_global(P, sh, x, tin);
        R.template finish_global<FAST>(P, sh, x, tin, rare);
    } else {
        R.gather_lds(sh, x, lds);
    }
    R.template butterflies<FAST>(sh, x, tw, 0, P.prune_log, -1, P.prio_balance, rare);
    if (sh == 0) {
        Fe none[E];
        if (P.blk_enable) R.template scatter_global<true, FAST>(P, x, none, false, rare);
        else R.template scatter_global<false, FAST>(P, x, none, false, rare);
    } else {
        R.scatter_lds(sh, x, lds);
    }
}

template <int LOGE, int GLR = -1, int GLC = -1>
SC_HD void ntt_round_dispatch(const PassParams& P, int s, int sh, bool first, uint32_t tile, uint32_t tid, Fe* lds, const Fe* tw) {
    if constexpr (LOGE >= 4) { if (s == 4) { ntt_round<LOGE, 4, GLR, GLC>(P, sh, first, tile, tid, lds, tw); return; } }
    if constexpr (LOGE >= 3) { if (s == 3) { ntt_round<LOGE, 3, GLR, GLC>(P, sh, first, tile, tid, lds, tw); return; } }
    if constexpr (LOGE >= 2) { if (s == 2) { ntt_round<LOGE, 2, GLR, GLC>(P, sh, first, tile, tid, lds, tw); return; } }
    ntt_round<LOGE, 1, GLR, GLC>(P, sh, first, tile, tid, lds, tw);
}

SC_HD void tile_twiddles_to_lds(const PassParams& P, int logR, uint32_t tid, uint32_t nthreads, Fe* tw) {
    const uint32_t count = logR > 0 ? (1u << (logR - 1)) : 0u;
    for (uint32_t i = tid; i < count; i += nthreads) tw[i] = P.mt[(uint64_t)i << P.mt_shift];
}

#define SC_FIXED4_SHAPES(X) X(8, 3) X(7, 4) X(10, 2) X(6, 5) X(9, 3) X(8, 4)
#define SC_FIXED8_SHAPES(X) X(10, 2) X(9, 3) X(8, 4)
template <int LOGE, int GLR, int GLC, int ROUND = 0, bool ALT = false, bool FAST = false>
struct FixedRounds {
    static constexpr int E = 1 << LOGE;
    static constexpr int NR = (GLR + LOGE - 1) / LOGE;
    static constexpr int S = (ROUND == 0) ? (GLR - LOGE * (NR - 1)) : LOGE;
    static constexpr int DONE = (ROUND == 0) ? 0 : (GLR - LOGE * (NR - 1)) + LOGE * (ROUND - 1);
    static constexpr int SH = GLR - DONE - S;
    static constexpr bool NEXT_WAVE_LOCAL = (ROUND >= 1) && (SH + GLC <= 6);
    static constexpr uint32_t TW_COUNT = 1u << (GLR - 1);

    template <class Sync, class WSync, class Stamp>
    SC_HD static void run(const PassParams& P, uint32_t tile, uint32_t tid, Fe* lds, Fe* tw, Sync sync, WSync wsync, Stamp stamp, bool wave_local) {
        rare_t none = 0;
        run(P, tile, tid, lds, tw, sync, wsync, stamp, wave_local, none);
    }
    template <class Sync, class WSync, class Stamp>
    SC_HD static void run(const PassParams& P, uint32_t tile, uint32_t tid, Fe* lds, Fe* tw, Sync sync, WSync wsync, Stamp stamp, bool wave_local, rare_t& rare) {
        Round<LOGE, S, GLR, GLC> R;
        R.setup(P, ROUND == 0, tile, tid);
        Fe x[E];
        if constexpr (ROUND == 0) {
            Fe tin[E];
            Fe twv = fe_zero();
            if (P.prio_balance == 2) Round<LOGE, S, GLR, GLC>::set_prio(1, 3);
            if (tid < TW_COUNT) twv = P.mt[(uint64_t)tid << P.mt_shift];
            R.gather_global(P, SH, x, tin);
            if (P.prio_balance == 2) Round<LOGE, S, GLR, GLC>::set_prio(1, 0);
            if (tid < TW_COUNT) tw[tid] = twv;
            stamp(1);
            sync();
            stamp(2);
            R.template finish_global<FAST>(P, SH, x, tin, &rare);
        } else {
            R.gather_lds(SH, x, lds);
        }
        Fe tpre[E];
        bool prefetched = false;
        if constexpr (ROUND + 1 == NR && NR > 1) {
            if (P.tw_enable && P.twd) {
                R.load_twd(P, tpre);
                prefetched = true;
            }
        }
        const int prune = (ROUND <= 1) ? P.prune_log : 0;
        R.template butterflies<FAST>(SH, x, tw, 0, prune, ROUND + 1 == NR ? 1 : 0, P.prio_balance == 1 ? 1 : 0, &rare);
        stamp(3 + 2 * ROUND);
        if constexpr (ROUND + 1 < NR) {
            R.scatter_lds(SH, x, lds);
            if (NEXT_WAVE_LOCAL && wave_local) wsync(); else sync();
            stamp(4 + 2 * ROUND);
            FixedRounds<LOGE, GLR, GLC, ROUND + 1, ALT, FAST>::run(P, tile, tid, lds, tw, sync, wsync, stamp, wave_local, rare);
        } else {
            R.template scatter_global<ALT, FAST>(P, x, tpre, prefetched, &rare);
            stamp(4 + 2 * ROUND);
        }
    }
};

inline bool fixed_offsets_fit(const PassParams& P) {
    typedef unsigned __int128 u128;
    const u128 lim = (u128)1 << 32, r1 = (1u << P.logR) - 1u, c1 = (1u << P.logC) - 1u;
    if (!P.in_split && (r1 * P.in_rs + c1 * P.in_cs) * sizeof(Fe) >= lim) return false;
    if (!P.blk_enable && (r1 * P.out_rs + c1 * P.out_cs) * sizeof(Fe) >= lim) return false;
    if (P.tw_enable && P.twd && (r1 * P.tw_row_k * P.twd_stride + (c1 >> P.tw_col_shift)) * sizeof(Fe) >= lim) return false;
    return true;
}

inline bool fast_pass_ok(const PassParams& P) { return !P.coset_enable && P.prune_log == 0; }

struct RoundSched {
    int nrounds;
    int s[16];
    int sh[16];
};
SC_HD RoundSched make_rounds(int logR, int loge) {
    RoundSched rs;
    rs.nrounds = (logR + loge - 1) / loge;
    if (rs.nrounds == 0) rs.nrounds = 1;
    int rem = logR;
    for (int i = 0; i < rs.nrounds; ++i) {
        int s = (i == 0) ? (logR - loge * (rs.nrounds - 1)) : loge;
        if (s < 1) s = (logR == 0) ? 0 : 1;
        rem -= s;
        rs.s[i] = s;
        rs.sh[i] = rem;
    }
    return rs;
}

}
```

Baseline: 48.63 billion field-elements/s.

## Replace flag-and-redo fast NTT passes with exact carry-fixup arithmetic

The fast fixed8 NTT pass used lazy field arithmetic that flagged rare carry cases per workgroup, then ran a second redo kernel to recompute flagged tiles. This adds 'fix' variants of add, sub and Montgomery mul whose rare carry-propagation path sits behind a scalar branch inside the same instruction stream, so results are exact in one pass. The flag buffer, its memset and the always-launched redo kernel go away. The risk is the extra branch and cndmask work in the hot butterfly, plus correctness of the new assembly.

```diff
diff --git a/stark-anatomy_amd/csrc/core.h b/stark-anatomy_amd/csrc/core.h
--- a/stark-anatomy_amd/csrc/core.h
+++ b/stark-anatomy_amd/csrc/core.h
@@ -125,7 +125,6 @@
     std::vector<hipStream_t> seen_streams;
     DevBuf scratch[8];
     std::map<hipStream_t, DevBuf> ntt_work;
-    std::map<hipStream_t, DevBuf> ntt_flags;
     int fast_fixups = 1;
     int num_cus = 256;
     int xcd_remap = 1;
diff --git a/stark-anatomy_amd/csrc/core.hip b/stark-anatomy_amd/csrc/core.hip
--- a/stark-anatomy_amd/csrc/core.hip
+++ b/stark-anatomy_amd/csrc/core.hip
@@ -69,7 +69,7 @@
 }
 template <int GLR, int GLC>
 __global__ void __launch_bounds__(1 << (GLR + GLC - 3)) __attribute__((amdgpu_waves_per_eu(4)))
-ntt_pass_kernel_fixed8(const PassParams P, uint32_t ntiles, int xcd_remap, int wave_local, uint32_t* flags) {
+ntt_pass_kernel_fixed8(const PassParams P, uint32_t ntiles, int xcd_remap, int wave_local) {
     extern __shared__ __attribute__((aligned(16))) unsigned char smem_raw[];
     Fe* lds = reinterpret_cast<Fe*>(smem_raw);
     const uint32_t tile = fixed8_tile<GLR, GLC>(P, blockIdx.x, ntiles, xcd_remap);
@@ -77,24 +77,20 @@
     auto stamp = [](int) {};
     auto sync = [] { __syncthreads(); };
     auto wsync = [] { __builtin_amdgcn_fence(__ATOMIC_RELEASE, "wavefront"); __builtin_amdgcn_wave_barrier(); __builtin_amdgcn_fence(__ATOMIC_ACQUIRE, "wavefront"); };
-    rare_t rare = 0;
-    FixedRounds<3, GLR, GLC, 0, false, true>::run(P, tile, threadIdx.x, lds, tw, sync, wsync, stamp, wave_local != 0, rare);
-    if (rare_any(rare)) Round<3, 3, GLR, GLC>::store_word_at(flags + blockIdx.x, 0u, 1u);
+    rare_t none = 0;
+    FixedRounds<3, GLR, GLC, 0, false, ARITH_FIX>::run(P, tile, threadIdx.x, lds, tw, sync, wsync, stamp, wave_local != 0, none);
 }
 
 template <int GLR, int GLC>
 __global__ void __launch_bounds__(1 << (GLR + GLC - 3)) __attribute__((amdgpu_waves_per_eu(4)))
-ntt_pass_redo8_kernel(const PassParams P, uint32_t ntiles, int xcd_remap, int wave_local, uint32_t* flags, int all) {
+ntt_pass_kernel_exact8(const PassParams P, uint32_t ntiles, int xcd_remap, int wave_local) {
     extern __shared__ __attribute__((aligned(16))) unsigned char smem_raw[];
-    if (!all && flags[blockIdx.x] == 0) return;
     Fe* lds = reinterpret_cast<Fe*>(smem_raw);
     Fe* tw = lds + (1u << (GLR + GLC));
     auto stamp = [](int) {};
     auto sync = [] { __syncthreads(); };
     auto wsync = [] { __builtin_amdgcn_fence(__ATOMIC_RELEASE, "wavefront"); __builtin_amdgcn_wave_barrier(); __builtin_amdgcn_fence(__ATOMIC_ACQUIRE, "wavefront"); };
     FixedRounds<3, GLR, GLC, 0, false>::run(P, fixed8_tile<GLR, GLC>(P, blockIdx.x, ntiles, xcd_remap), threadIdx.x, lds, tw, sync, wsync, stamp, wave_local != 0);
-    if (!all) __syncthreads();
-    if (threadIdx.x == 0) flags[blockIdx.x] = 0;
 }
 
 __global__ void __launch_bounds__(256) pow_table_kernel(Fe* out, uint64_t count, Fe base_m, uint64_t step, Fe scale_m) {
@@ -305,6 +301,11 @@
         case 4: r0 = mont_mul_fast(x, y, rare); flags = selftest_word<SC_ASM_MUL != 0>(rare); break;
         case 5: mont_mul2_fast(x, y, z, w, r0, r1, rare); flags = selftest_word<SC_ASM_MUL != 0>(rare); break;
         case 6: fe_addsub2_fast(x, y, z, w, r0, r1, r2, r3, rare); flags = selftest_word<SC_ASM_ADDSUB != 0>(rare); break;
+        case 16: r0 = fe_add_fix(x, y); break;
+        case 17: r0 = fe_sub_fix(x, y); break;
+        case 18: r0 = mont_mul_fix(x, y); break;
+        case 19: mont_mul2_fix(x, y, z, w, r0, r1); break;
+        case 20: fe_addsub2_fix(x, y, z, w, r0, r1, r2, r3); break;
         default: r0 = fe_neg(x); break;
     }
     out[i] = r0; out[n + i] = r1; out[2 * n + i] = r2; out[3 * n + i] = r3;
@@ -589,17 +590,6 @@
     if (!*ok || d.npasses != 2) return SC_OK;
     SCCHK(direct_twiddles(pt, d, 0, false, st, &ex.inner_twd));
     if (ex.inner_twd) *ok = plan_batched(d, kind, loglen, logbatch, tb, in, work, out, g.tuning, ex);
-    return SC_OK;
-}
-
-int pass_flags(hipStream_t st, uint32_t nwg, uint32_t** out) {
-    DevBuf& b = g.ntt_flags[st];
-    const void* before = b.p;
-    const size_t had = b.bytes;
-    void* p;
-    SCCHK(grow_buffer(b, (size_t)nwg * sizeof(uint32_t), &p));
-    if (p != before || b.bytes != had) HIPCHK(hipMemsetAsync(p, 0, b.bytes, st));
-    *out = (uint32_t*)p;
     return SC_OK;
 }
 
@@ -627,14 +617,12 @@
         if (k.kind == PK_FIXED8) {
             const int lr = pd.p.logR, lc = pd.p.logC;
             const uint32_t nwg = pd.ntiles * pd.cols;
-            const bool fast = g.fast_fixups != 0 && fast_pass_ok(pd.p) && !pass_in_place(pd);
-            const int all = (!fast || g.fast_fixups == 2) ? 1 : 0;
-            uint32_t* flags;
-            SCCHK(pass_flags(st, nwg, &flags));
+            const bool fast = g.fast_fixups != 0 && fast_pass_ok(pd.p);
+            const bool exact = !fast || (g.fast_fixups == 2 && !pass_in_place(pd));
 #define SC_FIXED8(LR, LC)                                                                                                                                   \
             if (lr == LR && lc == LC) {                                                                                                                     \
-                if (fast) hipLaunchKernelGGL((ntt_pass_kernel_fixed8<LR, LC>), dim3(nwg), dim3(pd.threads), pd.lds_bytes, st, pd.p, pd.ntiles, remap, g.wave_local, flags); \
-                hipLaunchKernelGGL((ntt_pass_redo8_kernel<LR, LC>), dim3(nwg), dim3(pd.threads), pd.lds_bytes, st, pd.p, pd.ntiles, remap, g.wave_local, flags, all); \
+                if (fast) hipLaunchKernelGGL((ntt_pass_kernel_fixed8<LR, LC>), dim3(nwg), dim3(pd.threads), pd.lds_bytes, st, pd.p, pd.ntiles, remap, g.wave_local); \
+                if (exact) hipLaunchKernelGGL((ntt_pass_kernel_exact8<LR, LC>), dim3(nwg), dim3(pd.threads), pd.lds_bytes, st, pd.p, pd.ntiles, remap, g.wave_local); \
                 return SC_OK;                                                                                                                               \
             }
             SC_FIXED8_SHAPES(SC_FIXED8)
@@ -870,8 +858,6 @@
     for (auto& b : g.scratch) { if (b.p) hipFree(b.p); b = DevBuf{}; }
     for (auto& kv : g.ntt_work) if (kv.second.p) hipFree(kv.second.p);
     g.ntt_work.clear();
-    for (auto& kv : g.ntt_flags) if (kv.second.p) hipFree(kv.second.p);
-    g.ntt_flags.clear();
     if (g.later_words) hipFree(g.later_words);
     g.later_words = nullptr;
     if (g.stream) hipStreamDestroy(g.stream);
@@ -1198,7 +1184,7 @@
 int sc_field_selftest2(int op, const void* a, const void* b, const void* c, const void* d, void* out, uint32_t* word, uint64_t n) {
     std::lock_guard<std::mutex> lk(g_mu);
     SCCHK(ensure_init());
-    if (op < 0 || op > 7) return fail(SC_ERR_BAD_ARG, "unknown field self-test op");
+    if (op < 0 || (op > 7 && op < 16) || op > 20) return fail(SC_ERR_BAD_ARG, "unknown field self-test op");
     if (!n) return SC_OK;
     if (!a || !b || !c || !d || !out || !word) return fail(SC_ERR_BAD_ARG, "null argument");
     void *din, *dout, *dword;
diff --git a/stark-anatomy_amd/csrc/field.cuh b/stark-anatomy_amd/csrc/field.cuh
--- a/stark-anatomy_amd/csrc/field.cuh
+++ b/stark-anatomy_amd/csrc/field.cuh
@@ -152,6 +152,67 @@
     return fe_fixup_fast_c((uint64_t)r, (uint64_t)(r >> 64), neg, rare);
 }
 
+SC_HD Fe fe_fixup_fix_c(uint64_t lo, uint64_t hi, bool neg) {
+    const uint32_t d0 = (uint32_t)lo, d1 = (uint32_t)(lo >> 32), d2 = (uint32_t)hi, d3 = (uint32_t)(hi >> 32);
+    const uint32_t o0 = d0 + (neg ? 1u : 0u);
+    uint32_t o1 = d1, o2 = d2, o3 = neg ? d3 + P_TOP32 : d3;
+    if (neg && o0 == 0) {
+        o1 += 1u;
+        const uint32_t c1 = o1 == 0;
+        o2 += c1;
+        const uint32_t c2 = c1 && o2 == 0;
+        o3 += c2;
+    }
+    return Fe{((uint64_t)o1 << 32) | o0, ((uint64_t)o3 << 32) | o2};
+}
+SC_HD Fe fe_sub_fix_c(Fe a, Fe b) {
+    const uint64_t lo = a.lo - b.lo;
+    const uint64_t b0 = a.lo < b.lo;
+    const uint64_t hi = a.hi - b.hi;
+    const bool neg = (a.hi < b.hi) || (hi < b0);
+    return fe_fixup_fix_c(lo, hi - b0, neg);
+}
+SC_HD Fe fe_add_fix_c(Fe a, Fe b) {
+    const uint64_t lo = a.lo + b.lo;
+    const uint64_t c0 = lo < a.lo;
+    const uint64_t hi = a.hi + b.hi;
+    const uint64_t hi2 = hi + c0;
+    const bool ca = (hi < a.hi) || (hi2 < hi);
+    const uint32_t r0 = (uint32_t)lo, r1 = (uint32_t)(lo >> 32), r2 = (uint32_t)hi2, r3 = (uint32_t)(hi2 >> 32);
+    const bool sel = ca || r3 >= P_TOP32;
+    uint32_t o0 = r0 - (sel ? 1u : 0u), o1 = r1, o2 = r2, o3 = sel ? r3 - P_TOP32 : r3;
+    if (sel && r0 == 0) {
+        const uint32_t b1 = o1 == 0;
+        o1 -= 1u;
+        const uint32_t b2 = b1 && o2 == 0;
+        o2 -= b1;
+        const uint32_t b3 = b2 && o3 == 0;
+        o3 -= b2;
+        if (b3 && !ca) { o0 = 0; o1 = 0; o2 = 0; o3 = P_TOP32; }
+    }
+    return Fe{((uint64_t)o1 << 32) | o0, ((uint64_t)o3 << 32) | o2};
+}
+SC_HD Fe mont_mul_fix_c(Fe a, Fe b) {
+    u128 p00 = (u128)a.lo * b.lo, p01 = (u128)a.lo * b.hi, p10 = (u128)a.hi * b.lo, p11 = (u128)a.hi * b.hi;
+    const uint64_t t0 = (uint64_t)p00;
+    u128 mid = (p00 >> 64) + (uint64_t)p01 + (uint64_t)p10;
+    const uint64_t t1 = (uint64_t)mid;
+    u128 top = (mid >> 64) + (p01 >> 64) + (p10 >> 64) + p11;
+    const uint32_t w0 = (uint32_t)t0, w1 = (uint32_t)(t0 >> 32), w2 = (uint32_t)t1, w3 = (uint32_t)(t1 >> 32);
+    const uint64_t PH = P_TOP32;
+    const uint64_t s0 = (uint64_t)w0 * PH;
+    const uint32_t m3 = w3 - (uint32_t)s0;
+    const uint64_t delta = w3 < (uint32_t)s0;
+    const uint64_t s1 = (uint64_t)w1 * PH + (s0 >> 32);
+    const uint64_t s2 = (uint64_t)w2 * PH + (s1 >> 32);
+    const uint64_t s3 = (uint64_t)m3 * PH + (s2 >> 32);
+    const u128 q = (u128)(uint32_t)s1 | ((u128)(uint32_t)s2 << 32) | ((u128)s3 << 64);
+    const u128 d = top - q;
+    const bool neg = top < q || d < delta;
+    const u128 r = d - delta;
+    return fe_fixup_fix_c((uint64_t)r, (uint64_t)(r >> 64), neg);
+}
+
 SC_HD Fe to_mont(Fe a) { return mont_mul(a, Fe{R2_LO, R2_HI}); }
 SC_HD Fe from_mont(Fe a) { return mont_mul(a, fe_one()); }
 SC_HD Fe fe_mul(Fe a, Fe b) { return mont_mul(mont_mul(a, b), Fe{R2_LO, R2_HI}); }
@@ -303,6 +364,43 @@
     s1 = fe_add_fast(u1, v1, rare); d1 = fe_sub_fast(u1, v1, rare);
 #endif
 }
+SC_HD Fe fe_add_fix(Fe a, Fe b) {
+#if defined(__HIP_DEVICE_COMPILE__) && SC_ASM_ADDSUB
+    return fe_add_fix_asm(a, b);
+#else
+    return fe_add_fix_c(a, b);
+#endif
+}
+SC_HD Fe fe_sub_fix(Fe a, Fe b) {
+#if defined(__HIP_DEVICE_COMPILE__) && SC_ASM_ADDSUB
+    return fe_sub_fix_asm(a, b);
+#else
+    return fe_sub_fix_c(a, b);
+#endif
+}
+SC_HD Fe mont_mul_fix(Fe a, Fe b) {
+#if defined(__HIP_DEVICE_COMPILE__) && SC_ASM_MUL
+    return mont_mul_fix_asm(a, b);
+#else
+    return mont_mul_fix_c(a, b);
+#endif
+}
+SC_HD void mont_mul2_fix(Fe a0, Fe b0, Fe a1, Fe b1, Fe& r0, Fe& r1) {
+#if defined(__HIP_DEVICE_COMPILE__) && SC_ASM_MUL && SC_MUL2
+    mont_mul2_fix_asm(a0, b0, a1, b1, r0, r1);
+#else
+    r0 = mont_mul_fix(a0, b0);
+    r1 = mont_mul_fix(a1, b1);
+#endif
+}
+SC_HD void fe_addsub2_fix(Fe u0, Fe v0, Fe u1, Fe v1, Fe& s0, Fe& d0, Fe& s1, Fe& d1) {
+#if defined(__HIP_DEVICE_COMPILE__) && SC_ASM_ADDSUB && SC_MUL2
+    fe_addsub2_fix_asm(u0, v0, u1, v1, s0, d0, s1, d1);
+#else
+    s0 = fe_add_fix(u0, v0); d0 = fe_sub_fix(u0, v0);
+    s1 = fe_add_fix(u1, v1); d1 = fe_sub_fix(u1, v1);
+#endif
+}
 
 SC_HD Fe fe_sample_bytes(const uint8_t* b, uint32_t width) {
     uint64_t w0 = 0, w1 = 0, w2 = 0, w3 = 0;
diff --git a/stark-anatomy_amd/csrc/field_asm.cuh b/stark-anatomy_amd/csrc/field_asm.cuh
--- a/stark-anatomy_amd/csrc/field_asm.cuh
+++ b/stark-anatomy_amd/csrc/field_asm.cuh
@@ -92,7 +92,36 @@
     return Fe{((uint64_t)d1 << 32) | o0, ((uint64_t)o3 << 32) | d2};
 }
 
-template <bool FAST>
+#define SC_FIX_CARRY(o1, o2, o3, c)                                                \
+    SC_HAZ_NOP "v_addc_co_u32_e64 %[" o1 "], %[t], %[" o1 "], 0, %[" c "]\n\t"      \
+    SC_HAZ_NOP "v_addc_co_u32_e64 %[" o2 "], %[t], %[" o2 "], 0, %[t]\n\t"          \
+    SC_HAZ_NOP "v_addc_co_u32_e64 %[" o3 "], %[t], %[" o3 "], 0, %[t]\n\t"
+#define SC_FIX_BORROW(o0, o1, o2, o3, r3, b, ca)                                   \
+    SC_HAZ_NOP "v_subb_co_u32_e64 %[" o1 "], %[t], %[" o1 "], 0, %[" b "]\n\t"      \
+    SC_HAZ_NOP "v_subb_co_u32_e64 %[" o2 "], %[t], %[" o2 "], 0, %[t]\n\t"          \
+    SC_HAZ_NOP "v_subb_co_u32_e64 %[" o3 "], %[t], %[" o3 "], 0, %[t]\n\t"          \
+    "s_andn2_b64 %[t], %[t], %[" ca "]\n\t"                                        \
+    SC_HAZ_NOP "v_cndmask_b32_e64 %[" o0 "], %[" o0 "], 0, %[t]\n\t"               \
+    "v_cndmask_b32_e64 %[" o1 "], %[" o1 "], 0, %[t]\n\t"                          \
+    "v_cndmask_b32_e64 %[" o2 "], %[" o2 "], 0, %[t]\n\t"                          \
+    "v_cndmask_b32_e64 %[" o3 "], %[" o3 "], %[" r3 "], %[t]\n\t"
+
+__device__ __forceinline__ Fe a_fixup_fix(uint32_t d0, uint32_t d1, uint32_t d2, uint32_t d3, smask_t bw) {
+    smask_t c, t;
+    const uint32_t d3p = d3 + PH3;
+    uint32_t o0 = a_addc(d0, 0u, bw, c);
+    uint32_t o3 = a_cnd(d3, d3p, bw);
+    asm("s_cmp_eq_u64 %[c], 0\n\t"
+        "s_cbranch_scc1 1f\n\t"
+        SC_FIX_CARRY("o1", "o2", "o3", "c")
+        "1:"
+        : [o1] "+v"(d1), [o2] "+v"(d2), [o3] "+v"(o3), [t] "=&s"(t)
+        : [c] "s"(c)
+        : "scc");
+    return Fe{((uint64_t)d1 << 32) | o0, ((uint64_t)o3 << 32) | d2};
+}
+
+template <int MODE>
 __device__ __forceinline__ Fe mont_mul_core(Fe a, Fe b, smask_t& rare) {
     const uint32_t a0 = lo32(a.lo), a1 = hi32(a.lo), a2 = lo32(a.hi), a3 = hi32(a.hi);
     const uint32_t b0 = lo32(b.lo), b1 = hi32(b.lo), b2 = lo32(b.hi), b3 = hi32(b.hi);
@@ -141,7 +170,8 @@
     uint32_t r1 = a_subb(t5, lo32(s2), bw, bw);
     uint32_t r2 = a_subb(t6, lo32(s3), bw, bw);
     uint32_t r3 = a_subb(t7, hi32(s3), bw, bw);
-    if constexpr (FAST) return a_fixup_fast(r0, r1, r2, r3, bw, rare);
+    if constexpr (MODE == 1) return a_fixup_fast(r0, r1, r2, r3, bw, rare);
+    if constexpr (MODE == 2) return a_fixup_fix(r0, r1, r2, r3, bw);
     uint32_t ph = a_cnd(0u, PH3, bw);
     uint32_t o0 = a_addc(r0, 0u, bw, c);
     uint32_t o1 = a_addc(r1, 0u, c, c);
@@ -151,9 +181,13 @@
 }
 __device__ __forceinline__ Fe mont_mul_asm(Fe a, Fe b) {
     smask_t none = 0;
-    return mont_mul_core<false>(a, b, none);
-}
-__device__ __forceinline__ Fe mont_mul_fast_asm(Fe a, Fe b, smask_t& rare) { return mont_mul_core<true>(a, b, rare); }
+    return mont_mul_core<0>(a, b, none);
+}
+__device__ __forceinline__ Fe mont_mul_fast_asm(Fe a, Fe b, smask_t& rare) { return mont_mul_core<1>(a, b, rare); }
+__device__ __forceinline__ Fe mont_mul_fix_asm(Fe a, Fe b) {
+    smask_t none = 0;
+    return mont_mul_core<2>(a, b, none);
+}
 
 #define SC_V_MAD(d, cy, x, y, c)   asm volatile("v_mad_u64_u32 %0, %1, %2, %3, %4" : "=v"(d), "=s"(cy) : "v"(x), "v"(y), "v"(c))
 #define SC_V_INC(d, x, ci, co)     asm volatile("v_addc_co_u32_e64 %0, %1, 0, %2, %3" : "=v"(d), "=s"(co) : "v"(x), "s"(ci))
@@ -187,7 +221,7 @@
     smask_t c1, c2, c3, c4, c5, c6, c7, c8, c9, ct, bw, cx;
 };
 
-template <bool FAST>
+template <int MODE>
 __device__ __forceinline__ void mont_mul2_core(Fe xa, Fe wa, Fe xb, Fe wb, Fe& ra, Fe& rb, smask_t& rare) {
     MulState A, B;
     A.a0 = lo32(xa.lo); A.a1 = hi32(xa.lo); A.a2 = lo32(xa.hi); A.a3 = hi32(xa.hi);
@@ -240,7 +274,25 @@
     SC_V_NOP0();
     SC_BOTH(SC_V_SUBB(M.r3, M.bw, M.t7, hi32(M.s3), M.bw);)
     SC_V_NOP0();
-    if constexpr (FAST) {
+    if constexpr (MODE == 2) {
+        A.ph = A.r3 + PHc;
+        B.ph = B.r3 + PHc;
+        SC_BOTH(SC_V_ADDC(M.o0, M.cx, M.r0, zero32, M.bw);)
+        SC_BOTH(SC_V_CND(M.o3, M.r3, M.ph, M.bw);)
+        smask_t t;
+        asm volatile("s_or_b64 %[t], %[ca], %[cb]\n\t"
+                     "s_cbranch_scc0 1f\n\t"
+                     SC_FIX_CARRY("a1", "a2", "a3", "ca")
+                     SC_FIX_CARRY("b1", "b2", "b3", "cb")
+                     "1:"
+                     : [a1] "+v"(A.r1), [a2] "+v"(A.r2), [a3] "+v"(A.o3), [b1] "+v"(B.r1), [b2] "+v"(B.r2), [b3] "+v"(B.o3), [t] "=&s"(t)
+                     : [ca] "s"(A.cx), [cb] "s"(B.cx)
+                     : "scc");
+        ra = Fe{((uint64_t)A.r1 << 32) | A.o0, ((uint64_t)A.o3 << 32) | A.r2};
+        rb = Fe{((uint64_t)B.r1 << 32) | B.o0, ((uint64_t)B.o3 << 32) | B.r2};
+        return;
+    }
+    if constexpr (MODE == 1) {
         A.ph = A.r3 + PHc;
         B.ph = B.r3 + PHc;
         SC_BOTH(SC_V_ADDC(M.o0, M.cx, M.r0, zero32, M.bw);)
@@ -265,10 +317,14 @@
 }
 __device__ __forceinline__ void mont_mul2_asm(Fe xa, Fe wa, Fe xb, Fe wb, Fe& ra, Fe& rb) {
     smask_t none = 0;
-    mont_mul2_core<false>(xa, wa, xb, wb, ra, rb, none);
+    mont_mul2_core<0>(xa, wa, xb, wb, ra, rb, none);
 }
 __device__ __forceinline__ void mont_mul2_fast_asm(Fe xa, Fe wa, Fe xb, Fe wb, Fe& ra, Fe& rb, smask_t& rare) {
-    mont_mul2_core<true>(xa, wa, xb, wb, ra, rb, rare);
+    mont_mul2_core<1>(xa, wa, xb, wb, ra, rb, rare);
+}
+__device__ __forceinline__ void mont_mul2_fix_asm(Fe xa, Fe wa, Fe xb, Fe wb, Fe& ra, Fe& rb) {
+    smask_t none = 0;
+    mont_mul2_core<2>(xa, wa, xb, wb, ra, rb, none);
 }
 
 struct AddSubState {
@@ -385,5 +441,78 @@
     db = Fe{((uint64_t)B.d1 << 32) | B.e0, ((uint64_t)B.e3 << 32) | B.d2};
 }
 
+__device__ __forceinline__ Fe fe_sub_fix_asm(Fe a, Fe b) {
+    smask_t bw;
+    uint32_t d0 = a_sub_co(lo32(a.lo), lo32(b.lo), bw);
+    uint32_t d1 = a_subb(hi32(a.lo), hi32(b.lo), bw, bw);
+    uint32_t d2 = a_subb(lo32(a.hi), lo32(b.hi), bw, bw);
+    uint32_t d3 = a_subb(hi32(a.hi), hi32(b.hi), bw, bw);
+    return a_fixup_fix(d0, d1, d2, d3, bw);
+}
+
+__device__ __forceinline__ Fe fe_add_fix_asm(Fe a, Fe b) {
+    smask_t ca, cb, bo, t;
+    uint32_t r0 = a_add_co(lo32(a.lo), lo32(b.lo), ca);
+    uint32_t r1 = a_addc(hi32(a.lo), hi32(b.lo), ca, ca);
+    uint32_t r2 = a_addc(lo32(a.hi), lo32(b.hi), ca, ca);
+    uint32_t r3 = a_addc(hi32(a.hi), hi32(b.hi), ca, ca);
+    uint32_t t3 = a_sub_co(r3, PH3, cb);
+    const smask_t sel = ca | ~cb;
+    uint32_t o0 = a_subb(r0, 0u, sel, bo);
+    uint32_t o3 = a_cnd(r3, t3, sel);
+    asm("s_cmp_eq_u64 %[bo], 0\n\t"
+        "s_cbranch_scc1 1f\n\t"
+        SC_FIX_BORROW("o0", "o1", "o2", "o3", "r3", "bo", "ca")
+        "1:"
+        : [o0] "+v"(o0), [o1] "+v"(r1), [o2] "+v"(r2), [o3] "+v"(o3), [t] "=&s"(t)
+        : [r3] "v"(r3), [bo] "s"(bo), [ca] "s"(ca)
+        : "scc");
+    return Fe{((uint64_t)r1 << 32) | o0, ((uint64_t)o3 << 32) | r2};
+}
+
+__device__ __forceinline__ void fe_addsub2_fix_asm(Fe ua, Fe va, Fe ub, Fe vb, Fe& sa, Fe& da, Fe& sb, Fe& db) {
+    AddSubState A, B;
+    A.u0 = lo32(ua.lo); A.u1 = hi32(ua.lo); A.u2 = lo32(ua.hi); A.u3 = hi32(ua.hi);
+    A.v0 = lo32(va.lo); A.v1 = hi32(va.lo); A.v2 = lo32(va.hi); A.v3 = hi32(va.hi);
+    B.u0 = lo32(ub.lo); B.u1 = hi32(ub.lo); B.u2 = lo32(ub.hi); B.u3 = hi32(ub.hi);
+    B.v0 = lo32(vb.lo); B.v1 = hi32(vb.lo); B.v2 = lo32(vb.hi); B.v3 = hi32(vb.hi);
+    const uint32_t zero32 = 0, PHc = PH3;
+#define SC_BOTH(STEP) { AddSubState& M = A; STEP } { AddSubState& M = B; STEP }
+    SC_BOTH(SC_V_ADDCO(M.r0, M.ca, M.u0, M.v0); SC_V_SUBCO(M.d0, M.bd, M.u0, M.v0);)
+    SC_BOTH(SC_V_ADDC(M.r1, M.ca, M.u1, M.v1, M.ca); SC_V_SUBB(M.d1, M.bd, M.u1, M.v1, M.bd);)
+    SC_BOTH(SC_V_ADDC(M.r2, M.ca, M.u2, M.v2, M.ca); SC_V_SUBB(M.d2, M.bd, M.u2, M.v2, M.bd);)
+    SC_BOTH(SC_V_ADDC(M.r3, M.ca, M.u3, M.v3, M.ca); SC_V_SUBB(M.d3, M.bd, M.u3, M.v3, M.bd);)
+    SC_BOTH(SC_V_SUBCO(M.t3, M.cb, M.r3, PHc);)
+    A.ph = A.d3 + PHc;
+    B.ph = B.d3 + PHc;
+    SC_BOTH(SC_V_ADDC(M.e0, M.ce, M.d0, zero32, M.bd);)
+    SC_BOTH(SC_V_CND(M.e3, M.d3, M.ph, M.bd);)
+    A.sel = A.ca | ~A.cb;
+    B.sel = B.ca | ~B.cb;
+    SC_BOTH(SC_V_SUBB(M.s0, M.cb, M.r0, zero32, M.sel);)
+    SC_BOTH(SC_V_CND(M.s3, M.r3, M.t3, M.sel);)
+#undef SC_BOTH
+    smask_t t;
+    asm volatile("s_or_b64 %[t], %[cea], %[ceb]\n\t"
+                 "s_or_b64 %[t], %[t], %[boa]\n\t"
+                 "s_or_b64 %[t], %[t], %[bob]\n\t"
+                 "s_cbranch_scc0 1f\n\t"
+                 SC_FIX_CARRY("da1", "da2", "da3", "cea")
+                 SC_FIX_CARRY("db1", "db2", "db3", "ceb")
+                 SC_FIX_BORROW("sa0", "sa1", "sa2", "sa3", "ra3", "boa", "caa")
+                 SC_FIX_BORROW("sb0", "sb1", "sb2", "sb3", "rb3", "bob", "cab")
+                 "1:"
+                 : [da1] "+v"(A.d1), [da2] "+v"(A.d2), [da3] "+v"(A.e3), [db1] "+v"(B.d1), [db2] "+v"(B.d2), [db3] "+v"(B.e3),
+                   [sa0] "+v"(A.s0), [sa1] "+v"(A.r1), [sa2] "+v"(A.r2), [sa3] "+v"(A.s3),
+                   [sb0] "+v"(B.s0), [sb1] "+v"(B.r1), [sb2] "+v"(B.r2), [sb3] "+v"(B.s3), [t] "=&s"(t)
+                 : [ra3] "v"(A.r3), [rb3] "v"(B.r3), [cea] "s"(A.ce), [ceb] "s"(B.ce), [boa] "s"(A.cb), [bob] "s"(B.cb),
+                   [caa] "s"(A.ca), [cab] "s"(B.ca)
+                 : "scc");
+    sa = Fe{((uint64_t)A.r1 << 32) | A.s0, ((uint64_t)A.s3 << 32) | A.r2};
+    da = Fe{((uint64_t)A.d1 << 32) | A.e0, ((uint64_t)A.e3 << 32) | A.d2};
+    sb = Fe{((uint64_t)B.r1 << 32) | B.s0, ((uint64_t)B.s3 << 32) | B.r2};
+    db = Fe{((uint64_t)B.d1 << 32) | B.e0, ((uint64_t)B.e3 << 32) | B.d2};
+}
+
 }
 #endif
diff --git a/stark-anatomy_amd/csrc/ntt_tile.cuh b/stark-anatomy_amd/csrc/ntt_tile.cuh
--- a/stark-anatomy_amd/csrc/ntt_tile.cuh
+++ b/stark-anatomy_amd/csrc/ntt_tile.cuh
@@ -85,6 +85,8 @@
     return mont_mul(mont_pow(base_m, i * step), scale_m);
 }
 
+enum : int { ARITH_EXACT = 0, ARITH_FAST = 1, ARITH_FIX = 2 };
+
 template <int LOGE, int S, int GLR = -1, int GLC = -1>
 struct Round {
     static constexpr int E = 1 << LOGE;
@@ -154,12 +156,7 @@
     SC_HD static void store_at(Fe* base, uint32_t lane_bytes, Fe v) {
         *reinterpret_cast<gfe*>(reinterpret_cast<gchar*>(sgpr_pin(reinterpret_cast<uint64_t>(base))) + vgpr_pin(lane_bytes)) = v;
     }
-    SC_HD static void store_word_at(uint32_t* base, uint32_t lane_bytes, uint32_t v) {
-        typedef __attribute__((address_space(1))) uint32_t gword;
-        *reinterpret_cast<gword*>(reinterpret_cast<gchar*>(sgpr_pin(reinterpret_cast<uint64_t>(base))) + vgpr_pin(lane_bytes)) = v;
-    }
 #else
-    static void store_word_at(uint32_t* base, uint32_t lane_bytes, uint32_t v) { *reinterpret_cast<uint32_t*>(reinterpret_cast<char*>(base) + lane_bytes) = v; }
     static Fe load_at(const Fe* base, uint32_t lane_bytes) { return *reinterpret_cast<const Fe*>(reinterpret_cast<const char*>(base) + lane_bytes); }
     static void store_at(Fe* base, uint32_t lane_bytes, Fe v) { *reinterpret_cast<Fe*>(reinterpret_cast<char*>(base) + lane_bytes) = v; }
 #endif
@@ -206,9 +203,9 @@
             if (P.twd_in) tin[i] = P.twd_in[(ju + lane) & P.twd_in_mask];
         }
     }
-    template <bool FAST = false>
+    template <int FAST = ARITH_EXACT>
     SC_HD void finish_global(const PassParams& P, int sh, Fe* x, const Fe* tin, rare_t* rare = nullptr) const {
-        if (!FAST && P.coset_enable) {
+        if (FAST == ARITH_EXACT && P.coset_enable) {
 #pragma unroll
             for (int i = 0; i < E; ++i) {
                 const uint64_t j = in_index(P, i, sh);
@@ -221,19 +218,21 @@
             if (E & 1) x[E - 1] = mul1<FAST>(x[E - 1], tin[E - 1], rare);
         }
     }
-    template <bool FAST> SC_HD static Fe mul1(Fe a, Fe b, rare_t* rare) {
-        if constexpr (FAST) return mont_mul_fast(a, b, *rare);
+    template <int FAST> SC_HD static Fe mul1(Fe a, Fe b, rare_t* rare) {
+        if constexpr (FAST == ARITH_FAST) return mont_mul_fast(a, b, *rare);
+        else if constexpr (FAST == ARITH_FIX) return mont_mul_fix(a, b);
         else return mont_mul(a, b);
     }
-    template <bool FAST> SC_HD static void mul2(Fe a0, Fe b0, Fe a1, Fe b1, Fe& r0, Fe& r1, rare_t* rare) {
-        if constexpr (FAST) mont_mul2_fast(a0, b0, a1, b1, r0, r1, *rare);
+    template <int FAST> SC_HD static void mul2(Fe a0, Fe b0, Fe a1, Fe b1, Fe& r0, Fe& r1, rare_t* rare) {
+        if constexpr (FAST == ARITH_FAST) mont_mul2_fast(a0, b0, a1, b1, r0, r1, *rare);
+        else if constexpr (FAST == ARITH_FIX) mont_mul2_fix(a0, b0, a1, b1, r0, r1);
         else mont_mul2(a0, b0, a1, b1, r0, r1);
     }
     SC_HD void gather_lds(int sh, Fe* x, const Fe* lds) const {
 #pragma unroll
         for (int i = 0; i < E; ++i) x[i] = lds[lds_index(row(i, sh), cc[i >> S], logC)];
     }
-    template <bool FAST = false>
+    template <int FAST = ARITH_EXACT>
     SC_HD void butterflies(int sh, Fe* x, const Fe* tw, int tw_shift, int prune_log = 0, int last_hint = -1, int prio = 0, rare_t* rare = nullptr) const {
         const bool last = last_hint < 0 ? (sh == 0) : (last_hint != 0);
         set_prio(prio, 3);
@@ -242,7 +241,7 @@
             const int bit = S - 1 - q;
             const int b = sh + bit;
             const int tau = logR - 1 - b;
-            if (!FAST && tau < prune_log) {
+            if (FAST == ARITH_EXACT && tau < prune_log) {
                 const uint32_t nz = 1u << (logR - prune_log);
 #pragma unroll
                 for (int i0 = 0; i0 < E; ++i0) {
@@ -275,13 +274,17 @@
                 if (bf + 1 < E / 2) {
                     const int j0 = (((bf + 1) >> bit) << (bit + 1)) | ((bf + 1) & ((1 << bit) - 1));
                     const int j1 = j0 | (1 << bit);
-                    if constexpr (FAST) fe_addsub2_fast(x[i0], x[i1], x[j0], x[j1], x[i0], dd[bf], x[j0], dd[bf + 1], *rare);
+                    if constexpr (FAST == ARITH_FAST) fe_addsub2_fast(x[i0], x[i1], x[j0], x[j1], x[i0], dd[bf], x[j0], dd[bf + 1], *rare);
+                    else if constexpr (FAST == ARITH_FIX) fe_addsub2_fix(x[i0], x[i1], x[j0], x[j1], x[i0], dd[bf], x[j0], dd[bf + 1]);
                     else fe_addsub2(x[i0], x[i1], x[j0], x[j1], x[i0], dd[bf], x[j0], dd[bf + 1]);
                 } else {
                     Fe u = x[i0], v = x[i1];
-                    if constexpr (FAST) {
+                    if constexpr (FAST == ARITH_FAST) {
                         x[i0] = fe_add_fast(u, v, *rare);
                         dd[bf] = fe_sub_fast(u, v, *rare);
+                    } else if constexpr (FAST == ARITH_FIX) {
+                        x[i0] = fe_add_fix(u, v);
+                        dd[bf] = fe_sub_fix(u, v);
                     } else {
                         x[i0] = fe_add(u, v);
                         dd[bf] = fe_sub(u, v);
@@ -362,7 +365,7 @@
         if (P.blk_enable) scatter_global<true>(P, x, none, false);
         else scatter_global<false>(P, x, none, false);
     }
-    template <bool ALT, bool FAST = false>
+    template <bool ALT, int FAST = ARITH_EXACT>
     SC_HD void scatter_global(const PassParams& P, const Fe* x, const Fe (&twd_prefetched)[E], bool have_prefetched, rare_t* rare = nullptr) const {
         Fe v[E];
 #pragma unroll
@@ -426,7 +429,7 @@
     }
 };
 
-template <int LOGE, int S, int GLR = -1, int GLC = -1, bool FAST = false>
+template <int LOGE, int S, int GLR = -1, int GLC = -1, int FAST = ARITH_EXACT>
 SC_HD void ntt_round(const PassParams& P, int sh, bool first, uint32_t tile, uint32_t tid, Fe* lds, const Fe* tw, rare_t* rare = nullptr) {
     constexpr int E = 1 << LOGE;
     Round<LOGE, S, GLR, GLC> R;
@@ -464,7 +467,7 @@
 
 #define SC_FIXED4_SHAPES(X) X(8, 3) X(7, 4) X(10, 2) X(6, 5) X(9, 3) X(8, 4)
 #define SC_FIXED8_SHAPES(X) X(10, 2) X(9, 3) X(8, 4)
-template <int LOGE, int GLR, int GLC, int ROUND = 0, bool ALT = false, bool FAST = false>
+template <int LOGE, int GLR, int GLC, int ROUND = 0, bool ALT = false, int FAST = ARITH_EXACT>
 struct FixedRounds {
     static constexpr int E = 1 << LOGE;
     static constexpr int NR = (GLR + LOGE - 1) / LOGE;
```

New measurement: 49.35 billion field-elements/s, median of 6. 1.5% higher.
